# GenkiK/monodepth2

Measured on AMD Instinct MI355X. Metric: training images/sec at 640x192 mono, 1/2/4/8 GPUs; loss delta vs ref, higher is better.
Workload: dtype f32; 1 GPU; mono_640x192 ResNet-18 batch=12/GPU full train step (configs[1]); global_batch=12, height=192, width=640, parallelism=dp1, step=hipgraph replay

## Files before the change

include/md2hot.h:

```cpp
#ifndef MD2HOT_H
#define MD2HOT_H

#include <stddef.h>
#include <stdint.h>

#ifdef __cplusplus
extern "C" {
#endif

#define MD2_ABI_VERSION 24
#define MD2_MAX_SCALES 4
#define MD2_MAX_SRC 3

#define MD2_OK 0
#define MD2_ERR_ARG (-1)
#define MD2_ERR_HIP (-2)

#define MD2_NO_SSIM          (1u << 0)
#define MD2_AVG_REPROJECTION (1u << 1)
#define MD2_NO_AUTOMASK      (1u << 2)
#define MD2_V1_MULTISCALE    (1u << 3)
#define MD2_T_PER_SCALE      (1u << 4)
#define MD2_PREDICTIVE_MASK  (1u << 5)

// ... 136 lines not shown
int md2_adam_apply_dev(const md2_adam_chunk* table, const int* chunk_start, int k_begin, int k_end,
                       const float* const* grads, double beta1, double beta2, double eps, const float* hyper,
                       void* stream);

int md2_pose_fwd(int32_t frames, int32_t batch, uint32_t invert_mask, const float* axisangle,
                 const float* translation, float* T, void* stream);
int md2_pose_bwd(int32_t frames, int32_t batch, uint32_t invert_mask, const float* axisangle,
                 const float* translation, const float* grad_T, float* grad_axisangle,
                 float* grad_translation, void* stream);

typedef struct md2_aug_desc {
    int32_t items;
    int32_t frames;
    int32_t in_height, in_width;
    int32_t height, width;
    int32_t num_scales;
    int32_t reserved;
} md2_aug_desc;

#define MD2_AUG_BRIGHTNESS 0
#define MD2_AUG_CONTRAST   1
#define MD2_AUG_SATURATION 2
#define MD2_AUG_HUE        3

typedef struct md2_aug_item {
    uint8_t flip;
    uint8_t color_aug;
    uint8_t hue_shift;
    uint8_t reserved;
    uint8_t order[4];
    float brightness, contrast, saturation;
} md2_aug_item;

typedef struct md2_aug_plan md2_aug_plan;

md2_aug_plan* md2_aug_plan_create(const md2_aug_desc* desc);
void md2_aug_plan_destroy(md2_aug_plan* plan);

int md2_aug_run(md2_aug_plan* plan, const uint8_t* frames, const md2_aug_item* items,
                float* const* color, float* const* color_aug, void* stream);
int md2_aug_run2(md2_aug_plan* plan, const uint8_t* frames, const md2_aug_item* items,
                 float* const* color, float* const* color_aug, uint32_t* src8, void* stream);

#define MD2_BN_RELU     (1u << 0)
#define MD2_BN_RESIDUAL (1u << 1)
#define MD2_BN_BF16     (1u << 2)

typedef struct md2_bn_desc {
    int64_t pixels;
    int32_t channels;
    uint32_t flags;
    float eps, momentum;
    int32_t groups;
    int32_t reserved;
} md2_bn_desc;

size_t md2_bn_workspace_bytes(const md2_bn_desc* desc);
int md2_bn_fwd(const md2_bn_desc* desc, const void* x, const float* gamma, const float* beta,
               const void* residual, float* running_mean, float* running_var, void* y,
               float* save_mean, float* save_invstd, void* workspace, void* stream);
int md2_bn_bwd(const md2_bn_desc* desc, const void* x, const void* y, const void* grad_y,
               const float* gamma, const float* save_mean, const float* save_invstd,
               void* grad_x, void* grad_residual, float* grad_gamma, float* grad_beta,
               void* workspace, void* stream);
int md2_bn_bwd_multi(const md2_bn_desc* desc, const void* x, const void* y, const void* grad_y,
                     const void* grad_y2, const void* grad_y3, const float* gamma, const float* save_mean,
                     const float* save_invstd, void* grad_x, void* grad_residual, float* grad_gamma,
                     float* grad_beta, void* workspace, void* stream);
int md2_bn_fwd_mask(const md2_bn_desc* desc, const void* x, const float* gamma, const float* beta,
                    const void* residual, float* running_mean, float* running_var, void* y, uint8_t* relu_mask,
                    float* save_mean, float* save_invstd, void* workspace, void* stream);
int md2_bn_bwd_mask(const md2_bn_desc* desc, const void* x, const uint8_t* relu_mask, const void* grad_y,
                    const void* grad_y2, const void* grad_y3, const float* gamma, const float* save_mean,
                    const float* save_invstd, void* grad_x, void* grad_residual, float* grad_gamma,
                    float* grad_beta, void* workspace, void* stream);

#define MD2_POOL_BF16 (1u << 0)

typedef struct md2_pool_desc {
    int32_t batch, channels, height, width;
    uint32_t flags;
    int32_t reserved;
} md2_pool_desc;

int md2_maxpool3s2_fwd(const md2_pool_desc* desc, const void* x, void* y, uint32_t* idx, void* stream);
int md2_maxpool3s2_bwd(const md2_pool_desc* desc, const uint32_t* idx, const void* grad_y, void* grad_x,
                       void* stream);
int md2_maxpool3s2_bwd_add(const md2_pool_desc* desc, const uint32_t* idx, const void* grad_y, const void* grad_add,
                           void* grad_x, void* stream);
int md2_maxpool3s2_bwd_multi(const md2_pool_desc* desc, const uint32_t* idx, const void* grad_y, const void* grad_y2,
                             const void* grad_add, void* grad_x, void* stream);

#define MD2_CONV_NO_SPLIT  (1u << 1)
#define MD2_CONV_TILE_N32  (1u << 2)
#define MD2_CONV_TILE_N64  (1u << 3)
#define MD2_CONV_TILE_N128 (1u << 4)
#define MD2_CONV_X6        (1u << 5)
#define MD2_CONV_BM256     (1u << 6)
#define MD2_CONV_PRESPLIT  (1u << 7)
#define MD2_CONV_PATCH     (1u << 8)
#define MD2_CONV_S2_ONE    (1u << 9)
#define MD2_CONV_WS        (1u << 10)
#define MD2_CONV_BF16      (1u << 11)

typedef struct md2_conv_desc {
    int32_t batch, height, width, in_channels;
    int32_t out_channels, kernel_h, kernel_w, stride, pad;
    uint32_t flags;
} md2_conv_desc;

size_t md2_conv_workspace_bytes(const md2_conv_desc* desc);
int md2_conv_split_weights(const md2_conv_desc* desc, const float* weight, void* planes_fwd, void* planes_dgrad,
                           void* stream);
typedef struct md2_wsplit_entry {
    const float* weight;
    void* planes_fwd;
    void* planes_dgrad;
    int32_t co, kt, ci;
    int32_t block0;
    void* planes_col;
} md2_wsplit_entry;
int md2_conv_split_weights_multi(const md2_wsplit_entry* table, int n, int total_blocks, void* stream);
int md2_conv_bf16_weights(const md2_conv_desc* desc, const float* weight, void* w_fwd, void* w_dgrad, void* stream);
int md2_conv_bf16_weights_multi(const md2_wsplit_entry* table, int n, int total_blocks, void* stream);
int md2_conv_fwd(const md2_conv_desc* desc, const float* x, const float* weight, float* y, void* workspace,
                 void* stream);
int md2_conv_dgrad(const md2_conv_desc* desc, const float* grad_y, const float* weight, float* grad_x,
                   void* workspace, void* stream);
int md2_conv_col2im(const md2_conv_desc* desc, const float* cols, float* grad_x, void* stream);
int md2_conv_wgrad(const md2_conv_desc* desc, const float* x, const float* grad_y, float* grad_weight,
                   void* workspace, void* stream);
int md2_conv_direct(const md2_conv_desc* desc, const float* x, const float* wk, float* y, void* stream);
size_t md2_conv_wgrad_direct_workspace_bytes(const md2_conv_desc* desc);
int md2_conv_wgrad_direct(const md2_conv_desc* desc, const float* x, const float* grad_y, float* grad_weight,
                          void* workspace, void* stream);

#define MD2_EVAL_POST_PROCESS (1u << 0)
#define MD2_EVAL_RESIZE_DEPTH (1u << 1)
#define MD2_EVAL_GT_RANGE     (1u << 2)
#define MD2_EVAL_MEDIAN_SCALE (1u << 3)
#define MD2_EVAL_MEDIAN_LOWER (1u << 4)
#define MD2_EVAL_POOL_BATCH   (1u << 5)
#define MD2_EVAL_OUT 10

typedef struct md2_eval_desc {
    int32_t batch;
    int32_t height, width;
    int32_t gt_height, gt_width;
    int32_t crop_y0, crop_y1, crop_x0, crop_x1;
    uint32_t flags;
    double min_depth, max_depth;
    float eval_min, eval_max;
    double scale_factor;
} md2_eval_desc;

size_t md2_depth_eval_workspace_bytes(const md2_eval_desc* desc);
int md2_depth_eval(const md2_eval_desc* desc, const float* disp, const float* disp_flipped, const float* gt,
                   float* out, void* workspace, void* stream);

#ifdef __cplusplus
}
#endif
#endif
```

monodepth2_amd/_lib.py:

```python
from __future__ import annotations

import ctypes
import os
import threading

import torch

from .build import LIB_PATH as _BUILT_LIB
from .build import source_hash

LIB_PATH = os.environ.get("MD2_LIB", _BUILT_LIB)

MAX_SCALES = 4
MAX_SRC = 3
ABI_VERSION = 24

NO_SSIM = 1 << 0
AVG_REPROJECTION = 1 << 1
NO_AUTOMASK = 1 << 2
V1_MULTISCALE = 1 << 3
T_PER_SCALE = 1 << 4
PREDICTIVE_MASK = 1 << 5

_vp = ctypes.c_void_p


class Desc(ctypes.Structure):
    _fields_ = [("batch", ctypes.c_int32), ("height", ctypes.c_int32), ("width", ctypes.c_int32),
                ("num_src", ctypes.c_int32), ("num_scales", ctypes.c_int32), ("flags", ctypes.c_uint32),
                ("min_depth", ctypes.c_float), ("max_depth", ctypes.c_float),
                ("disparity_smoothness", ctypes.c_float), ("disp_dtype", ctypes.c_uint32),
                ("seed", ctypes.c_uint64)]


class Tensors(ctypes.Structure):
    _fields_ = [("disp", _vp * MAX_SCALES),
                ("color", (_vp * (1 + MAX_SRC)) * MAX_SCALES),
                ("K", _vp * MAX_SCALES),
                ("inv_K", _vp * MAX_SCALES),
                ("T", _vp),
                ("noise", _vp),
                ("seed_ptr", _vp),
                ("mask", _vp),
                ("src8", _vp)]


_lock = threading.Lock()
_lib = None

EXPORTS = ["md2_abi_version", "md2_last_error", "md2_workspace_bytes", "md2_select_bytes",
           "md2_photometric_fwd", "md2_photometric_bwd", "md2_generate_images", "md2_tiebreak_noise",
           "md2_timing_begin", "md2_timing_end", "md2_timing_calls", "md2_decoder_pad_fwd", "md2_decoder_pad_bwd",
           "md2_decoder_pad_workspace_bytes", "md2_adam_step", "md2_adam_step_dev", "md2_adam_hyper", "md2_adam_apply_dev", "md2_encoder_input",
           "md2_pose_fwd", "md2_pose_bwd", "md2_aug_plan_create", "md2_aug_plan_destroy", "md2_aug_run",
           "md2_bn_workspace_bytes", "md2_bn_fwd", "md2_bn_bwd", "md2_maxpool3s2_fwd", "md2_maxpool3s2_bwd",
           "md2_disp_head_workspace_bytes", "md2_disp_head_fwd", "md2_disp_head_bwd",
           "md2_stem_wgrad_workspace_bytes", "md2_stem_wgrad", "md2_stem_fwd", "md2_conv_col2im", "md2_bias_act_fwd", "md2_bias_act_bwd",
           "md2_bias_act_workspace_bytes", "md2_maxpool3s2_bwd_add", "md2_bn_bwd_multi",
           "md2_conv_fwd", "md2_conv_workspace_bytes", "md2_conv_split_weights",
           "md2_conv_dgrad", "md2_conv_wgrad", "md2_conv_direct", "md2_conv_wgrad_direct",
           "md2_conv_wgrad_direct_workspace_bytes", "md2_conv_split_weights_multi", "md2_bn_fwd_mask",
           "md2_bn_bwd_mask", "md2_build_id", "md2_maxpool3s2_bwd_multi", "md2_decoder_pad_bwd2", "md2_aug_run2",
           "md2_conv_bf16_weights", "md2_conv_bf16_weights_multi",
           "md2_depth_eval", "md2_depth_eval_workspace_bytes"]

DTYPE_F32 = 0
DTYPE_BF16 = 1
PAD_ELU = 1 << 0
PAD_UPSAMPLE = 1 << 1
PAD_NHWC = 1 << 2
PAD_BF16 = 1 << 3


class PadDesc(ctypes.Structure):
    _fields_ = [("batch", ctypes.c_int32), ("channels", ctypes.c_int32), ("height", ctypes.c_int32),
                ("width", ctypes.c_int32), ("skip_channels", ctypes.c_int32), ("flags", ctypes.c_uint32)]


class AugDesc(ctypes.Structure):
    _fields_ = [("items", ctypes.c_int32), ("frames", ctypes.c_int32), ("in_height", ctypes.c_int32),
                ("in_width", ctypes.c_int32), ("height", ctypes.c_int32), ("width", ctypes.c_int32),
                ("num_scales", ctypes.c_int32), ("reserved", ctypes.c_int32)]


class AugItem(ctypes.Structure):
    _fields_ = [("flip", ctypes.c_uint8), ("color_aug", ctypes.c_uint8), ("hue_shift", ctypes.c_uint8),
                ("reserved", ctypes.c_uint8), ("order", ctypes.c_uint8 * 4), ("brightness", ctypes.c_float),
                ("contrast", ctypes.c_float), ("saturation", ctypes.c_float)]


BN_RELU = 1 << 0
BN_RESIDUAL = 1 << 1
BN_BF16 = 1 << 2


class BnDesc(ctypes.Structure):
    _fields_ = [("pixels", ctypes.c_int64), ("channels", ctypes.c_int32), ("flags", ctypes.c_uint32),
                ("eps", ctypes.c_float), ("momentum", ctypes.c_float), ("groups", ctypes.c_int32),
                ("reserved", ctypes.c_int32)]


POOL_BF16 = 1 << 0


CONV_NO_SPLIT = 1 << 1
CONV_TILE_N32 = 1 << 2
CONV_TILE_N64 = 1 << 3
CONV_TILE_N128 = 1 << 4
CONV_X6 = 1 << 5
CONV_BM256 = 1 << 6
CONV_PRESPLIT = 1 << 7
CONV_PATCH = 1 << 8
CONV_S2_ONE = 1 << 9
CONV_WS = 1 << 10
CONV_BF16 = 1 << 11


class ConvDesc(ctypes.Structure):
    _fields_ = [("batch", ctypes.c_int32), ("height", ctypes.c_int32), ("width", ctypes.c_int32),
                ("in_channels", ctypes.c_int32), ("out_channels", ctypes.c_int32), ("kernel_h", ctypes.c_int32),
                ("kernel_w", ctypes.c_int32), ("stride", ctypes.c_int32), ("pad", ctypes.c_int32),
                ("flags", ctypes.c_uint32)]


class WsplitEntry(ctypes.Structure):
    _fields_ = [("weight", _vp), ("planes_fwd", _vp), ("planes_dgrad", _vp), ("co", ctypes.c_int32),
                ("kt", ctypes.c_int32), ("ci", ctypes.c_int32), ("block0", ctypes.c_int32), ("planes_col", _vp)]


class PoolDesc(ctypes.Structure):
    _fields_ = [("batch", ctypes.c_int32), ("channels", ctypes.c_int32), ("height", ctypes.c_int32),
                ("width", ctypes.c_int32), ("flags", ctypes.c_uint32), ("reserved", ctypes.c_int32)]


HEAD_WEIGHT_CL = 1 << 0
HEAD_BF16 = 1 << 1


class HeadDesc(ctypes.Structure):
    _fields_ = [("batch", ctypes.c_int32), ("channels", ctypes.c_int32), ("height", ctypes.c_int32),
                ("width", ctypes.c_int32), ("flags", ctypes.c_uint32)]


STEM_WEIGHT_CL = 1 << 0
STEM_BF16 = 1 << 1


class StemDesc(ctypes.Structure):
    _fields_ = [("batch", ctypes.c_int32), ("channels", ctypes.c_int32), ("height", ctypes.c_int32),
                ("width", ctypes.c_int32), ("flags", ctypes.c_uint32)]


# ... 88 lines not shown
    L.md2_generate_images.restype = ctypes.c_int
    L.md2_generate_images.argtypes = [ctypes.POINTER(Desc), ctypes.POINTER(Tensors),
                                      ctypes.POINTER(_vp), ctypes.POINTER(_vp), ctypes.POINTER(_vp), _vp]
    L.md2_tiebreak_noise.restype = ctypes.c_int
    L.md2_tiebreak_noise.argtypes = [ctypes.POINTER(Desc), _vp, ctypes.c_int, _vp, _vp]
    L.md2_decoder_pad_fwd.restype = ctypes.c_int
    L.md2_decoder_pad_fwd.argtypes = [ctypes.POINTER(PadDesc), _vp, _vp, _vp, _vp, _vp]
    L.md2_decoder_pad_bwd.restype = ctypes.c_int
    L.md2_decoder_pad_bwd.argtypes = [ctypes.POINTER(PadDesc), _vp, _vp, _vp, _vp, _vp, _vp, _vp, _vp]
    L.md2_decoder_pad_bwd2.restype = ctypes.c_int
    L.md2_decoder_pad_bwd2.argtypes = [ctypes.POINTER(PadDesc)] + [_vp] * 9
    L.md2_encoder_input.restype = ctypes.c_int
    L.md2_encoder_input.argtypes = [ctypes.c_int, ctypes.c_int, ctypes.c_int, ctypes.c_int, ctypes.c_int, _vp,
                                    ctypes.c_float, ctypes.c_float, _vp, _vp]
    L.md2_adam_step.restype = ctypes.c_int
    L.md2_adam_step.argtypes = [_vp, _vp, ctypes.c_int, _vp, ctypes.c_double, ctypes.c_double, ctypes.c_double,
                                ctypes.c_double, ctypes.c_int, _vp]
    L.md2_adam_step_dev.restype = ctypes.c_int
    L.md2_adam_step_dev.argtypes = [_vp, _vp, ctypes.c_int, _vp, _vp, ctypes.c_double, ctypes.c_double,
                                    ctypes.c_double, _vp, _vp, _vp]
    L.md2_adam_hyper.restype = ctypes.c_int
    L.md2_adam_hyper.argtypes = [_vp, ctypes.c_double, ctypes.c_double, _vp, _vp, _vp]
    L.md2_adam_apply_dev.restype = ctypes.c_int
    L.md2_adam_apply_dev.argtypes = [_vp, _vp, ctypes.c_int, ctypes.c_int, _vp, ctypes.c_double, ctypes.c_double,
                                     ctypes.c_double, _vp, _vp]
    L.md2_decoder_pad_workspace_bytes.restype = ctypes.c_size_t
    L.md2_decoder_pad_workspace_bytes.argtypes = [ctypes.POINTER(PadDesc)]
    L.md2_pose_fwd.restype = ctypes.c_int
    L.md2_pose_fwd.argtypes = [ctypes.c_int32, ctypes.c_int32, ctypes.c_uint32, _vp, _vp, _vp, _vp]
    L.md2_pose_bwd.restype = ctypes.c_int
    L.md2_pose_bwd.argtypes = [ctypes.c_int32, ctypes.c_int32, ctypes.c_uint32, _vp, _vp, _vp, _vp, _vp, _vp]
    L.md2_aug_plan_create.restype = _vp
    L.md2_aug_plan_create.argtypes = [ctypes.POINTER(AugDesc)]
    L.md2_aug_plan_destroy.restype = None
    L.md2_aug_plan_destroy.argtypes = [_vp]
    L.md2_aug_run.restype = ctypes.c_int
    L.md2_aug_run.argtypes = [_vp, _vp, _vp, ctypes.POINTER(_vp), ctypes.POINTER(_vp), _vp]
    L.md2_aug_run2.restype = ctypes.c_int
    L.md2_aug_run2.argtypes = [_vp, _vp, _vp, ctypes.POINTER(_vp), ctypes.POINTER(_vp), _vp, _vp]
    L.md2_bn_workspace_bytes.restype = ctypes.c_size_t
    L.md2_bn_workspace_bytes.argtypes = [ctypes.POINTER(BnDesc)]
    L.md2_bn_fwd.restype = ctypes.c_int
    L.md2_bn_fwd.argtypes = [ctypes.POINTER(BnDesc)] + [_vp] * 11
    L.md2_bn_bwd.restype = ctypes.c_int
    L.md2_bn_bwd.argtypes = [ctypes.POINTER(BnDesc)] + [_vp] * 12
    L.md2_maxpool3s2_fwd.restype = ctypes.c_int
    L.md2_maxpool3s2_fwd.argtypes = [ctypes.POINTER(PoolDesc), _vp, _vp, _vp, _vp]
    L.md2_maxpool3s2_bwd.restype = ctypes.c_int
    L.md2_maxpool3s2_bwd.argtypes = [ctypes.POINTER(PoolDesc), _vp, _vp, _vp, _vp]
    L.md2_bn_bwd_multi.restype = ctypes.c_int
    L.md2_bn_bwd_multi.argtypes = [ctypes.POINTER(BnDesc)] + [_vp] * 14
    L.md2_bn_fwd_mask.restype = ctypes.c_int
    L.md2_bn_fwd_mask.argtypes = [ctypes.POINTER(BnDesc)] + [_vp] * 12
    L.md2_bn_bwd_mask.restype = ctypes.c_int
    L.md2_bn_bwd_mask.argtypes = [ctypes.POINTER(BnDesc)] + [_vp] * 14
    L.md2_maxpool3s2_bwd_add.restype = ctypes.c_int
    L.md2_maxpool3s2_bwd_add.argtypes = [ctypes.POINTER(PoolDesc)] + [_vp] * 5
    L.md2_maxpool3s2_bwd_multi.restype = ctypes.c_int
    L.md2_maxpool3s2_bwd_multi.argtypes = [ctypes.POINTER(PoolDesc)] + [_vp] * 6
    L.md2_timing_begin.restype = ctypes.c_int
    L.md2_timing_begin.argtypes = [ctypes.c_int]
    L.md2_timing_calls.restype = ctypes.c_int
    L.md2_timing_calls.argtypes = [ctypes.POINTER(ctypes.c_double), ctypes.POINTER(ctypes.c_int),
                                   ctypes.POINTER(ctypes.c_double), ctypes.POINTER(ctypes.c_int)]
    L.md2_timing_end.restype = ctypes.c_int
    L.md2_timing_end.argtypes = [ctypes.POINTER(ctypes.c_double), ctypes.POINTER(ctypes.c_int),
                                 ctypes.POINTER(ctypes.c_double), ctypes.POINTER(ctypes.c_int)]


def lib():
    global _lib
    if _lib is not None:
        return _lib
    with _lock:
        if _lib is None:
            if not os.path.exists(LIB_PATH):
                raise RuntimeError(
                    f"{LIB_PATH} is not built. Build it with `python -m monodepth2_amd.build` "
                    "(hipcc --offload-arch=gfx950); there is no CPU fallback.")
            L = ctypes.CDLL(LIB_PATH, mode=ctypes.RTLD_GLOBAL)
            _declare(L)
            v = L.md2_abi_version()
            if v != ABI_VERSION:
                raise RuntimeError(f"libmd2hot ABI {v} != expected {ABI_VERSION}")
            if LIB_PATH == _BUILT_LIB:
                got, want = L.md2_build_id().decode(), source_hash()
                if got != want:
                    raise RuntimeError(
                        f"{LIB_PATH} was built from other sources (build id {got}, tree {want}): "
                        "rebuild it with `python -m monodepth2_amd.build`")
            _lib = L
    return _lib


def stream(device) -> int:
    idx = device.index if isinstance(device, torch.device) else device
    return torch._C._cuda_getCurrentRawStream(torch.cuda.current_device() if idx is None else idx)


def check(rc: int, what: str):
    if rc != 0:
        msg = lib().md2_last_error().decode(errors="replace")
        raise RuntimeError(f"{what} failed ({rc}): {msg}")


class KernelTimer:
# ... 21 lines not shown
```

monodepth2_amd/bn_ops.py:

```python
from __future__ import annotations

import contextlib
import ctypes
import os
from typing import Dict, Optional

import torch
import torch.nn as nn
import torch.nn.functional as F

from . import _lib

ENABLED = True
_GROUPS = 1


@contextlib.contextmanager
def bn_groups(n: int):
    global _GROUPS
    prev, _GROUPS = _GROUPS, int(n)
    try:
        yield
    finally:
        _GROUPS = prev

_CL = torch.channels_last
_workspaces: Dict[int, torch.Tensor] = {}
_workspaces_keep = []


def _workspace(device: torch.device, nbytes: int) -> torch.Tensor:
    key = _lib.stream(device)
    ws = _workspaces.get(key)
    if ws is None or ws.numel() < nbytes:
        if ws is not None:
            _workspaces_keep.append(ws)
        with torch.cuda.stream(torch.cuda.current_stream(device)):
            ws = torch.empty(max(nbytes, 1 << 20), dtype=torch.uint8, device=device)
        _workspaces[key] = ws
    return ws


_descs: Dict[tuple, tuple] = {}


def _desc(key: tuple):
    hit = _descs.get(key)
    if hit is None:
        d = _lib.BnDesc(*key, 0)
        hit = _descs[key] = (d, _lib.lib().md2_bn_workspace_bytes(ctypes.byref(d)))
    return hit


def _supported(C: int) -> bool:
    Q = C // 4
    return C % 4 == 0 and Q > 0 and (Q & (Q - 1)) == 0


class _BNAct(torch.autograd.Function):

    @staticmethod
    def forward(ctx, x, weight, bias, running_mean, running_var, residual, relu: bool, eps: float,
                momentum: float, groups: int, aliases: int = 0):
        B, C, H, W = x.shape
        flags = ((_lib.BN_RELU if relu else 0) | (_lib.BN_RESIDUAL if residual is not None else 0)
                 | (_lib.BN_BF16 if x.dtype == torch.bfloat16 else 0))
        key = (B * H * W, C, flags, eps, momentum, groups)
        d, nbytes = _desc(key)
        L = _lib.lib()
        ws = _workspace(x.device, nbytes)
        y = torch.empty_like(x, memory_format=_CL)
        stats = torch.empty(2, groups, C, device=x.device)
        mean, invstd = stats[0], stats[1]
        mask = torch.empty(x.numel() // 4, dtype=torch.uint8, device=x.device) if relu else None
        stream = _lib.stream(x.device)
        rc = L.md2_bn_fwd_mask(ctypes.byref(d), x.data_ptr(), weight.data_ptr(), bias.data_ptr(),
                               residual.data_ptr() if residual is not None else None,
                               running_mean.data_ptr() if running_mean is not None else None,
                               running_var.data_ptr() if running_var is not None else None,
                               y.data_ptr(), mask.data_ptr() if mask is not None else None,
                               mean.data_ptr(), invstd.data_ptr(), ws.data_ptr(), stream)
        _lib.check(rc, "md2_bn_fwd_mask")
        ctx.save_for_backward(x, mask, weight, mean, invstd)
        ctx.desc = key
        ctx.has_res = residual is not None
        if aliases:
            ctx.set_materialize_grads(False)
            return (y,) + tuple(y.view_as(y) for _ in range(aliases))
        return y

    @staticmethod
    def backward(ctx, *grads):
        x, mask, weight, mean, invstd = ctx.saved_tensors
        gs = [g.to(x.dtype).contiguous(memory_format=_CL) for g in grads if g is not None]
        if not gs:
            return (None,) * 11
        gy = gs[0]
        d, nbytes = _desc(ctx.desc)
        L = _lib.lib()
        ws = _workspace(x.device, nbytes)
        gx = torch.empty_like(x, memory_format=_CL)
        gr = torch.empty_like(x, memory_format=_CL) if ctx.has_res else None
        gw = torch.empty_like(weight)
        gb = torch.empty_like(weight)
        bwd, name = (L.md2_bn_bwd_mask, "md2_bn_bwd_mask") if mask is not None else \
            (L.md2_bn_bwd_multi, "md2_bn_bwd_multi")
        rc = bwd(ctypes.byref(d), x.data_ptr(), mask.data_ptr() if mask is not None else None,
                 gy.data_ptr(), gs[1].data_ptr() if len(gs) > 1 else None,
                 gs[2].data_ptr() if len(gs) > 2 else None,
                 weight.data_ptr(), mean.data_ptr(), invstd.data_ptr(), gx.data_ptr(),
                 gr.data_ptr() if gr is not None else None, gw.data_ptr(), gb.data_ptr(), ws.data_ptr(),
                 _lib.stream(x.device))
        _lib.check(rc, name)
        return gx, gw, gb, None, None, gr, None, None, None, None, None


def bn_act(bn: nn.BatchNorm2d, x: torch.Tensor, residual: Optional[torch.Tensor] = None,
           relu: bool = True, aliases: int = 0):
    if not 0 <= aliases <= 2:
        raise ValueError("bn_act: at most two aliases")
    groups = _GROUPS if bn.training else 1
    if groups > 1 and x.shape[0] % groups:
        raise ValueError(f"batch {x.shape[0]} does not split into {groups} BatchNorm groups")
    if (ENABLED and bn.training and x.is_cuda and x.dtype in (torch.float32, torch.bfloat16) and x.dim() == 4
            and bn.affine and bn.track_running_stats and bn.momentum is not None and _supported(x.shape[1])
            and x.numel() // 4 // groups < 2 ** 31
            and x.is_contiguous(memory_format=_CL) and x.shape[1] > 1
            and (residual is None or residual.is_contiguous(memory_format=_CL))):
        if residual is not None and residual.dtype != x.dtype:
            residual = residual.to(x.dtype)
        if bn.num_batches_tracked is not None:
            bn.num_batches_tracked.add_(groups)
        k = aliases if torch.is_grad_enabled() else 0
        out = _BNAct.apply(x, bn.weight, bn.bias, bn.running_mean, bn.running_var, residual, relu, bn.eps,
                           bn.momentum, groups, k)
        if aliases and not k:
            return (out,) * (aliases + 1)
        return out
    y = bn(x) if groups == 1 else torch.cat([bn(xc) for xc in x.chunk(groups)], 0)
    if residual is not None:
        y = y + residual
    y = F.relu(y) if relu else y
    return (y,) * (aliases + 1) if aliases else y


_ALIAS_SUM = os.environ.get("MD2_ALIAS_SUM", "1") != "0"


class _MaxPool(torch.autograd.Function):

    @staticmethod
    def forward(ctx, x, with_alias: bool = False, out_alias: bool = False):
        B, C, H, W = x.shape
        Ho, Wo = (H - 1) // 2 + 1, (W - 1) // 2 + 1
        d = _lib.PoolDesc(B, C, H, W, _lib.POOL_BF16 if x.dtype == torch.bfloat16 else 0, 0)
        y = torch.empty((B, C, Ho, Wo), device=x.device, dtype=x.dtype, memory_format=_CL)
        idx = torch.empty(B * Ho * Wo * C // 4, device=x.device, dtype=torch.int32)
        stream = _lib.stream(x.device)
        _lib.check(_lib.lib().md2_maxpool3s2_fwd(ctypes.byref(d), x.data_ptr(), y.data_ptr(), idx.data_ptr(), stream),
                   "md2_maxpool3s2_fwd")
        ctx.save_for_backward(idx)
        ctx.desc = (B, C, H, W, d.flags, 0)
        ctx.xshape, ctx.dtype = x.shape, x.dtype
        ctx.with_alias, ctx.out_alias = with_alias, out_alias
        if not (with_alias or out_alias):
            return y
        ctx.set_materialize_grads(False)
        outs = (y,) + ((y.view_as(y),) if out_alias else ()) + ((x.view_as(x),) if with_alias else ())
        return outs

    @staticmethod
    def backward(ctx, gy, *rest):
        (idx,) = ctx.saved_tensors
        rest = list(rest)
        gy2 = rest.pop(0) if ctx.out_alias else None
        galias = rest.pop(0) if ctx.with_alias else None
        if gy is None:
            gy, gy2 = gy2, None
        if gy is None:
            return (galias.to(ctx.dtype) if galias is not None else None), None, None
        gy = gy.to(ctx.dtype).contiguous(memory_format=_CL)
        if gy2 is not None:
            gy2 = gy2.to(ctx.dtype).contiguous(memory_format=_CL)
        if galias is not None:
            galias = galias.to(ctx.dtype).contiguous(memory_format=_CL)
        gx = torch.empty(ctx.xshape, device=gy.device, dtype=ctx.dtype, memory_format=_CL)
        d = _lib.PoolDesc(*ctx.desc)
        _lib.check(_lib.lib().md2_maxpool3s2_bwd_multi(ctypes.byref(d), idx.data_ptr(), gy.data_ptr(),
                                                       gy2.data_ptr() if gy2 is not None else None,
                                                       galias.data_ptr() if galias is not None else None,
                                                       gx.data_ptr(), _lib.stream(gy.device)),
                   "md2_maxpool3s2_bwd_multi")
        return gx, None, None


def _pool_ok(pool: nn.MaxPool2d, x: torch.Tensor) -> bool:
# ... 21 lines not shown
```

monodepth2_amd/build.py:

```python
from __future__ import annotations

import hashlib
import os
import shutil
import subprocess
import sys

HERE = os.path.dirname(os.path.abspath(__file__))
CSRC = os.path.join(HERE, "csrc")
INCLUDE = os.path.join(os.path.dirname(HERE), "include")
LIB_NAME = "libmd2hot.so"
LIB_PATH = os.path.join(CSRC, LIB_NAME)
SOURCES = ["md2hot.hip", "decoder.hip", "pose.hip", "augment.hip", "bnorm.hip", "pool.hip", "adam.hip", "disphead.hip", "stem.hip", "bias_act.hip", "conv.hip", "direct.hip", "glue.hip", "eval.hip"]
ARCH = os.environ.get("MD2_OFFLOAD_ARCH", "gfx950")


def hipcc() -> str:
    for cand in (os.environ.get("HIPCC"), "/opt/rocm/bin/hipcc", shutil.which("hipcc")):
        if cand and os.path.exists(cand):
            return cand
    raise RuntimeError("hipcc not found (ROCm toolchain required to build libmd2hot.so)")


def needs_build() -> bool:
    if not os.path.exists(LIB_PATH):
        return True
    t = os.path.getmtime(LIB_PATH)
    deps = [os.path.join(CSRC, s) for s in SOURCES] + [os.path.join(INCLUDE, "md2hot.h"),
                                                       os.path.join(CSRC, "md2_bf16.h")]
    if any(os.path.getmtime(d) > t for d in deps):
        return True
    return built_id(LIB_PATH) != source_hash()


def built_id(path: str):
    try:
        with open(path, "rb") as f:
            data = f.read()
    except OSError:
        return None
    i = data.find(BUILD_ID_MARKER)
    if i < 0:
        return None
    i += len(BUILD_ID_MARKER)
    return data[i:i + 16].decode("ascii", errors="replace")


BUILD_ID_MARKER = b"md2-build-id:"


FLAGS = {"md2hot.hip": ["-fno-slp-vectorize", "-mllvm", "--amdgpu-sched-strategy=iterative-ilp"],
         "conv.hip": ["-mllvm", "--amdgpu-sched-strategy=max-ilp"],
         "bnorm.hip": ["-mllvm", "--amdgpu-sched-strategy=max-ilp"],
         "decoder.hip": ["-mllvm", "--amdgpu-sched-strategy=max-ilp"],
         "disphead.hip": ["-fno-slp-vectorize"], "glue.hip": ["-fno-slp-vectorize"]}


def source_hash() -> str:
    h = hashlib.sha256()
    for path in [os.path.join(CSRC, s) for s in SOURCES] + [os.path.join(INCLUDE, "md2hot.h"),
                                                          os.path.join(CSRC, "md2_bf16.h")]:
        h.update(os.path.basename(path).encode())
        with open(path, "rb") as f:
            h.update(f.read())
    h.update(repr(sorted(FLAGS.items())).encode())
    h.update(ARCH.encode())
    return h.hexdigest()[:16]


def build(force: bool = False, verbose: bool = False) -> str:
    if not force and not needs_build():
        return LIB_PATH
    import concurrent.futures as cf
    objdir = os.path.join(CSRC, "obj")
    os.makedirs(objdir, exist_ok=True)
    base = [hipcc(), "-O3", f"--offload-arch={ARCH}", "-std=c++17", "-fPIC", "-I" + INCLUDE]
    bid = ['-DMD2_BUILD_ID="%s"' % source_hash()]

    def compile_one(src):
        obj = os.path.join(objdir, os.path.splitext(src)[0] + ".o")
        cmd = base + FLAGS.get(src, []) + (bid if src == "glue.hip" else []) + ["-c", os.path.join(CSRC, src), "-o", obj]
        if verbose:
            print(" ".join(cmd), file=sys.stderr)
        subprocess.run(cmd, check=True)
        return obj

    with cf.ThreadPoolExecutor(max_workers=min(len(SOURCES), os.cpu_count() or 1)) as ex:
        objs = list(ex.map(compile_one, SOURCES))
    tmp = LIB_PATH + ".tmp"
    cmd = [hipcc(), f"--offload-arch={ARCH}", "-fPIC", "-shared", "-o", tmp] + objs
    if verbose:
        print(" ".join(cmd), file=sys.stderr)
    subprocess.run(cmd, check=True)
    os.replace(tmp, LIB_PATH)
    return LIB_PATH


if __name__ == "__main__":
    print(build(force="--force" in sys.argv, verbose=True))
```

monodepth2_amd/conv_ops.py:

```python
from __future__ import annotations

import ctypes
import os
import types
from typing import Dict, Tuple

import torch
import torch.nn as nn
import torch.nn.functional as F

from . import _lib

_CL = torch.channels_last
ENABLED = True
AUTOTUNE = True
PLANE_BANK = os.environ.get("MD2_PLANE_BANK", "1") != "0"
_ws: Dict[Tuple[int, int], torch.Tensor] = {}
_choice: Dict[tuple, int] = {}
_times: Dict[tuple, dict] = {}
X6 = _lib.CONV_X6
BM256 = _lib.CONV_BM256
PRESPLIT = _lib.CONV_PRESPLIT
PATCH = _lib.CONV_PATCH
S2_ONE = _lib.CONV_S2_ONE
# ... 4 lines not shown
_NAMES_X6 = ("x6", "x6_256", "x6_ns", "x6_256_ns")
_NAMES_X6P = ("x6p", "x6p_256", "x6p_ns", "x6p_256_ns")
_WFLAGS = (X6 | WS, X6 | WS | BM256)
_NAMES_WS = ("x6ws", "x6ws_256")


def _x6_flags(gemm_c: int, k: int, stride: int, n_out: int):
    flags, names = _FLAGS, _NAMES_X6
    if n_out > 64 and gemm_c >= 32:
        flags, names = flags + _WFLAGS, names + _NAMES_WS
    if k == 3 and stride == 1 and gemm_c % 32 == 0 and n_out > 16:
        return flags + _PFLAGS, names + _NAMES_X6P
    return flags, names


_ws_keep = []


def _workspace(device: torch.device, nbytes: int) -> torch.Tensor:
    key = (device.index, _lib.stream(device))
    ws = _ws.get(key)
    if ws is None or ws.numel() < nbytes:
        if ws is not None:
            _ws_keep.append(ws)
        ws = torch.empty(max(nbytes, 1 << 20), dtype=torch.uint8, device=device)
        _ws[key] = ws
    return ws


_descs: Dict[tuple, tuple] = {}


def _desc_ws(x: torch.Tensor, w: torch.Tensor, stride: int, pad: int, flags: int = 0):
    k = (tuple(x.shape), tuple(w.shape), stride, pad, flags)
    hit = _descs.get(k)
    if hit is None:
        B, C, H, W = x.shape
        N, _, KH, KW = w.shape
        d = _lib.ConvDesc(B, H, W, C, N, KH, KW, stride, pad, flags)
        hit = _descs[k] = (d, _lib.lib().md2_conv_workspace_bytes(ctypes.byref(d)))
    return hit


def _desc(x: torch.Tensor, w: torch.Tensor, stride: int, pad: int, flags: int = 0):
    return _desc_ws(x, w, stride, pad, flags)[0]


def _call(fn: str, x, w, stride, pad, flags, p0, p1, p2, device):
    d, nbytes = _desc_ws(x, w, stride, pad, flags)
    ws = _workspace(device, nbytes)
    _lib.check(getattr(_lib.lib(), fn)(ctypes.byref(d), p0, p1, p2, ws.data_ptr(), _lib.stream(device)), fn)


def _fwd(x, w, stride, pad, flags=0):
    B, _, H, W = x.shape
    N, _, KH, KW = w.shape
    y = torch.empty(B, N, (H + 2 * pad - KH) // stride + 1, (W + 2 * pad - KW) // stride + 1, device=x.device,
                    memory_format=_CL)
    _call("md2_conv_fwd", x, w, stride, pad, flags, x.data_ptr(), w.data_ptr(), y.data_ptr(), x.device)
    return y


def _dgrad(gy, x, w, pad, flags=0, stride=1):
    gx = torch.empty_like(x, memory_format=_CL)
    _call("md2_conv_dgrad", x, w, stride, pad, flags, gy.data_ptr(), w.data_ptr(), gx.data_ptr(), x.device)
    return gx


def _dgrad_col(gy, x, w, stride, pad, flags):
    N, C, KH, KW = w.shape
    B, _, H, W = x.shape
    pc = _bank.col_planes(w) if (_bank is not None and flags & X6 and _COL_BANK) else None
    if pc is not None:
        cols = _fwd_planes(gy, _col_shape(KH * KW * C, N), pc, 1, 0, flags)
    else:
        wcol = w.permute(2, 3, 1, 0).reshape(KH * KW * C, N, 1, 1).contiguous()
        cols = _fwd(gy, wcol, 1, 0, flags)
    gx = torch.empty_like(x, memory_format=_CL)
    d = _lib.ConvDesc(B, H, W, C, N, KH, KW, stride, pad, 0)
    _lib.check(_lib.lib().md2_conv_col2im(ctypes.byref(d), cols.data_ptr(), gx.data_ptr(), _lib.stream(x.device)),
               "md2_conv_col2im")
    return gx


_COL_BANK = os.environ.get("MD2_COL_PLANES", "1") != "0"


def _col_shape(rows: int, n: int):
    return types.SimpleNamespace(shape=torch.Size((rows, n, 1, 1)))


def _col_x(w):
    return types.SimpleNamespace(shape=torch.Size((1, w.shape[1], 8, 8)))


def _x6_ok(x, w) -> bool:
    return x.shape[1] % 8 == 0 and w.shape[0] % 8 == 0


def _x6_s2_ok(x, w, stride) -> bool:
    return stride == 2 and _x6_ok(x, w) and w.shape[0] >= 32


def _split_weights(x, w, stride, pad, dgrad: bool):
    n = w.numel()
    pf = torch.empty(3 * n, dtype=torch.bfloat16, device=w.device)
    pd = torch.empty(3 * n, dtype=torch.bfloat16, device=w.device) if dgrad else None
    _lib.check(_lib.lib().md2_conv_split_weights(ctypes.byref(_desc(x, w, stride, pad)), w.data_ptr(), pf.data_ptr(),
                                                 pd.data_ptr() if pd is not None else None,
                                                 _lib.stream(w.device)),
               "md2_conv_split_weights")
    return pf, pd
# ... 94 lines not shown
                                                         pf.data_ptr(), None, _lib.stream(w.device)),
                       "md2_conv_split_weights")
            self.entries[k] = [w, pf, None, pc]
        else:
            e[3] = pc
        self._col_pending.add(k)
        self.dirty = True
        return None


_bank: PlaneBank | None = None
_bank_bf: PlaneBank | None = None


def plane_bank() -> PlaneBank:
    global _bank
    if _bank is None:
        _bank = PlaneBank()
    return _bank


def plane_bank_bf16() -> PlaneBank:
    global _bank_bf
    if _bank_bf is None:
        _bank_bf = PlaneBank(bf16=True)
    return _bank_bf


def begin_step(device: torch.device, bf16: bool = False):
    (plane_bank_bf16() if bf16 else plane_bank()).begin_step(device)


def end_step():
    for b in (_bank, _bank_bf):
        if b is not None:
            b.end_step()


def _planes_for(x, w, stride, pad, need_dg: bool):
    if _bank is not None:
        got = _bank.planes(x, w, stride, pad, need_dg)
        if got is not None:
            return got
    return _split_weights(x, w, stride, pad, need_dg)


def _bank_dgrad(x, w, stride, pad):
    if _bank is None:
        return None
    got = _bank.planes(x, w, stride, pad, True)
    return got[1] if got is not None else None


def _fwd_planes(x, w, planes, stride, pad, flags):
    B, _, H, W = x.shape
    N, _, KH, KW = w.shape
    y = torch.empty(B, N, (H + 2 * pad - KH) // stride + 1, (W + 2 * pad - KW) // stride + 1, device=x.device,
                    memory_format=_CL)
    _call("md2_conv_fwd", x, w, stride, pad, flags | PRESPLIT, x.data_ptr(), planes.data_ptr(), y.data_ptr(),
          x.device)
    return y


def _dgrad_planes(gy, x, w, planes, pad, flags, stride=1):
    gx = torch.empty_like(x, memory_format=_CL)
    _call("md2_conv_dgrad", x, w, stride, pad, flags | PRESPLIT, gy.data_ptr(), planes.data_ptr(), gx.data_ptr(),
          x.device)
    return gx


def _wgrad(gy, x, w, stride, pad, flags=0):
    gw = torch.empty_like(w, memory_format=_CL)
    _call("md2_conv_wgrad", x, w, stride, pad, flags, x.data_ptr(), gy.data_ptr(), gw.data_ptr(), x.device)
    return gw


def _miopen_bwd(gy, x, w, stride, pad, mask):
    return torch.ops.aten.convolution_backward(gy, x, w, None, (stride, stride), (pad, pad), (1, 1), False, (0, 0), 1,
                                               mask)


_pinned: Dict[tuple, str] = {}


def _key_of(row) -> tuple:
    return (row["op"], tuple(row["x"]), tuple(row["w"]), int(row["stride"]), int(row["pad"]))


def load_choices(path: str) -> int:
    import json
    with open(path) as f:
        rows = json.load(f)["rows"]
    for row in rows:
        _pinned[_key_of(row)] = row["kept"]
    _choice.clear()
    return len(rows)


def save_choices(path: str) -> int:
    import json
    rows = []
    for k, i in sorted(_choice.items()):
        names = _names.get(k)
        if names is None:
            continue
        op, xs, ws, st, pd = k
        rows.append({"op": op, "x": list(xs), "w": list(ws), "stride": st, "pad": pd, "kept": names[i],
                     "ms": _times.get(k, {})})
    with open(path, "w") as f:
        json.dump({"rows": rows}, f, indent=1)
    return len(rows)


# ... 112 lines not shown
            i = names.index(name)
            changed += int(_choice.get(k) != i)
            _choice[k] = i
    return changed


_DIRECT = ((16, 16), (32, 16), (16, 32))
_ddescs: Dict[tuple, object] = {}


def _direct_ok(cin: int, cout: int, k: int, stride: int) -> bool:
    return k == 3 and stride == 1 and (cin, cout) in _DIRECT


def _direct(a: torch.Tensor, wk: torch.Tensor, pad: int, cout: int, flags: int = 0) -> torch.Tensor:
    B, C, H, W = a.shape
    y = torch.empty(B, cout, H + 2 * pad - 2, W + 2 * pad - 2, device=a.device, memory_format=_CL,
                    dtype=torch.bfloat16 if flags & BF else torch.float32)
    k = (tuple(a.shape), cout, pad, flags)
    d = _ddescs.get(k)
    if d is None:
        d = _ddescs[k] = _lib.ConvDesc(B, H, W, C, cout, 3, 3, 1, pad, flags)
    _lib.check(_lib.lib().md2_conv_direct(ctypes.byref(d), a.data_ptr(), wk.data_ptr(), y.data_ptr(),
                                          _lib.stream(a.device)), "md2_conv_direct")
    return y


def _direct_wgrad(gy, x, w, pad, flags=0):
    N, C = w.shape[0], w.shape[1]
    gw = torch.empty_like(w, memory_format=_CL)
    d = _desc(x, w, 1, pad, flags)
    nbytes = _lib.lib().md2_conv_wgrad_direct_workspace_bytes(ctypes.byref(d))
    ws = _workspace(x.device, nbytes)
    _lib.check(_lib.lib().md2_conv_wgrad_direct(ctypes.byref(d), x.data_ptr(), gy.data_ptr(), gw.data_ptr(),
                                                ws.data_ptr(), _lib.stream(x.device)), "md2_conv_wgrad_direct")
    return gw


def _direct_fwd(x, w, pad, flags=0):
    return _direct(x, w.permute(2, 3, 1, 0).contiguous(), pad, w.shape[0], flags)


def _direct_dgrad(gy, w, pad, flags=0):
    return _direct(gy, w.flip(2, 3).permute(2, 3, 0, 1).contiguous(), 2 - pad, w.shape[1], flags)


def _fits(cin: int, cout: int) -> bool:
    return cin % 4 == 0 and cout % 4 == 0


class _Conv(torch.autograd.Function):

    @staticmethod
    def forward(ctx, x, weight, stride: int, pad: int):
        ctx.stride, ctx.pad = stride, pad
        ctx.key = (tuple(x.shape), tuple(weight.shape), stride, pad)
        x6 = _x6_ok(x, weight)
        xf, xn = _x6_flags(x.shape[1], weight.shape[2], stride, weight.shape[0]) if x6 else ((), ())
        cands = None
        i = _cached("fwd", ctx.key)
        if i is None or not (x6 and i < len(xf)):
            direct = _direct_ok(weight.shape[1], weight.shape[0], weight.shape[2], stride)
            cands = [(lambda f=f: _fwd(x, weight, stride, pad, f)) for f in xf] + \
                [lambda: _fwd(x, weight, stride, pad)] + \
                ([lambda: _direct_fwd(x, weight, pad), lambda: _direct_fwd(x, weight, pad, X6)] if direct else []) + \
                [lambda: F.conv2d(x, weight, None, stride, pad)]
            names = list(xn) + ["f32mfma"] + (["direct", "direct_x6"] if direct else []) + ["miopen"]
            if i is None:
                i = _fastest("fwd", ctx.key, cands, names)
        planes_dg = None
        if x6 and i < len(xf):
            pf, planes_dg = _planes_for(x, weight, stride, pad, stride == 1 or _x6_s2_ok(x, weight, stride))
            y = _fwd_planes(x, weight, pf, stride, pad, xf[i])
        else:
            y = cands[i]()
        ctx.save_for_backward(x, weight, planes_dg)
        return y

    @staticmethod
    def backward(ctx, gy):
        x, w, planes_dg = ctx.saved_tensors
        s, p = ctx.stride, ctx.pad
        gy = gy.contiguous(memory_format=_CL)
        need_x, need_w = ctx.needs_input_grad[0], ctx.needs_input_grad[1]
        gx = gw = None
        mi_x = mi_w = False
        if need_x:
            if s == 1:
                x6 = _x6_ok(x, w)
                xf, xn = _x6_flags(w.shape[0], w.shape[2], 1, w.shape[1]) if x6 else ((), ())
                direct = _direct_ok(w.shape[0], w.shape[1], w.shape[2], s)
                cands = [(lambda f=f: _dgrad(gy, x, w, p, f)) for f in xf] + \
                    [lambda: _dgrad(gy, x, w, p)] + \
                    ([lambda: _direct_dgrad(gy, w, p), lambda: _direct_dgrad(gy, w, p, X6)] if direct else []) + \
                    [lambda: _miopen_bwd(gy, x, w, s, p, (True, False, False))[0]]
                names = list(xn) + ["f32mfma"] + (["direct", "direct_x6"] if direct else []) + ["miopen"]
                i = _fastest("dgrad", ctx.key, cands, names)
                if x6 and i < len(xf) and planes_dg is None:
                    planes_dg = _bank_dgrad(x, w, s, p)
                if x6 and i < len(xf) and planes_dg is not None:
                    gx = _dgrad_planes(gy, x, w, planes_dg, p, xf[i])
                elif i < len(cands) - 1:
                    gx = cands[i]()
                else:
                    mi_x = True
            elif _x6_s2_ok(x, w, s):
                sf = (X6, X6 | S2_ONE)
                cands = [(lambda f=f: _dgrad(gy, x, w, p, f, 2)) for f in sf] + \
                    [lambda: _dgrad_col(gy, x, w, s, p, X6), lambda: _dgrad_col(gy, x, w, s, p, X6 | BM256)] + \
                    [lambda: _miopen_bwd(gy, x, w, s, p, (True, False, False))[0]]
                i = _fastest("dgrad", ctx.key, cands, ["x6_s2", "x6_s2one", "x6_col", "x6_col_256", "miopen"])
                if i < len(sf) and planes_dg is None:
                    planes_dg = _bank_dgrad(x, w, s, p)
                if i < len(sf):
                    gx = (_dgrad_planes(gy, x, w, planes_dg, p, sf[i], 2) if planes_dg is not None else cands[i]())
                elif i < len(cands) - 1:
                    gx = cands[i]()
                else:
                    mi_x = True
            else:
                mi_x = True
        if need_w:
            direct = _direct_ok(w.shape[1], w.shape[0], w.shape[2], s) and w.shape[0] == 16
            x6 = _x6_ok(x, w)
            pw = x6 and w.shape[2] == 3 and w.shape[3] == 3 and s == 1
            wsw = x6 and w.shape[0] > 64
            cands = ([lambda: _wgrad(gy, x, w, s, p, X6)] if x6 else []) + \
                ([lambda: _wgrad(gy, x, w, s, p, X6 | WS), lambda: _wgrad(gy, x, w, s, p, X6 | WS | BM256)]
                 if wsw else []) + \
                ([lambda: _wgrad(gy, x, w, s, p, X6 | PATCH)] if pw else []) + [lambda: _wgrad(gy, x, w, s, p)] + \
                ([lambda: _direct_wgrad(gy, x, w, p), lambda: _direct_wgrad(gy, x, w, p, X6)] if direct else []) + \
                [lambda: _miopen_bwd(gy, x, w, s, p, (False, True, False))[1]]
            i = _fastest("wgrad", ctx.key, cands,
                         (["x6"] if x6 else []) + (["x6ws", "x6ws_256"] if wsw else []) + (["x6pw"] if pw else []) + ["f32mfma"] +
                         (["direct", "direct_x6"] if direct else []) + ["miopen"])
            if i < len(cands) - 1:
                gw = cands[i]()
            else:
                mi_w = True
        if mi_x or mi_w:
            gxm, gwm, _ = _miopen_bwd(gy, x, w, s, p, (mi_x, mi_w, False))
            gx = gxm if mi_x else gx
            gw = gwm if mi_w else gw
        return gx, gw, None, None


BF16_ENABLED = os.environ.get("MD2_CONV_BF16", "1") != "0"
BF = _lib.CONV_BF16
_FLAGS_BF = (BF, BF | BM256, BF | NO_SPLIT, BF | BM256 | NO_SPLIT)
_NAMES_BF = ("bf16", "bf16_256", "bf16_ns", "bf16_256_ns")


_PFLAGS_BF = (BF | PATCH, BF | PATCH | NO_SPLIT, BF | PATCH | BM256, BF | PATCH | BM256 | NO_SPLIT)
_PNAMES_BF = ("bf16p", "bf16p_ns", "bf16p_256", "bf16p_256_ns")


def _bf_flags(n_out: int, gemm_c: int = 0, k: int = 0, stride: int = 0):
    wide = n_out > 64
    fl = _FLAGS_BF if wide else (_FLAGS_BF[0], _FLAGS_BF[2])
    nm = _NAMES_BF if wide else (_NAMES_BF[0], _NAMES_BF[2])
    if k == 3 and stride == 1 and gemm_c % 32 == 0 and n_out > 16:
        fl = fl + (_PFLAGS_BF if wide else _PFLAGS_BF[:2])
        nm = nm + (_PNAMES_BF if wide else _PNAMES_BF[:2])
    return fl, nm


def _bf_planes_for(x, w, stride, pad, need_dg: bool):
    if _bank_bf is not None:
        got = _bank_bf.planes(x, w, stride, pad, need_dg)
        if got is not None:
            return got
    return _bf16_weights(x, w, stride, pad, need_dg)


def _w_bf16_view(x, w, stride, pad):
    N, C, kh, kw = w.shape
    pf = _bf_planes_for(x, w, stride, pad, False)[0]
    return pf.view(N, kh, kw, C).permute(0, 3, 1, 2)


def _fwd_bf(x, w, plane, stride, pad, flags):
    B, _, H, W = x.shape
    N, _, KH, KW = w.shape
    y = torch.empty(B, N, (H + 2 * pad - KH) // stride + 1, (W + 2 * pad - KW) // stride + 1, device=x.device,
                    dtype=torch.bfloat16, memory_format=_CL)
    _call("md2_conv_fwd", x, w, stride, pad, flags, x.data_ptr(), plane.data_ptr(), y.data_ptr(), x.device)
    return y


def _dgrad_bf(gy, x, w, plane, pad, flags, stride=1):
    gx = torch.empty_like(x, memory_format=_CL)
    _call("md2_conv_dgrad", x, w, stride, pad, flags, gy.data_ptr(), plane.data_ptr(), gx.data_ptr(), x.device)
    return gx


def _wgrad_bf(gy, x, w, stride, pad, flags=BF):
    gw = torch.empty_like(w, memory_format=_CL)
# ... 65 lines not shown
                                ["bf16"] + (["bf16pw"] if pw else []) + (["bf16ws_256"] if w256 else []) +
                                (["direct_bf16"] if direct else []))]()
        return gx, gw, None, None


def _bf16_autocast() -> bool:
    return torch.is_autocast_enabled("cuda") and torch.get_autocast_dtype("cuda") == torch.bfloat16


def _bf16_ok(x: torch.Tensor, weight: torch.Tensor, stride: int, pad: int) -> bool:
    return (ENABLED and BF16_ENABLED and x.is_cuda and x.dim() == 4 and x.dtype in (torch.bfloat16, torch.float32)
            and weight.dtype == torch.float32 and weight.shape[2] == weight.shape[3]
            and _fits(weight.shape[1], weight.shape[0]) and x.is_contiguous(memory_format=_CL)
            and weight.is_contiguous(memory_format=_CL) and stride >= 1 and 0 <= pad < weight.shape[2]
            and _sizes_ok(x, weight, stride, pad) and _bf16_autocast())


def conv2d_bf16(x: torch.Tensor, weight: torch.Tensor, stride: int, pad: int) -> torch.Tensor:
    xb = x if x.dtype == torch.bfloat16 else x.to(torch.bfloat16)
    with torch.autocast("cuda", enabled=False):
        return _ConvBF16.apply(xb, weight, stride, pad)


def _sizes_ok(x: torch.Tensor, weight: torch.Tensor, stride: int, pad: int) -> bool:
    B, _, H, W = x.shape
    Co, _, kh, kw = weight.shape
    ho = (H + 2 * pad - kh) // stride + 1
    wo = (W + 2 * pad - kw) // stride + 1
    return (ho >= 1 and wo >= 1 and x.numel() < 2 ** 29 and B * ho * wo * Co < 2 ** 29
            and weight.numel() < 2 ** 29)


def _shape_ok(x: torch.Tensor, weight: torch.Tensor, stride: int = 1, pad: int = 0) -> bool:
    return (ENABLED and x.is_cuda and x.dtype == torch.float32 and weight.dtype == torch.float32 and x.dim() == 4
            and weight.shape[2] == weight.shape[3] and _fits(weight.shape[1], weight.shape[0])
            and x.is_contiguous(memory_format=_CL) and weight.is_contiguous(memory_format=_CL)
            and not torch.is_autocast_enabled() and stride >= 1 and 0 <= pad < weight.shape[2]
            and _sizes_ok(x, weight, stride, pad))


def supports(conv: nn.Conv2d, x: torch.Tensor) -> bool:
    k, s, p = conv.kernel_size, conv.stride, conv.padding
    return (conv.bias is None and conv.groups == 1 and tuple(conv.dilation) == (1, 1)
            and conv.padding_mode == "zeros" and k[0] == k[1] and s[0] == s[1] and p[0] == p[1] and p[0] < k[0]
            and _shape_ok(x, conv.weight, s[0], p[0]))


def _module_ok(conv: nn.Conv2d) -> bool:
    k, s, p = conv.kernel_size, conv.stride, conv.padding
    return (conv.bias is None and conv.groups == 1 and tuple(conv.dilation) == (1, 1)
            and conv.padding_mode == "zeros" and k[0] == k[1] and s[0] == s[1] and p[0] == p[1] and p[0] < k[0])


def conv2d(conv: nn.Conv2d, x: torch.Tensor) -> torch.Tensor:
    if supports(conv, x):
        return _Conv.apply(x, conv.weight, conv.stride[0], conv.padding[0])
    if _module_ok(conv) and _bf16_ok(x, conv.weight, conv.stride[0], conv.padding[0]):
        return conv2d_bf16(x, conv.weight, conv.stride[0], conv.padding[0])
    return conv(x)


def conv2d_w(x: torch.Tensor, weight: torch.Tensor, stride: int = 1, pad: int = 0) -> torch.Tensor:
    if _shape_ok(x, weight, stride, pad):
        return _Conv.apply(x, weight, stride, pad)
    if _bf16_ok(x, weight, stride, pad):
        return conv2d_bf16(x, weight, stride, pad)
    return F.conv2d(x, weight, None, stride, pad)


if os.environ.get("MD2_CONV_CHOICES"):
    load_choices(os.environ["MD2_CONV_CHOICES"])
```

monodepth2_amd/csrc/bnorm.hip:

```cpp

#include <hip/hip_runtime.h>

#include <stdint.h>
#include <stdlib.h>

#include "md2_bf16.h"
#include "md2hot.h"

int md2_report_error(int code, const char* msg);

namespace {

constexpr int kThreads = 256;
constexpr int kMaxBlocks = 1024;

struct Map {
    int Q;
    int QPT;
    int PPB;
};

__host__ __device__ inline Map make_map(int C) {
    Map m;
    m.Q = C / 4;
    m.QPT = m.Q > kThreads ? m.Q / kThreads : 1;
    m.PPB = m.Q >= kThreads ? 1 : kThreads / m.Q;
    return m;
}

struct Work {
    float* part;
    float* coef;
};

__host__ __device__ __forceinline__ Work work(void* ws, int G, int C, int NG) {
    Work w;
    w.part = (float*)ws;
    w.coef = w.part + 2 * (size_t)NG * G * C;
    return w;
}

__device__ __forceinline__ float4 ld4(const float* p) { return *(const float4*)p; }
__device__ __forceinline__ void st4(float* p, float4 v) { *(float4*)p = v; }

template <typename T>
__device__ __forceinline__ float4 ldT(const void* p, size_t off) { return md2::ld4T<T>(p, off); }
template <typename T>
__device__ __forceinline__ void stT(void* p, size_t off, float4 v) { md2::st4T<T>(p, off, v); }

__device__ void block_partials(float4 a, float4 b, int q, int pl, const Map& m, int C, int rows, int row, Work w,
                               float4 (*lds)[kThreads]) {
    lds[0][threadIdx.x] = a;
    lds[1][threadIdx.x] = b;
    __syncthreads();
    for (int half = m.PPB / 2; half > 0; half /= 2) {
        if (pl < half) {
            const int o = threadIdx.x + half * m.Q;
            const float4 u = lds[0][o], v = lds[1][o];
            a.x += u.x; a.y += u.y; a.z += u.z; a.w += u.w;
            b.x += v.x; b.y += v.y; b.z += v.z; b.w += v.w;
            lds[0][threadIdx.x] = a;
            lds[1][threadIdx.x] = b;
        }
        __syncthreads();
    }
    if (pl == 0) {
        float* pa = w.part + (size_t)(4 * q) * rows + row;
        float* pb = w.part + ((size_t)C + 4 * q) * rows + row;
        pa[0] = a.x; pa[rows] = a.y; pa[2 * (size_t)rows] = a.z; pa[3 * (size_t)rows] = a.w;
        pb[0] = b.x; pb[rows] = b.y; pb[2 * (size_t)rows] = b.z; pb[3 * (size_t)rows] = b.w;
    }
    __syncthreads();
}

template <typename T>
__global__ void __launch_bounds__(kThreads) bn_stats_kernel(const void* __restrict__ x, long long P, int C, int G,
                                                            void* ws) {
    const Map m = make_map(C);
    const int NG = gridDim.y, grp = blockIdx.y;
    const Work w = work(ws, G, C, NG);
    x = (const char*)x + (size_t)grp * P * C * sizeof(T);
    __shared__ float4 lds[2][kThreads];
    for (int qq = 0; qq < m.QPT; ++qq) {
        const int q = (threadIdx.x % m.Q) + qq * kThreads, pl = threadIdx.x / m.Q;
        float4 s = {0.f, 0.f, 0.f, 0.f}, ss = {0.f, 0.f, 0.f, 0.f};
        auto acc = [&](const float4 v) {
            s.x += v.x; s.y += v.y; s.z += v.z; s.w += v.w;
            ss.x += v.x * v.x; ss.y += v.y * v.y; ss.z += v.z * v.z; ss.w += v.w * v.w;
        };
        const long long stride = (long long)G * m.PPB;
        long long p = (long long)blockIdx.x * m.PPB + pl;
        for (; p + 3 * stride < P; p += 4 * stride) {
            const float4 v0 = ldT<T>(x, p * C + 4 * q), v1 = ldT<T>(x, (p + stride) * C + 4 * q),
                         v2 = ldT<T>(x, (p + 2 * stride) * C + 4 * q), v3 = ldT<T>(x, (p + 3 * stride) * C + 4 * q);
            acc(v0); acc(v1); acc(v2); acc(v3);
        }
        for (; p < P; p += stride) acc(ldT<T>(x, p * C + 4 * q));
        block_partials(s, ss, q, pl, m, C, NG * G, grp * G + blockIdx.x, w, lds);
    }
}

__device__ bool channel_sums(Work w, int rows, int r0, int G, int C, int c, double& a, double& b) {
    __shared__ double red[2][kThreads / 64];
    static_assert(kMaxBlocks <= 4 * kThreads, "four partial rows per thread at most");
    const float* ca = w.part + (size_t)c * rows + r0;
    const float* cb = w.part + ((size_t)C + c) * rows + r0;
    float pa[4], pb[4];
#pragma unroll
    for (int u = 0; u < 4; ++u) {
        const int g = threadIdx.x + u * kThreads;
        pa[u] = g < G ? ca[g] : 0.f;
        pb[u] = g < G ? cb[g] : 0.f;
    }
    a = 0.0;
    b = 0.0;
#pragma unroll
    for (int u = 0; u < 4; ++u) {
        a += pa[u];
        b += pb[u];
    }
#pragma unroll
    for (int o = 32; o > 0; o >>= 1) {
        a += __shfl_xor(a, o, 64);
        b += __shfl_xor(b, o, 64);
    }
    if ((threadIdx.x & 63) == 0) {
        red[0][threadIdx.x >> 6] = a;
        red[1][threadIdx.x >> 6] = b;
    }
    __syncthreads();
    a = red[0][0];
    b = red[1][0];
#pragma unroll
    for (int i = 1; i < kThreads / 64; ++i) {
        a += red[0][i];
        b += red[1][i];
    }
    __syncthreads();
    return threadIdx.x == 0;
}

__global__ void __launch_bounds__(kThreads) bn_stats_final_kernel(long long P, int C, int G, int NG, float eps,
// ... 353 lines not shown
        if (g2) {
            float u[8];
            ld8bf(g2, o, u);
#pragma unroll
            for (int e = 0; e < 8; ++e) gv[e] += u[e];
        }
        if (g3) {
            float u[8];
            ld8bf(g3, o, u);
#pragma unroll
            for (int e = 0; e < 8; ++e) gv[e] += u[e];
        }
        if (RELU) {
            if constexpr (MIN) {
                const uint32_t m = ((const uint16_t*)y)[o / 8];
#pragma unroll
                for (int e = 0; e < 8; ++e) gv[e] = ((m >> ((e & 3) + 8 * (e >> 2))) & 1u) ? gv[e] : 0.f;
            } else {
                float yv[8];
                ld8bf(y, o, yv);
#pragma unroll
                for (int e = 0; e < 8; ++e) gv[e] = yv[e] > 0.f ? gv[e] : 0.f;
            }
        }
        ld8bf(x, o, v);
#pragma unroll
        for (int e = 0; e < 8; ++e) {
            s[e] += gv[e];
            sx[e] += gv[e] * (v[e] - mu[e]);
        }
    }
    block_partials(make_float4(s[0], s[1], s[2], s[3]), make_float4(sx[0], sx[1], sx[2], sx[3]), 2 * q8, pl, m8, C,
                   NG * G, grp * G + blockIdx.x, w, lds);
    block_partials(make_float4(s[4], s[5], s[6], s[7]), make_float4(sx[4], sx[5], sx[6], sx[7]), 2 * q8 + 1, pl, m8,
                   C, NG * G, grp * G + blockIdx.x, w, lds);
}

bool reduce8_on() {
    static const bool on = [] {
        const char* e = getenv("MD2_BN_RED8");
        return !(e && e[0] == '0');
    }();
    return on;
}

bool apply8_on() {
    static const bool on = [] {
        const char* e = getenv("MD2_BN_V8");
        return !(e && e[0] == '0');
    }();
    return on;
}

int blocks_for_stats(long long P, int C) {
    const Map m = make_map(C);
    const long long rows = (P + m.PPB - 1) / m.PPB;
    const long long g = (rows + 7) / 8;
    return (int)(g < 1 ? 1 : (g > kMaxBlocks ? kMaxBlocks : g));
}

int grid_elem(long long n4, int NG) {
    const long long cap = (4096 + NG - 1) / NG;
    const long long g = (n4 + kThreads - 1) / kThreads;
    return (int)(g < cap ? g : cap);
}

int groups_of(const md2_bn_desc* d) { return d->groups > 1 ? d->groups : 1; }

bool valid(const md2_bn_desc* d) {
    if (!d || d->channels < 4 || d->channels % 4) return false;
    if (d->groups < 0 || d->pixels % groups_of(d) || d->pixels / groups_of(d) < 2) return false;
    const int Q = d->channels / 4;
    if ((Q & (Q - 1)) != 0) return false;
    if ((long long)d->pixels / groups_of(d) * Q >= (1ll << 31)) return false;
    return Q >= kThreads ? (Q % kThreads == 0) : (kThreads % Q == 0);
}

template <typename T>
void launch_fwd(const md2_bn_desc* d, const void* x, const float* gamma, const float* beta, const void* residual,
                float* running_mean, float* running_var, void* y, float* save_mean, float* save_invstd,
                void* workspace, hipStream_t st, uint8_t* mask = nullptr) {
    const int NG = groups_of(d);
    const long long P = d->pixels / NG;
    const int C = d->channels, G = blocks_for_stats(P, C);
    if (sizeof(T) == 2 && C % 8 == 0 && C <= 8 * kThreads && reduce8_on())
        hipLaunchKernelGGL(bn_stats8_kernel<>, dim3(G, NG), dim3(kThreads), 0, st, x, P, C, G, workspace);
    else
        hipLaunchKernelGGL(bn_stats_kernel<T>, dim3(G, NG), dim3(kThreads), 0, st, x, P, C, G, workspace);
    hipLaunchKernelGGL(bn_stats_final_kernel, dim3(C), dim3(kThreads), 0, st, P, C, G, NG, d->eps, d->momentum,
                       running_mean, running_var, save_mean, save_invstd, workspace);
    const int n4g = (int)(P * C / 4);
    const bool relu = d->flags & MD2_BN_RELU, res = d->flags & MD2_BN_RESIDUAL;
    if (sizeof(T) == 2 && C % 8 == 0 && apply8_on()) {
        auto k8 = relu ? (mask ? (res ? bn_apply8_kernel<true, true, true> : bn_apply8_kernel<true, false, true>)
                               : (res ? bn_apply8_kernel<true, true> : bn_apply8_kernel<true, false>))
                       : (res ? bn_apply8_kernel<false, true> : bn_apply8_kernel<false, false>);
        hipLaunchKernelGGL(k8, dim3(grid_elem(n4g / 2, NG), NG), dim3(kThreads), 0, st, x, residual, gamma, beta,
                           save_mean, save_invstd, y, n4g / 2, C / 8, mask);
        return;
    }
    auto k = relu ? (mask ? (res ? bn_apply_kernel<T, true, true, true> : bn_apply_kernel<T, true, false, true>)
                          : (res ? bn_apply_kernel<T, true, true> : bn_apply_kernel<T, true, false>))
                  : (res ? bn_apply_kernel<T, false, true> : bn_apply_kernel<T, false, false>);
    hipLaunchKernelGGL(k, dim3(grid_elem(n4g, NG), NG), dim3(kThreads), 0, st, x, residual, gamma, beta, save_mean,
                       save_invstd, y, n4g, C / 4, mask);
}

template <typename T>
void launch_bwd(const md2_bn_desc* d, const void* x, const void* y, const void* grad_y, const void* grad_y2,
                const void* grad_y3, const float* gamma,
                const float* save_mean, const float* save_invstd, void* grad_x, void* grad_residual,
                float* grad_gamma, float* grad_beta, void* workspace, hipStream_t st, bool mask_in = false) {
    const int NG = groups_of(d);
    const long long P = d->pixels / NG;
    const int C = d->channels, G = blocks_for_stats(P, C);
    const bool relu = d->flags & MD2_BN_RELU, res = d->flags & MD2_BN_RESIDUAL;
    auto red = relu ? (mask_in ? bn_bwd_reduce_kernel<T, true, true> : bn_bwd_reduce_kernel<T, true>)
                    : bn_bwd_reduce_kernel<T, false>;
    if (sizeof(T) == 2 && C % 8 == 0 && C <= 8 * kThreads && reduce8_on())
        red = relu ? (mask_in ? bn_bwd_reduce8_kernel<true, true> : bn_bwd_reduce8_kernel<true>)
                   : bn_bwd_reduce8_kernel<false>;
    hipLaunchKernelGGL(red, dim3(G, NG), dim3(kThreads), 0, st, x, y, grad_y, grad_y2, grad_y3, P, C, G, save_mean,
                       workspace);
    hipLaunchKernelGGL(bn_bwd_final_kernel, dim3(C), dim3(kThreads), 0, st, P, C, G, NG, gamma, save_invstd,
                       grad_gamma, grad_beta, workspace);
    const int n4g = (int)(P * C / 4);
    const float* coef = work(workspace, G, C, NG).coef;
    if (sizeof(T) == 2 && C % 8 == 0 && apply8_on()) {
        auto k8 = relu ? (mask_in ? (res ? bn_bwd_apply8_kernel<true, true, true> : bn_bwd_apply8_kernel<true, false, true>)
                                  : (res ? bn_bwd_apply8_kernel<true, true> : bn_bwd_apply8_kernel<true, false>))
                       : (res ? bn_bwd_apply8_kernel<false, true> : bn_bwd_apply8_kernel<false, false>);
        hipLaunchKernelGGL(k8, dim3(grid_elem(n4g / 2, NG), NG), dim3(kThreads), 0, st, x, y, grad_y, grad_y2,
                           grad_y3, save_mean, coef, grad_x, grad_residual, n4g / 2, C / 8, C, NG);
        return;
    }
    auto k = relu ? (mask_in ? (res ? bn_bwd_apply_kernel<T, true, true, true> : bn_bwd_apply_kernel<T, true, false, true>)
                             : (res ? bn_bwd_apply_kernel<T, true, true> : bn_bwd_apply_kernel<T, true, false>))
                  : (res ? bn_bwd_apply_kernel<T, false, true> : bn_bwd_apply_kernel<T, false, false>);
    hipLaunchKernelGGL(k, dim3(grid_elem(n4g, NG), NG), dim3(kThreads), 0, st, x, y, grad_y, grad_y2, grad_y3,
                       save_mean, coef, grad_x, grad_residual, n4g, C / 4, C, NG);
}

}

extern "C" {

size_t md2_bn_workspace_bytes(const md2_bn_desc* d) {
    if (!valid(d)) return 0;
    const int NG = groups_of(d);
    const int G = blocks_for_stats(d->pixels / NG, d->channels);
    return (2 * (size_t)NG * G * d->channels + 3 * (size_t)NG * d->channels) * sizeof(float);
}

int md2_bn_fwd_mask(const md2_bn_desc* d, const void* x, const float* gamma, const float* beta, const void* residual,
                    float* running_mean, float* running_var, void* y, uint8_t* relu_mask, float* save_mean,
                    float* save_invstd, void* workspace, void* stream) {
    if (!valid(d)) return md2_report_error(MD2_ERR_ARG, "bn: need pixels >= 2 and channels a multiple of 4 "
                                                        "with channels/4 dividing (or a multiple of) 256");
    if (!x || !gamma || !beta || !y || !save_mean || !save_invstd || !workspace ||
        ((d->flags & MD2_BN_RESIDUAL) && !residual) || (!running_mean != !running_var))
        return md2_report_error(MD2_ERR_ARG, "bn_fwd: NULL operand");
    if (relu_mask && !(d->flags & MD2_BN_RELU)) return md2_report_error(MD2_ERR_ARG, "bn_fwd: relu_mask without MD2_BN_RELU");
    if (d->flags & MD2_BN_BF16)
        launch_fwd<uint16_t>(d, x, gamma, beta, residual, running_mean, running_var, y, save_mean, save_invstd,
                             workspace, (hipStream_t)stream, relu_mask);
    else
        launch_fwd<float>(d, x, gamma, beta, residual, running_mean, running_var, y, save_mean, save_invstd,
                          workspace, (hipStream_t)stream, relu_mask);
    const hipError_t e = hipGetLastError();
    return e == hipSuccess ? MD2_OK : md2_report_error(MD2_ERR_HIP, hipGetErrorString(e));
}

int md2_bn_fwd(const md2_bn_desc* d, const void* x, const float* gamma, const float* beta, const void* residual,
               float* running_mean, float* running_var, void* y, float* save_mean, float* save_invstd,
               void* workspace, void* stream) {
    return md2_bn_fwd_mask(d, x, gamma, beta, residual, running_mean, running_var, y, nullptr, save_mean, save_invstd,
                           workspace, stream);
}

static int bn_bwd_impl(const md2_bn_desc* d, const void* x, const void* y, bool mask_in, const void* grad_y,
                       const void* grad_y2, const void* grad_y3, const float* gamma, const float* save_mean,
                       const float* save_invstd, void* grad_x, void* grad_residual, float* grad_gamma,
                       float* grad_beta, void* workspace, void* stream) {
    if (!valid(d)) return md2_report_error(MD2_ERR_ARG, "bn: unsupported shape");
    const bool relu = d->flags & MD2_BN_RELU, res = d->flags & MD2_BN_RESIDUAL;
    if (!x || !grad_y || !gamma || !save_mean || !save_invstd || !grad_x || !grad_gamma || !grad_beta ||
        !workspace || (relu && !y) || (res && !grad_residual) || (grad_y3 && !grad_y2))
        return md2_report_error(MD2_ERR_ARG, "bn_bwd: NULL operand");
    if (d->flags & MD2_BN_BF16)
        launch_bwd<uint16_t>(d, x, y, grad_y, grad_y2, grad_y3, gamma, save_mean, save_invstd, grad_x,
                             grad_residual, grad_gamma, grad_beta, workspace, (hipStream_t)stream, mask_in);
    else
        launch_bwd<float>(d, x, y, grad_y, grad_y2, grad_y3, gamma, save_mean, save_invstd, grad_x, grad_residual,
                          grad_gamma, grad_beta, workspace, (hipStream_t)stream, mask_in);
    const hipError_t e = hipGetLastError();
    return e == hipSuccess ? MD2_OK : md2_report_error(MD2_ERR_HIP, hipGetErrorString(e));
}

int md2_bn_bwd_multi(const md2_bn_desc* d, const void* x, const void* y, const void* grad_y, const void* grad_y2,
                     const void* grad_y3, const float* gamma, const float* save_mean, const float* save_invstd,
                     void* grad_x, void* grad_residual, float* grad_gamma, float* grad_beta, void* workspace,
                     void* stream) {
    return bn_bwd_impl(d, x, y, false, grad_y, grad_y2, grad_y3, gamma, save_mean, save_invstd, grad_x, grad_residual,
                       grad_gamma, grad_beta, workspace, stream);
// ... 20 lines not shown
```

monodepth2_amd/csrc/conv.hip:

```cpp

#include <hip/hip_runtime.h>

#include <stdlib.h>

#include <stdint.h>

#include <algorithm>
#include <type_traits>

#include "md2hot.h"

int md2_report_error(int code, const char* msg);

namespace {

typedef float f32x16 __attribute__((ext_vector_type(16)));

constexpr int kThreads = 256;
constexpr int BM = 128;
constexpr int BK = 32;

enum { MODE_FWD = 0, MODE_DGRAD = 1, MODE_WGRAD = 2 };

__device__ __forceinline__ int swz(int r, int q) { return (q ^ (r >> 1)) & 7; }

struct ConvArgs {
    int B, H, W, C;
    int Ho, Wo;
    int N;
    int M;
    int P;
    int Cg;
    int KH, KW, stride, pad;
    int mblocks, nblocks, splits, chunks_per_split, nchunks;
    int a_elems, b_elems;
    int bn;
    int bm;
    int par, py, px, kh0, kw0, ntw, dy0, dx0, oHf, oWf;
    int flatk;
    int ptr, ptc;
    int ncls;
    int cls_blk[4], cls_py[4], cls_px[4], cls_kh0[4], cls_kw0[4], cls_ntw[4], cls_dy0[4], cls_dx0[4], cls_Ho[4],
        cls_Wo[4], cls_nchunks[4];
    const float* a;
    const float* b;
    float* y;
    int ybf16;
};

__device__ __forceinline__ int xcd_contiguous_block(int bid, int n) {
    const int q = n >> 3, r = n & 7;
    const int xcd = bid & 7, idx = bid >> 3;
    return xcd < r ? xcd * (q + 1) + idx : r * (q + 1) + (xcd - r) * q + idx;
}

__device__ __forceinline__ float4 bload(__amdgpu_buffer_rsrc_t r, int byte_off) {
    return __builtin_bit_cast(float4, __builtin_amdgcn_raw_buffer_load_b128(r, byte_off, 0, 0));
}

constexpr int kBad = 0x7fffffff;

__device__ __forceinline__ uint2 bload8(__amdgpu_buffer_rsrc_t r, int byte_off) {
    return __builtin_bit_cast(uint2, __builtin_amdgcn_raw_buffer_load_b64(r, byte_off, 0, 0));
}
__device__ __forceinline__ uint16_t f2bf16(float v) {
    const uint32_t u = __builtin_bit_cast(uint32_t, v);
    if ((u & 0x7fffffffu) > 0x7f800000u) return (uint16_t)((u >> 16) | 0x40u);
    return (uint16_t)((u + 0x7fffu + ((u >> 16) & 1u)) >> 16);
}
__device__ __forceinline__ float bf16_round(float v) {
    return __builtin_bit_cast(float, (uint32_t)f2bf16(v) << 16);
}

__device__ __forceinline__ int fdiv(int n, int d, float rd) {
    int q = (int)((float)n * rd);
    const int r = n - q * d;
    q += (r >= d) - (r < 0);
    return q;
}

template <int BN, int MODE>
struct Cfg {
    static constexpr int WAVES_M = BN == 32 ? 4 : 2;
    static constexpr int WAVES_N = 4 / WAVES_M;
    static constexpr int TM = BM / WAVES_M / 32;
    static constexpr int TN = BN / WAVES_N / 32;
    static constexpr bool A_ROWK = MODE != MODE_WGRAD;
    static constexpr bool B_ROWK = MODE == MODE_FWD;
    static constexpr int AQ = BM * BK / 4 / kThreads;
    static constexpr int BQ = BN * BK / 4 / kThreads;
    static constexpr int A_FLOATS = BM * BK, B_FLOATS = BN * BK;
};

template <int BN, int MODE>
__global__ __launch_bounds__(kThreads, BN == 128 ? 2 : (BN == 64 ? 3 : 4)) void conv_gemm_kernel(ConvArgs a) {
    using G = Cfg<BN, MODE>;
    constexpr int TM = G::TM, TN = G::TN, AQ = G::AQ, BQ = G::BQ;
    __shared__ float lds[2][G::A_FLOATS + G::B_FLOATS];

    const int tid = threadIdx.x, lane = tid & 63, wid = tid >> 6;
    const int wm = wid / G::WAVES_N, wn = wid % G::WAVES_N;
    int blk = xcd_contiguous_block(blockIdx.x, gridDim.x);
    const int nb = blk % a.nblocks;
    blk /= a.nblocks;
    const int mb = blk % a.mblocks, ks = blk / a.mblocks;
    const int m0 = mb * BM, n0 = nb * BN;
    const int t0 = ks * a.chunks_per_split;
    const int nchunks = min(a.chunks_per_split, a.nchunks - t0);
    const int KT = a.KH * a.KW;

    const int qa = tid & 7, ra = tid >> 3;
    int aih[AQ], aiw[AQ], apb[AQ];
    const __amdgpu_buffer_rsrc_t ar = __builtin_amdgcn_make_buffer_rsrc(
        (void*)a.a, 0, a.a_elems * 4, 0x00020000);
    if (MODE != MODE_WGRAD) {
#pragma unroll
        for (int j = 0; j < AQ; ++j) {
            const int m = m0 + ra + 32 * j;
            if (m < a.M) {
                const int b = m / (a.Ho * a.Wo), rem = m - b * a.Ho * a.Wo;
                const int oh = rem / a.Wo, ow = rem - oh * a.Wo;
                aih[j] = oh * a.stride - a.pad;
                aiw[j] = ow * a.stride - a.pad;
                apb[j] = ((b * a.H + aih[j]) * a.W + aiw[j]) * a.C + 4 * qa;
            } else {
                aih[j] = -(1 << 20);
                aiw[j] = 0;
                apb[j] = 0;
            }
        }
    }
    int wkh[AQ], wkw[AQ], wci[AQ];
    int pb_b = 0, pb_oh = 0, pb_ow = 0;
    if (MODE == MODE_WGRAD) {
#pragma unroll
        for (int j = 0; j < AQ; ++j) {
            const int m = m0 + 4 * (tid % (BM / 4));
            const int tap = m / a.C, ci = m - tap * a.C;
            wkh[j] = m < a.M ? tap / a.KW : -(1 << 20);
            wkw[j] = tap - (tap / a.KW) * a.KW;
            wci[j] = ci;
        }
        const int pk = t0 * BK + tid / (BM / 4);
        pb_b = pk / (a.Ho * a.Wo);
        const int rem = pk - pb_b * a.Ho * a.Wo;
        pb_oh = rem / a.Wo;
        pb_ow = rem - pb_oh * a.Wo;
// ... 100 lines not shown
#define CONV_MMA(buf)                                                                                        \
    {                                                                                                        \
        const float* As_ = lds[buf];                                                                         \
        const float* Bs_ = lds[buf] + G::A_FLOATS;                                                           \
        _Pragma("unroll") for (int kq = 0; kq < 4; ++kq) {                                                   \
            float fa[TM][4], fb[TN][4];                                                                      \
            _Pragma("unroll") for (int i = 0; i < TM; ++i) {                                                 \
                if (G::A_ROWK) {                                                                             \
                    const float4 v = *(const float4*)(As_ + (arow + 32 * i) * BK + 4 * swz(arow + 32 * i, 4 * h + kq)); \
                    fa[i][0] = v.x; fa[i][1] = v.y; fa[i][2] = v.z; fa[i][3] = v.w;                          \
                } else {                                                                                     \
                    _Pragma("unroll") for (int e = 0; e < 4; ++e)                                            \
                        fa[i][e] = As_[(16 * h + 4 * kq + e) * BM + arow + 32 * i];                          \
                }                                                                                            \
            }                                                                                                \
            _Pragma("unroll") for (int j = 0; j < TN; ++j) {                                                 \
                if (G::B_ROWK) {                                                                             \
                    const float4 v = *(const float4*)(Bs_ + (brow + 32 * j) * BK + 4 * swz(brow + 32 * j, 4 * h + kq)); \
                    fb[j][0] = v.x; fb[j][1] = v.y; fb[j][2] = v.z; fb[j][3] = v.w;                          \
                } else {                                                                                     \
                    _Pragma("unroll") for (int e = 0; e < 4; ++e)                                            \
                        fb[j][e] = Bs_[(16 * h + 4 * kq + e) * BN + brow + 32 * j];                          \
                }                                                                                            \
            }                                                                                                \
            _Pragma("unroll") for (int e = 0; e < 4; ++e)                                                    \
                _Pragma("unroll") for (int i = 0; i < TM; ++i)                                               \
                    _Pragma("unroll") for (int j = 0; j < TN; ++j)                                           \
                        acc[i][j] = __builtin_amdgcn_mfma_f32_32x32x2f32(fa[i][e], fb[j][e], acc[i][j], 0, 0, 0); \
        }                                                                                                    \
        asm volatile("" ::: "memory");                    \
    }

    CONV_LOAD(0, ra0, rb0);
    if (nchunks > 1) CONV_LOAD(1, ra1, rb1);
    CONV_STORE(0, ra0, rb0);
    __syncthreads();
    int t = 0;
    for (; t + 1 < nchunks; t += 2) {
        if (t + 2 < nchunks) CONV_LOAD(t + 2, ra0, rb0);
        CONV_MMA(0);
        CONV_STORE(1, ra1, rb1);
        __syncthreads();
        if (t + 3 < nchunks) CONV_LOAD(t + 3, ra1, rb1);
        CONV_MMA(1);
        if (t + 2 < nchunks) CONV_STORE(0, ra0, rb0);
        __syncthreads();
    }
    if (t < nchunks) CONV_MMA(0);
#undef CONV_LOAD
#undef CONV_STORE
#undef CONV_MMA

    float* out = a.y + (size_t)ks * a.M * a.N;
#pragma unroll
    for (int i = 0; i < TM; ++i)
#pragma unroll
        for (int j = 0; j < TN; ++j) {
            const int n = n0 + wn * (TN * 32) + 32 * j + (lane & 31);
            if (n < a.N) {
#pragma unroll
                for (int e = 0; e < 16; ++e) {
                    const int m = m0 + wm * (TM * 32) + 32 * i + (e & 3) + 8 * (e >> 2) + 4 * h;
                    if (m < a.M) out[MODE == MODE_WGRAD ? n * a.M + m : m * a.N + n] = acc[i][j][e];
                }
            }
        }
}

typedef __bf16 bf16x8 __attribute__((ext_vector_type(8)));
typedef __bf16 bf16x4 __attribute__((ext_vector_type(4)));
constexpr int XBK = 32;

__device__ __forceinline__ uint32_t hi16x2(float lo, float hi) {
    return __builtin_amdgcn_perm(__builtin_bit_cast(uint32_t, hi), __builtin_bit_cast(uint32_t, lo), 0x07060302u);
}
__device__ __forceinline__ float trunc16(float x) {
    return __builtin_bit_cast(float, __builtin_bit_cast(uint32_t, x) & 0xFFFF0000u);
}
__device__ __forceinline__ void split3(float4 v, bf16x4& p0, bf16x4& p1, bf16x4& p2) {
    const float x[4] = {v.x, v.y, v.z, v.w};
    float a[4], b[4], c[4];
#pragma unroll
    for (int i = 0; i < 4; ++i) {
        a[i] = trunc16(x[i]);
        const float r1 = x[i] - a[i];
        b[i] = trunc16(r1);
        c[i] = r1 - b[i];
    }
    typedef uint32_t u32x2 __attribute__((ext_vector_type(2)));
    u32x2 q0, q1, q2;
    q0.x = hi16x2(a[0], a[1]), q0.y = hi16x2(a[2], a[3]);
    q1.x = hi16x2(b[0], b[1]), q1.y = hi16x2(b[2], b[3]);
    q2.x = hi16x2(c[0], c[1]), q2.y = hi16x2(c[2], c[3]);
    p0 = __builtin_bit_cast(bf16x4, q0);
    p1 = __builtin_bit_cast(bf16x4, q1);
    p2 = __builtin_bit_cast(bf16x4, q2);
}

__device__ __forceinline__ int xidx(int r, int k) { return r * XBK + ((((k >> 3) ^ (r >> 2)) & 3) << 3) + (k & 7); }
__device__ __forceinline__ int xidx2(int r, int k) { return xidx(r ^ ((r >> 2) & 1), k); }
template <int MT>
__device__ __forceinline__ int xsw(int r, int k) {
    if constexpr (MT == 32) return xidx(r, k);
    return r * XBK + ((((k >> 3) ^ ((r >> 2) & 2)) & 3) << 3) + (k & 7);
}

// ... 363 lines not shown
        split(fa1);
        mma(0);
        asm volatile("" ::: "memory");
        store(1);
        wait_vm<AQ>();
        lds_sync();
        if (t + 1 >= nchunks) break;
        dma(t + 2, 0);
        load(t + 3, fa1);
        split(fa0);
        mma(1);
        asm volatile("" ::: "memory");
        store(0);
        wait_vm<AQ>();
        lds_sync();
    }

    float* out = a.y + (size_t)ks * a.M * a.N;
    auto orow = [&](int m) {
        if (!a.par || a.splits > 1) return m;
        const int hw = a.Ho * a.Wo, b = m / hw, rem = m - b * hw, oh = rem / a.Wo, ow = rem - oh * a.Wo;
        return (b * a.oHf + 2 * oh + a.py) * a.oWf + 2 * ow + a.px;
    };
    const bool obf = BF && a.ybf16 == 1 && a.splits == 1;
    auto put = [&](int m, int n, float v) {
        if (obf) ((uint16_t*)a.y)[orow(m) * a.N + n] = f2bf16(v);
        else out[orow(m) * a.N + n] = v;
    };
    if constexpr (G::MT == 16) {
        const int n = n0 + wn * 16 + (lane & 15);
        if (n < a.N) {
#pragma unroll
            for (int i = 0; i < TM; ++i)
#pragma unroll
                for (int e = 0; e < 4; ++e) {
                    const int m = m0 + wm * (TM * 16) + 16 * i + 4 * (lane >> 4) + e;
                    if (m < a.M) put(m, n, acc[i][e]);
                }
        }
    } else {
        const int n = n0 + wn * 32 + lr;
        if (n < a.N) {
#pragma unroll
            for (int i = 0; i < TM; ++i)
#pragma unroll
                for (int e = 0; e < 16; ++e) {
                    const int m = m0 + wm * (TM * 32) + 32 * i + (e & 3) + 8 * (e >> 2) + 4 * h;
                    if (m < a.M) put(m, n, acc[i][e]);
                }
        }
    }
}

template <int BMX>
__global__ __launch_bounds__(512, 1) void conv_x6ws_kernel(ConvArgs a) {
    constexpr int BN = 128, NP = 256;
    constexpr int TMc = BMX / 64, TNc = 2;
    constexpr int AQ = BMX * XBK / 4 / NP;
    constexpr int PIECES = 3 * BN / 16, BQ = PIECES / 4;
    constexpr int PA = BMX * XBK, PB = BN * XBK;
    static_assert(AQ * NP * 4 == BMX * XBK && BQ * 4 == PIECES, "staging must tile the chunk");
    __shared__ __bf16 lds[2][3 * (PA + PB)];

    const int tid = threadIdx.x, lane = tid & 63, wid = __builtin_amdgcn_readfirstlane(tid >> 6);
    const bool mfma_wave = wid < 4;
    int blk = xcd_contiguous_block(blockIdx.x, gridDim.x);
    const int nb = blk % a.nblocks;
    blk /= a.nblocks;
    const int mb = blk % a.mblocks, ks = blk / a.mblocks;
    const int m0 = mb * BMX, n0 = nb * BN;
    const int t0 = ks * a.chunks_per_split;
    const int nchunks = min(a.chunks_per_split, a.nchunks - t0);
    const int KT = a.KH * a.KW;
    const int cchunks = (a.C + XBK - 1) / XBK;

    const int st = tid - 256, sw = wid - 4;
    const int qa = st & 7, ra = st >> 3;
    int aih[AQ], aiw[AQ], apb[AQ];
    int bsrc[BQ], bk8[BQ], bdst[BQ];
    const __amdgpu_buffer_rsrc_t ar = __builtin_amdgcn_make_buffer_rsrc((void*)a.a, 0, a.a_elems * 4, 0x00020000);
    const __amdgpu_buffer_rsrc_t br = __builtin_amdgcn_make_buffer_rsrc((void*)a.b, 0, a.b_elems * 2, 0x00020000);
    if (!mfma_wave) {
#pragma unroll
        for (int j = 0; j < AQ; ++j) {
            const int m = m0 + ra + (NP / 8) * j;
            if (m < a.M) {
                const int b = m / (a.Ho * a.Wo), rem = m - b * a.Ho * a.Wo;
                const int oh = rem / a.Wo, ow = rem - oh * a.Wo;
                aih[j] = oh * a.stride - a.pad;
                aiw[j] = ow * a.stride - a.pad;
                apb[j] = ((b * a.H + aih[j]) * a.W + aiw[j]) * a.C + 4 * qa;
            } else {
                aih[j] = -(1 << 20);
                aiw[j] = 0;
                apb[j] = 0;
            }
        }
#pragma unroll
        for (int j = 0; j < BQ; ++j) {
            const int piece = sw + 4 * j, pl = piece / (BN / 16), rb = piece - pl * (BN / 16);
            const int r = rb * 16 + (lane >> 2), q = ((lane & 3) ^ (r >> 2)) & 3;
            const int n = n0 + r;
            bk8[j] = 8 * q;
            bsrc[j] = n < a.N ? ((pl * a.N + n) * KT) * a.C + 8 * q : -1;
            bdst[j] = (3 * PA + pl * PB + rb * 16 * XBK) * 2;
        }
    }
// ... 44 lines not shown
#pragma unroll
            for (int e = 0; e < 16; ++e) acc[i][jn][e] = 0.f;
    auto mma = [&](int buf) {
        const __bf16* L = lds[buf];
#pragma unroll
        for (int s2 = 0; s2 < XBK / 16; ++s2) {
            bf16x8 fb[TNc][3];
#pragma unroll
            for (int jn = 0; jn < TNc; ++jn) {
                const int eb = xidx(wn * 64 + 32 * jn + lr, 16 * s2 + 8 * h);
#pragma unroll
                for (int pl = 0; pl < 3; ++pl) fb[jn][pl] = *(const bf16x8*)(L + 3 * PA + pl * PB + eb);
            }
#pragma unroll
            for (int i = 0; i < TMc; ++i) {
                bf16x8 fa[3];
                const int e = xidx(wm * (BMX / 2) + 32 * i + lr, 16 * s2 + 8 * h);
#pragma unroll
                for (int pl = 0; pl < 3; ++pl) fa[pl] = *(const bf16x8*)(L + pl * PA + e);
#pragma unroll
                for (int jn = 0; jn < TNc; ++jn) {
                    acc[i][jn] = __builtin_amdgcn_mfma_f32_32x32x16_bf16(fa[2], fb[jn][0], acc[i][jn], 0, 0, 0);
                    acc[i][jn] = __builtin_amdgcn_mfma_f32_32x32x16_bf16(fa[1], fb[jn][1], acc[i][jn], 0, 0, 0);
                    acc[i][jn] = __builtin_amdgcn_mfma_f32_32x32x16_bf16(fa[0], fb[jn][2], acc[i][jn], 0, 0, 0);
                    acc[i][jn] = __builtin_amdgcn_mfma_f32_32x32x16_bf16(fa[1], fb[jn][0], acc[i][jn], 0, 0, 0);
                    acc[i][jn] = __builtin_amdgcn_mfma_f32_32x32x16_bf16(fa[0], fb[jn][1], acc[i][jn], 0, 0, 0);
                    acc[i][jn] = __builtin_amdgcn_mfma_f32_32x32x16_bf16(fa[0], fb[jn][0], acc[i][jn], 0, 0, 0);
                }
            }
        }
    };

    if (!mfma_wave) {
        load(0);
        dma(0, 0);
        wait_vm<BQ>();
        split_store(0);
        load(1);
        wait_vm<AQ>();
    }
    lds_sync();
    for (int t = 0; t < nchunks; ++t) {
        if (mfma_wave) {
            mma(t & 1);
        } else if (t + 1 < nchunks) {
            dma(t + 1, (t + 1) & 1);
            wait_vm<BQ>();
            split_store((t + 1) & 1);
            load(t + 2);
            wait_vm<AQ>();
        }
        lds_sync();
    }
    if (!mfma_wave) return;

    float* out = a.y + (size_t)ks * a.M * a.N;
#pragma unroll
    for (int jn = 0; jn < TNc; ++jn) {
        const int n = n0 + wn * 64 + 32 * jn + lr;
        if (n >= a.N) continue;
#pragma unroll
        for (int i = 0; i < TMc; ++i)
#pragma unroll
            for (int e = 0; e < 16; ++e) {
                const int m = m0 + wm * (BMX / 2) + 32 * i + (e & 3) + 8 * (e >> 2) + 4 * h;
                if (m < a.M) out[(size_t)m * a.N + n] = acc[i][jn][e];
            }
    }
}

__device__ __forceinline__ int pidx16(int pix, int pr, int pc, int k) {
    const int sw = (pr & 1) ^ (((pc >> 2) & 1) << 1);
    return pix * XBK + ((((k >> 3) ^ sw) & 3) << 3) + (k & 7);
}

template <int BN, int BMX, int TC, bool BF = false>
__global__ __launch_bounds__((X6Geo<BN, BMX>::NT), 1) void conv_x6p_kernel(ConvArgs a) {
    using G = X6Geo<BN, BMX>;
    static_assert(G::MT == 32, "patch kernel: 32x32x16 MFMA tiles");
    constexpr int NT = G::NT, TM = G::TM;
    constexpr int NP = BF ? 1 : 3;
    constexpr int TR = BMX / TC, PW = TC + 2, PH = TR + 2, PP = PH * PW;
    constexpr int AQP = (PP * 8 + NT - 1) / NT;
    constexpr int NW = NT / 64, PIECES = NP * BN / 16;
    constexpr int BQ = (PIECES + NW - 1) / NW;
    constexpr int PA = PP * XBK, PB = BN * XBK;
    constexpr int TPS = BF ? 3 : 1, NGR = 9 / TPS;
    __shared__ __bf16 lds[NP * PA + 2 * TPS * NP * PB];

    const int tid = threadIdx.x, lane = tid & 63, wid = tid >> 6;
    const int wm = wid / G::WN, wn = wid % G::WN;
    int blk = xcd_contiguous_block(blockIdx.x, gridDim.x);
    const int nb = blk % a.nblocks;
    blk /= a.nblocks;
    const int mb = blk % a.mblocks, ks = blk / a.mblocks;
    const int per_img = a.ptr * a.ptc;
    const int b = mb / per_img, trc = mb - b * per_img, tr = trc / a.ptc, tc = trc - tr * a.ptc;
    const int oh0 = tr * TR, ow0 = tc * TC, n0 = nb * BN;
    const int t0 = ks * a.chunks_per_split;
    const int nchunks = min(a.chunks_per_split, a.nchunks - t0);
    constexpr int KT = 9;

    int aofs[AQP];
    const __amdgpu_buffer_rsrc_t ar =
        __builtin_amdgcn_make_buffer_rsrc((void*)a.a, 0, a.a_elems * (BF ? 2 : 4), 0x00020000);
#pragma unroll
    for (int j = 0; j < AQP; ++j) {
        const int f = tid + NT * j, pix = f >> 3, q = f & 7;
        const int pr = pix / PW, pc = pix - pr * PW;
        const int ih = oh0 + pr - a.pad, iw = ow0 + pc - a.pad;
        const bool ok = f < PP * 8 && (unsigned)ih < (unsigned)a.H && (unsigned)iw < (unsigned)a.W;
        aofs[j] = ok ? ((b * a.H + ih) * a.W + iw) * a.C + 4 * q : -1;
    }
    constexpr int RB16 = BN / 16;
    int bsrc[BQ], bk8[BQ], bdst[BQ];
    const __amdgpu_buffer_rsrc_t br = __builtin_amdgcn_make_buffer_rsrc((void*)a.b, 0, a.b_elems * 2, 0x00020000);
#pragma unroll
    for (int j = 0; j < BQ; ++j) {
        const int piece = wid + NW * j, pl = piece / RB16, rb = piece - pl * RB16;
        const int r = rb * 16 + (lane >> 2), q = ((lane & 3) ^ (r >> 2)) & 3;
        const int n = n0 + r;
        bk8[j] = 8 * q;
        bsrc[j] = n < a.N ? ((pl * a.N + n) * KT) * a.C + 8 * q : -1;
        bdst[j] = (NP * PA + pl * PB + rb * 16 * XBK) * 2;
    }
    f32x16 acc[TM];
#pragma unroll
    for (int i = 0; i < TM; ++i)
#pragma unroll
// ... 65 lines not shown
            for (int pl = 0; pl < NP; ++pl) fb[pl] = *(const bf16x8*)(LB + pl * PB + eb);
#pragma unroll
            for (int i = 0; i < TM; ++i) {
                bf16x8 fa[NP];
                const int e = TC == 16 ? pidx16(abase[i] + toff, arow[i] + th, acol[i] + tw, 16 * s + 8 * h)
                                       : xidx(abase[i] + toff, 16 * s + 8 * h);
#pragma unroll
                for (int pl = 0; pl < NP; ++pl) fa[pl] = *(const bf16x8*)(lds + pl * PA + e);
                if constexpr (BF) {
                    acc[i] = __builtin_amdgcn_mfma_f32_32x32x16_bf16(fa[0], fb[0], acc[i], 0, 0, 0);
                    continue;
                } else {
                acc[i] = __builtin_amdgcn_mfma_f32_32x32x16_bf16(fa[2], fb[0], acc[i], 0, 0, 0);
                acc[i] = __builtin_amdgcn_mfma_f32_32x32x16_bf16(fa[1], fb[1], acc[i], 0, 0, 0);
                acc[i] = __builtin_amdgcn_mfma_f32_32x32x16_bf16(fa[0], fb[2], acc[i], 0, 0, 0);
                acc[i] = __builtin_amdgcn_mfma_f32_32x32x16_bf16(fa[1], fb[0], acc[i], 0, 0, 0);
                acc[i] = __builtin_amdgcn_mfma_f32_32x32x16_bf16(fa[0], fb[1], acc[i], 0, 0, 0);
                acc[i] = __builtin_amdgcn_mfma_f32_32x32x16_bf16(fa[0], fb[0], acc[i], 0, 0, 0);
                }
            }
        }
    };

    if (NT == 512 && wid >= 4) __builtin_amdgcn_s_setprio(1);
    if (nchunks > 0) {
        load(0);
        dma_group(0, 0, 0);
        store_patch();
        wait_vm<0>();
        lds_sync();
    }
    int buf = 0;
    for (int t = 0; t < nchunks; ++t) {
        for (int g = 0; g < NGR; ++g) {
            const bool more = g + 1 < NGR || t + 1 < nchunks;
            if (more) dma_group(g + 1 < NGR ? t : t + 1, g + 1 < NGR ? g + 1 : 0, buf ^ 1);
            if (g == 0 && t + 1 < nchunks) load(t + 1);
#pragma unroll
            for (int u = 0; u < TPS; ++u) mma(buf * TPS + u, g * TPS + u);
            asm volatile("" ::: "memory");
            if (g == 0 && t + 1 < nchunks) wait_vm<AQP>();
            else wait_vm<0>();
            lds_sync();
            buf ^= 1;
        }
        if (t + 1 < nchunks) {
            store_patch();
            lds_sync();
        }
    }

    float* out = a.y + (size_t)ks * a.M * a.N;
    const int n = n0 + wn * 32 + lr;
    if (n < a.N) {
#pragma unroll
        for (int i = 0; i < TM; ++i)
#pragma unroll
            for (int e = 0; e < 16; ++e) {
                const int ml = wm * (TM * 32) + 32 * i + (e & 3) + 8 * (e >> 2) + 4 * h;
                const int r = ml / TC, c = ml - r * TC, oh = oh0 + r, ow = ow0 + c;
                if (oh < a.Ho && ow < a.Wo) {
                    const size_t o = ((size_t)(b * a.Ho + oh) * a.Wo + ow) * a.N + n;
                    if (BF && a.ybf16 == 1 && a.splits == 1) ((uint16_t*)a.y)[o] = f2bf16(acc[i][e]);
                    else out[o] = acc[i][e];
                }
            }
    }
}

template <int BMW, bool XFAST, bool BF = false>
__global__ __launch_bounds__(512, (BMW == 64 ? 2 : 1)) void conv_x6_wgrad_kernel(ConvArgs a) {
    constexpr int NT = 512, BNW = 128, TM = BMW / 64;
    constexpr int NP = BF ? 1 : 3;
    constexpr int PA = BMW * XBK, PB = BNW * XBK;
    static_assert(BMW == 64 || BMW == 128, "wgrad row tile");
    __shared__ __bf16 lds[2][NP * (PA + PB)];
    const int tid = threadIdx.x, lane = tid & 63, wid = tid >> 6;
    const int wm = wid >> 2, wn = wid & 3;
    int blk = xcd_contiguous_block(blockIdx.x, gridDim.x);
    const int nb = blk % a.nblocks;
    blk /= a.nblocks;
    const int mb = blk % a.mblocks, ks = blk / a.mblocks;
    const int m0 = mb * BMW, n0 = nb * BNW;
    const int t0 = ks * a.chunks_per_split;
    const int nchunks = min(a.chunks_per_split, a.nchunks - t0);
    const int HoWo = a.Ho * a.Wo;
    const float rHoWo = 1.0f / (float)HoWo, rWo = 1.0f / (float)a.Wo;

    const int side = tid >> 8, u = tid & 255, kq = u & 7, mq = u >> 3;
    const int row = 4 * mq;
    const bool stager = side == 1 || u < 2 * BMW;
    int ci = 0, kh = 0, kw = 0;
    bool rok;
    if (side == 0) {
        rok = stager && m0 + row < a.M;
    } else {
        const int n = n0 + row;
        rok = n < a.N;
        const int tap = n / a.C;
        ci = n - tap * a.C;
        kh = tap / a.KW;
        kw = tap - kh * a.KW;
    }
    constexpr int ES = BF ? 2 : 4;
    const __amdgpu_buffer_rsrc_t xr = __builtin_amdgcn_make_buffer_rsrc((void*)a.a, 0, a.a_elems * ES, 0x00020000);
    const __amdgpu_buffer_rsrc_t gr = __builtin_amdgcn_make_buffer_rsrc((void*)a.b, 0, a.b_elems * ES, 0x00020000);
// ... 894 lines not shown

constexpr int kRedOut = 64, kRedLanes = 256 / kRedOut;
template <int OUT, int OM = 0>
__global__ __launch_bounds__(256) void conv_reduce_kernel(const float4* part, float4* y, int n4, int splits) {
    constexpr int LANES = 256 / OUT;
    __shared__ float4 red[LANES][OUT];
    const int o = threadIdx.x % OUT, l = threadIdx.x / OUT;
    const int i = blockIdx.x * OUT + o;
    float4 s = {0.f, 0.f, 0.f, 0.f};
    if (i < n4) {
#pragma unroll 4
        for (int k = l; k < splits; k += LANES) {
            const float4 v = part[(size_t)k * n4 + i];
            s.x += v.x;
            s.y += v.y;
            s.z += v.z;
            s.w += v.w;
        }
    }
    red[l][o] = s;
    __syncthreads();
    if (l == 0 && i < n4) {
#pragma unroll
        for (int j = 1; j < LANES; ++j) {
            const float4 v = red[j][o];
            s.x += v.x;
            s.y += v.y;
            s.z += v.z;
            s.w += v.w;
        }
        if constexpr (OM == 1) {
            ((uint2*)y)[i] = make_uint2((uint32_t)f2bf16(s.x) | ((uint32_t)f2bf16(s.y) << 16),
                                        (uint32_t)f2bf16(s.z) | ((uint32_t)f2bf16(s.w) << 16));
        } else if constexpr (OM == 2) {
            y[i] = make_float4(bf16_round(s.x), bf16_round(s.y), bf16_round(s.z), bf16_round(s.w));
        } else {
            y[i] = s;
        }
    }
}

template <int OM>
void launch_reduce_om(const float4* part, float4* y, int n4, int splits, hipStream_t st) {
    if (splits >= 16 && (n4 + kRedOut - 1) / kRedOut < 512)
        hipLaunchKernelGGL((conv_reduce_kernel<16, OM>), dim3((n4 + 15) / 16), dim3(256), 0, st, part, y, n4, splits);
    else
        hipLaunchKernelGGL((conv_reduce_kernel<kRedOut, OM>), dim3((n4 + kRedOut - 1) / kRedOut), dim3(256), 0, st,
                           part, y, n4, splits);
}
void launch_reduce(const float4* part, float4* y, int n4, int splits, hipStream_t st, int om = 0) {
    if (om == 1) launch_reduce_om<1>(part, y, n4, splits, st);
    else if (om == 2) launch_reduce_om<2>(part, y, n4, splits, st);
    else launch_reduce_om<0>(part, y, n4, splits, st);
}

template <int OM = 0>
__global__ __launch_bounds__(256) void conv_reduce_scatter_kernel(const float4* part, float4* y, int n4, int splits,
                                                                   int N4, int Hc, int Wc, int oHf, int oWf, int py,
                                                                   int px) {
    __shared__ float4 red[kRedLanes][kRedOut];
    const int o = threadIdx.x % kRedOut, l = threadIdx.x / kRedOut;
    const int i = blockIdx.x * kRedOut + o;
    float4 s = {0.f, 0.f, 0.f, 0.f};
    if (i < n4) {
        for (int k = l; k < splits; k += kRedLanes) {
            const float4 v = part[(size_t)k * n4 + i];
            s.x += v.x;
            s.y += v.y;
            s.z += v.z;
            s.w += v.w;
        }
    }
    red[l][o] = s;
    __syncthreads();
    if (l == 0 && i < n4) {
#pragma unroll
        for (int j = 1; j < kRedLanes; ++j) {
            const float4 v = red[j][o];
            s.x += v.x;
            s.y += v.y;
            s.z += v.z;
            s.w += v.w;
        }
        const int m = i / N4, q = i - m * N4, hw = Hc * Wc, b = m / hw, rem = m - b * hw, oh = rem / Wc,
                  ow = rem - oh * Wc;
        const size_t o = ((size_t)(b * oHf + 2 * oh + py) * oWf + 2 * ow + px) * N4 + q;
        if constexpr (OM == 1)
            ((uint2*)y)[o] = make_uint2((uint32_t)f2bf16(s.x) | ((uint32_t)f2bf16(s.y) << 16),
                                        (uint32_t)f2bf16(s.z) | ((uint32_t)f2bf16(s.w) << 16));
        else
            y[o] = s;
    }
}

bool valid(const md2_conv_desc* d) {
    if (!d) return false;
    if (d->batch < 1 || d->height < 1 || d->width < 1) return false;
    if (d->in_channels < 4 || d->in_channels % 4 || d->out_channels < 4 || d->out_channels % 4) return false;
    if (d->kernel_h < 1 || d->kernel_w < 1 || d->stride < 1 || d->pad < 0) return false;
    if (d->pad >= d->kernel_h || d->pad >= d->kernel_w) return false;
    const long long ho = (d->height + 2ll * d->pad - d->kernel_h) / d->stride + 1;
    const long long wo = (d->width + 2ll * d->pad - d->kernel_w) / d->stride + 1;
    if (ho < 1 || wo < 1) return false;
    if ((long long)d->batch * d->height * d->width * d->in_channels >= (1ll << 29)) return false;
    if ((long long)d->batch * ho * wo * d->out_channels >= (1ll << 29)) return false;
    if ((long long)d->out_channels * d->kernel_h * d->kernel_w * d->in_channels >= (1ll << 29)) return false;
// ... 81 lines not shown
        a.Cg = s.N;
        a.N = s.N;
        a.P = s.B * s.Ho * s.Wo;
        a.nchunks = (a.P + BK - 1) / BK;
        a.a_elems = s.B * s.H * s.W * s.C;
        a.b_elems = s.B * s.Ho * s.Wo * s.N;
    }
    return a;
}

int resident_blocks_x6(int BN, int BMX) { return 256 * ((BN <= 64 && BMX == 128) || BMX == 64 ? 2 : 1); }

double split_launch_cost() {
    static const double c = [] {
        const char* e = getenv("MD2_X6_SPLIT_COST");
        return e ? atof(e) : 0.0;
    }();
    return c;
}

void plan_x6(ConvArgs& a, uint32_t flags, bool wgrad = false) {
    const bool w256 = wgrad && a.M > 64 && (flags & MD2_CONV_WS) && (flags & MD2_CONV_BM256);
    const int BN = wgrad ? (w256 ? 256 : 128) : (a.N <= 16 ? 16 : (a.N <= 32 ? 32 : (a.N <= 64 ? 64 : 128)));
    const int BMX = wgrad ? (a.M <= 64 ? 64 : 128) : ((BN == 128 && (flags & MD2_CONV_BM256)) ? 256 : 128);
    const int mblocks = (a.M + BMX - 1) / BMX, nblocks = (a.N + BN - 1) / BN;
    const int base = mblocks * nblocks, res = resident_blocks_x6(BN, BMX);
    int best_s = 1;
    double best_t = 1e30;
    const int smin = w256 ? (a.nchunks + 63) / 64 : 1;
    const int smax = std::max(smin, (flags & MD2_CONV_NO_SPLIT) ? 1 : (a.nchunks / 6 > 1 ? a.nchunks / 6 : 1));
    for (int sp = smin; sp <= smax && sp <= std::max(64, smin); ++sp) {
        const int per = (a.nchunks + sp - 1) / sp;
        const int splits = (a.nchunks + per - 1) / per;
        const int rounds = (base * splits + res - 1) / res;
        const double red = splits > 1 ? (double)(splits + 1) * a.M * a.N * 4.0 / 2400.0 / 1536.0 + split_launch_cost()
                                      : 0.0;
        const double t = (double)rounds * per * (BMX / 128.0) * (BN / 128 > 1 ? BN / 128 : 1) + red;
        if (t < best_t - 1e-9) {
            best_t = t;
            best_s = splits;
        }
    }
    a.bm = BMX;
    a.bn = BN;
    a.mblocks = mblocks;
    a.nblocks = nblocks;
    a.chunks_per_split = (a.nchunks + best_s - 1) / best_s;
    a.splits = (a.nchunks + a.chunks_per_split - 1) / a.chunks_per_split;
}

template <int MODE>
void launch(const ConvArgs& a, int BN, hipStream_t st) {
    const dim3 grid(a.mblocks * a.nblocks * a.splits);
    if (BN == 128)
        hipLaunchKernelGGL((conv_gemm_kernel<128, MODE>), grid, dim3(kThreads), 0, st, a);
    else if (BN == 64)
        hipLaunchKernelGGL((conv_gemm_kernel<64, MODE>), grid, dim3(kThreads), 0, st, a);
    else
        hipLaunchKernelGGL((conv_gemm_kernel<32, MODE>), grid, dim3(kThreads), 0, st, a);
}

int min_chunks_of(int mode) { return mode == MODE_WGRAD ? 8 : 6; }

bool use_x6(const md2_conv_desc* d, int mode) {
    if (d->flags & MD2_CONV_BF16) return false;
    if (!((d->flags & MD2_CONV_X6) && d->in_channels % 8 == 0 && d->out_channels % 8 == 0)) return false;
    if (mode == MODE_WGRAD) {
        const Shape s = shape_of(d);
        if ((long long)s.B * s.Ho * s.Wo + 64 >= (1ll << 24)) return false;
    }
    return true;
}

bool use_bf(const md2_conv_desc* d, int mode) {
    if (!(d->flags & MD2_CONV_BF16)) return false;
    if (mode == MODE_FWD) return d->in_channels % 8 == 0;
    if (mode == MODE_DGRAD) return d->stride == 1 && d->out_channels % 8 == 0;
    const Shape s = shape_of(d);
    return (long long)s.B * s.Ho * s.Wo + 64 < (1ll << 24);
}

bool use_bfp(const md2_conv_desc* d, int mode, const ConvArgs& a) {
    return (d->flags & MD2_CONV_PATCH) && use_bf(d, mode) && mode != MODE_WGRAD && a.KH == 3 && a.KW == 3 &&
           a.stride == 1 && a.C % XBK == 0 && a.N > 16 && !a.flatk;
}

bool use_bfpw(const md2_conv_desc* d) {
    return (d->flags & MD2_CONV_PATCH) && use_bf(d, MODE_WGRAD) && d->kernel_h == 3 && d->kernel_w == 3 &&
           d->stride == 1;
}

ConvArgs args_x6_wgrad(const md2_conv_desc* d) {
    const Shape s = shape_of(d);
    ConvArgs a = {};
    a.KH = s.KH;
    a.KW = s.KW;
    a.B = s.B; a.H = s.H; a.W = s.W; a.C = s.C;
    a.Ho = s.Ho; a.Wo = s.Wo; a.stride = s.s; a.pad = s.p;
    a.M = s.N;
    a.N = s.KH * s.KW * s.C;
    a.Cg = s.N;
    a.P = s.B * s.Ho * s.Wo;
    a.nchunks = (a.P + XBK - 1) / XBK;
    a.a_elems = s.B * s.H * s.W * s.C;
    a.b_elems = s.B * s.Ho * s.Wo * s.N;
    return a;
}

size_t x6_planes_bytes(const md2_conv_desc* d) {
    return (3 * sizeof(uint16_t) * (size_t)d->out_channels * d->kernel_h * d->kernel_w * d->in_channels + 255) &
           ~(size_t)255;
}

void flat_k(ConvArgs& a, int mode) {
    if (mode != MODE_WGRAD && a.C < XBK) {
        a.flatk = 1;
        a.nchunks = (a.KH * a.KW * a.C + XBK - 1) / XBK;
    }
}

void launch_bf(const ConvArgs& a, hipStream_t st) {
    const dim3 grid(a.mblocks * a.nblocks * a.splits);
    if (a.bm == 256) hipLaunchKernelGGL((conv_x6_kernel<128, 256, true>), grid, dim3(X6Geo<128, 256>::NT), 0, st, a);
    else if (a.bn == 128)
        hipLaunchKernelGGL((conv_x6_kernel<128, 128, true>), grid, dim3(X6Geo<128, 128>::NT), 0, st, a);
    else if (a.bn == 64) hipLaunchKernelGGL((conv_x6_kernel<64, 128, true>), grid, dim3(X6Geo<64, 128>::NT), 0, st, a);
    else if (a.bn == 32) hipLaunchKernelGGL((conv_x6_kernel<32, 128, true>), grid, dim3(X6Geo<32, 128>::NT), 0, st, a);
    else hipLaunchKernelGGL((conv_x6_kernel<16, 128, true>), grid, dim3(X6Geo<16, 128>::NT), 0, st, a);
}

void launch_x6(const ConvArgs& a, hipStream_t st, bool ws = false) {
    const dim3 grid(a.mblocks * a.nblocks * a.splits);
    if (ws && a.bn == 128 && !a.flatk && !a.par) {
        if (a.bm == 256) hipLaunchKernelGGL((conv_x6ws_kernel<256>), grid, dim3(512), 0, st, a);
        else hipLaunchKernelGGL((conv_x6ws_kernel<128>), grid, dim3(512), 0, st, a);
        return;
    }
    if (a.bm == 256) hipLaunchKernelGGL((conv_x6_kernel<128, 256>), grid, dim3(X6Geo<128, 256>::NT), 0, st, a);
    else if (a.bn == 128) hipLaunchKernelGGL((conv_x6_kernel<128, 128>), grid, dim3(X6Geo<128, 128>::NT), 0, st, a);
    else if (a.bn == 64) hipLaunchKernelGGL((conv_x6_kernel<64, 128>), grid, dim3(X6Geo<64, 128>::NT), 0, st, a);
    else if (a.bn == 32) hipLaunchKernelGGL((conv_x6_kernel<32, 128>), grid, dim3(X6Geo<32, 128>::NT), 0, st, a);
    else hipLaunchKernelGGL((conv_x6_kernel<16, 128>), grid, dim3(X6Geo<16, 128>::NT), 0, st, a);
}

bool use_x6p(const md2_conv_desc* d, int mode, const ConvArgs& a) {
    return (d->flags & MD2_CONV_PATCH) && use_x6(d, mode) && mode != MODE_WGRAD && a.KH == 3 && a.KW == 3 &&
           a.stride == 1 && a.C % XBK == 0 && a.N > 16 && !a.flatk;
}

void plan_x6p(ConvArgs& a, uint32_t flags) {
    const int BN = a.N <= 32 ? 32 : (a.N <= 64 ? 64 : 128);
    const int BMX = (BN == 128 && (flags & MD2_CONV_BM256)) ? 256 : 128;
    int best_tc = 64;
    long long best_cost = -1;
    for (int TC = 64; TC >= 16; TC /= 2) {
        const int TR = BMX / TC;
        const long long area = (long long)((a.Ho + TR - 1) / TR) * TR * ((a.Wo + TC - 1) / TC) * TC;
        const long long cost = area * 4096 + (TR + 2) * (TC + 2);
        if (best_cost < 0 || cost < best_cost) {
            best_cost = cost;
            best_tc = TC;
        }
    }
    const int TR = BMX / best_tc;
    a.ptr = (a.Ho + TR - 1) / TR;
    a.ptc = (a.Wo + best_tc - 1) / best_tc;
    a.nchunks = a.C / XBK;
    const int mblocks = a.B * a.ptr * a.ptc, nblocks = (a.N + BN - 1) / BN;
    const int base = mblocks * nblocks, res = BN == 128 ? 256 : 512;
    int best_s = 1;
    double best_t = 1e30;
    const int smax = (flags & MD2_CONV_NO_SPLIT) ? 1 : a.nchunks;
    for (int sp = 1; sp <= smax && sp <= 64; ++sp) {
        const int per = (a.nchunks + sp - 1) / sp;
        const int splits = (a.nchunks + per - 1) / per;
        const int rounds = (base * splits + res - 1) / res;
        const double red = splits > 1 ? (double)(splits + 1) * a.M * a.N * 4.0 / 2400.0 / 1536.0 + split_launch_cost()
                                      : 0.0;
        const double t = (double)rounds * per * 9.0 * (BMX / 128.0) + red;
        if (t < best_t - 1e-9) {
            best_t = t;
            best_s = splits;
        }
    }
    a.bm = BMX;
    a.bn = BN;
    a.mblocks = mblocks;
    a.nblocks = nblocks;
    a.chunks_per_split = (a.nchunks + best_s - 1) / best_s;
    a.splits = (a.nchunks + a.chunks_per_split - 1) / a.chunks_per_split;
    a.flatk = best_tc;
}

template <int BN, int BMX, bool BF = false>
void launch_x6p_tc(const ConvArgs& a, hipStream_t st) {
    const dim3 grid(a.mblocks * a.nblocks * a.splits), block(X6Geo<BN, BMX>::NT);
    ConvArgs b = a;
    b.flatk = 0;
    if (a.flatk == 64) hipLaunchKernelGGL((conv_x6p_kernel<BN, BMX, 64, BF>), grid, block, 0, st, b);
    else if (a.flatk == 32) hipLaunchKernelGGL((conv_x6p_kernel<BN, BMX, 32, BF>), grid, block, 0, st, b);
    else hipLaunchKernelGGL((conv_x6p_kernel<BN, BMX, 16, BF>), grid, block, 0, st, b);
}

template <bool BF = false>
void launch_x6p(const ConvArgs& a, hipStream_t st) {
    if (a.bm == 256) launch_x6p_tc<128, 256, BF>(a, st);
    else if (a.bn == 128) launch_x6p_tc<128, 128, BF>(a, st);
    else if (a.bn == 64) launch_x6p_tc<64, 128, BF>(a, st);
    else launch_x6p_tc<32, 128, BF>(a, st);
}

bool use_x6pw(const md2_conv_desc* d) {
    return (d->flags & MD2_CONV_PATCH) && use_x6(d, MODE_WGRAD) && d->kernel_h == 3 && d->kernel_w == 3 &&
           d->stride == 1;
}

constexpr int kX6pwMaxChunks = 64;

void plan_x6pw(ConvArgs& a, uint32_t flags) {
    const int BMW = a.M <= 32 ? 32 : 64;
    a.ptc = (a.Wo + 31) / 32;
    a.nchunks = a.B * a.Ho * a.ptc;
    const int smin = (a.nchunks + kX6pwMaxChunks - 1) / kX6pwMaxChunks;
    const int mblocks = (a.M + BMW - 1) / BMW, nblocks = (a.C + XBK - 1) / XBK;
    const int base = mblocks * nblocks, res = 256;
    int best_s = 1;
    double best_t = 1e30;
    const int smax = std::max(1, a.nchunks / 4);
    for (int k = 0; k <= 8; ++k) {
        const int sp = std::max(smin, std::min(smax, k == 0 ? 1 : std::max(1, k * res / base)));
        const int per = (a.nchunks + sp - 1) / sp;
        const int splits = (a.nchunks + per - 1) / per;
        const int rounds = (base * splits + res - 1) / res;
        const double red = splits > 1 ? (double)(splits + 1) * a.M * a.N * 4.0 / 2400.0 / 1700.0 + split_launch_cost()
                                      : 0.0;
        const double t = (double)rounds * per + red;
        if (t < best_t - 1e-9) {
            best_t = t;
            best_s = splits;
        }
    }
    a.bm = BMW;
    a.mblocks = mblocks;
    a.nblocks = nblocks;
    a.chunks_per_split = (a.nchunks + best_s - 1) / best_s;
    a.splits = (a.nchunks + a.chunks_per_split - 1) / a.chunks_per_split;
}

bool dgrad_s2_class(const md2_conv_desc* d, int py, int px, ConvArgs& a, uint32_t extra_flags = 0) {
    const Shape s = shape_of(d);
    a = ConvArgs{};
// ... 153 lines not shown
                if (j >= Wo) continue;
                const float4 v = cols[(((size_t)(b * Ho + i) * Wo + j) * (KH * KW) + kh * KW + kw) * Q + q];
                acc.x += v.x;
                acc.y += v.y;
                acc.z += v.z;
                acc.w += v.w;
            }
        }
        gx[t] = acc;
    }
}

int run_bf(const md2_conv_desc* d, int mode, const void* A, const void* B, void* out, void* ws, void* stream,
           const char* name) {
    if (!use_bf(d, mode))
        return md2_report_error(MD2_ERR_ARG, "conv bf16: fwd in_channels % 8; dgrad stride 1, out_channels % 8; "
                                             "wgrad fewer than 2^24 output pixels");
    ConvArgs a = mode == MODE_WGRAD ? args_x6_wgrad(d) : args_of(d, mode);
    const bool pw = mode == MODE_WGRAD && use_bfpw(d);
    flat_k(a, mode);
    const bool patch = use_bfp(d, mode, a);
    if (pw) plan_x6pw(a, d->flags);
    else if (patch) plan_x6p(a, d->flags);
    else plan_x6(a, d->flags, mode == MODE_WGRAD);
    a.a = (const float*)A;
    a.b = (const float*)B;
    a.ybf16 = mode == MODE_WGRAD ? 2 : 1;
    if (mode != MODE_WGRAD) a.b_elems = d->out_channels * d->kernel_h * d->kernel_w * d->in_channels;
    if (a.splits > 1 && !ws) return md2_report_error(MD2_ERR_ARG, name);
    a.y = a.splits > 1 ? (float*)ws : (float*)out;
    const hipStream_t st = (hipStream_t)stream;
    if (pw) {
        const dim3 grid(a.mblocks * a.nblocks * a.splits);
        if (a.bm == 64) hipLaunchKernelGGL((conv_x6pw_kernel<64, true>), grid, dim3(576), 0, st, a);
        else hipLaunchKernelGGL((conv_x6pw_kernel<32, true>), grid, dim3(576), 0, st, a);
    } else if (mode == MODE_WGRAD) {
        const dim3 grid(a.mblocks * a.nblocks * a.splits);
        const bool xf = (a.Wo & 3) == 0;
        void (*k)(ConvArgs) = a.bm == 64
                                  ? (xf ? conv_x6_wgrad_kernel<64, true, true> : conv_x6_wgrad_kernel<64, false, true>)
                                  : (xf ? conv_x6_wgrad_kernel<128, true, true> : conv_x6_wgrad_kernel<128, false, true>);
        if (a.bn == 256) k = xf ? conv_x6wws256_kernel<true, true> : conv_x6wws256_kernel<false, true>;
        hipLaunchKernelGGL(k, grid, dim3(512), 0, st, a);
    } else if (patch) {
        launch_x6p<true>(a, st);
    } else {
        launch_bf(a, st);
    }
    if (a.splits > 1) launch_reduce((const float4*)a.y, (float4*)out, a.M * a.N / 4, a.splits, st, a.ybf16);
    const hipError_t e = hipGetLastError();
    return e == hipSuccess ? MD2_OK : md2_report_error(MD2_ERR_HIP, hipGetErrorString(e));
}

int run(const md2_conv_desc* d, int mode, const float* A, const float* B, float* out, void* ws, void* stream,
        const char* name) {
    if (d->flags & MD2_CONV_BF16) return run_bf(d, mode, A, B, out, ws, stream, name);
    ConvArgs a = (mode == MODE_WGRAD && use_x6(d, mode)) ? args_x6_wgrad(d) : args_of(d, mode);
    if (use_x6(d, mode)) flat_k(a, mode);
    const bool patch = use_x6p(d, mode, a);
    const bool patch_w = mode == MODE_WGRAD && use_x6pw(d);
    if (patch) plan_x6p(a, d->flags);
    else if (patch_w) plan_x6pw(a, d->flags);
    else if (use_x6(d, mode)) plan_x6(a, d->flags, mode == MODE_WGRAD);
    else plan(a, d->flags, min_chunks_of(mode));
    const int BN = a.bn;
    a.a = A;
    a.b = B;
    if ((a.splits > 1 || (use_x6(d, mode) && mode != MODE_WGRAD)) && !ws) return md2_report_error(MD2_ERR_ARG, name);
    a.y = a.splits > 1 ? (float*)ws : out;
    const hipStream_t st = (hipStream_t)stream;
    if (patch_w) {
        const dim3 grid(a.mblocks * a.nblocks * a.splits);
        if (a.bm == 64) hipLaunchKernelGGL(conv_x6pw_kernel<64>, grid, dim3(576), 0, st, a);
        else hipLaunchKernelGGL(conv_x6pw_kernel<32>, grid, dim3(576), 0, st, a);
    } else if (use_x6(d, mode) && mode == MODE_WGRAD) {
        const dim3 grid(a.mblocks * a.nblocks * a.splits);
        const bool xf = (a.Wo & 3) == 0;
        void (*k)(ConvArgs) = a.bm == 64 ? (xf ? conv_x6_wgrad_kernel<64, true> : conv_x6_wgrad_kernel<64, false>)
                                         : (xf ? conv_x6_wgrad_kernel<128, true> : conv_x6_wgrad_kernel<128, false>);
        if (a.bm == 128 && (d->flags & MD2_CONV_WS))
            k = xf ? conv_x6wws_kernel<true> : conv_x6wws_kernel<false>;
        if (a.bn == 256) k = xf ? conv_x6wws256_kernel<true> : conv_x6wws256_kernel<false>;
        hipLaunchKernelGGL(k, grid, dim3(512), 0, st, a);
    } else if (use_x6(d, mode)) {
        __bf16* planes = (d->flags & MD2_CONV_PRESPLIT) ? (__bf16*)B : (__bf16*)ws;
        a.b = (const float*)planes;
        a.b_elems = 3 * d->out_channels * d->kernel_h * d->kernel_w * d->in_channels;
        if (a.splits > 1) a.y = (float*)((char*)ws + x6_planes_bytes(d));
        const int nw = a.b_elems / 3;
        if (!(d->flags & MD2_CONV_PRESPLIT))
            hipLaunchKernelGGL(conv_wsplit_kernel, dim3((nw + 255) / 256), dim3(256), 0, st, B, planes,
                               d->out_channels, d->kernel_h * d->kernel_w, d->in_channels, mode == MODE_DGRAD ? 1 : 0);
        if (patch) launch_x6p(a, st);
        else launch_x6(a, st, (d->flags & MD2_CONV_WS) != 0);
    } else if (mode == MODE_FWD) launch<MODE_FWD>(a, BN, st);
    else if (mode == MODE_DGRAD) launch<MODE_DGRAD>(a, BN, st);
    else launch<MODE_WGRAD>(a, BN, st);
    if (a.splits > 1) {
        const int n4 = a.M * a.N / 4;
        launch_reduce((const float4*)a.y, (float4*)out, n4, a.splits, st);
    }
    const hipError_t e = hipGetLastError();
    return e == hipSuccess ? MD2_OK : md2_report_error(MD2_ERR_HIP, hipGetErrorString(e));
}

size_t ws_bytes(const md2_conv_desc* d, int mode) {
    if (d->flags & MD2_CONV_BF16) {
        if (mode == MODE_DGRAD && use_bf_s2(d)) {
            size_t part = 0;
            for (int py = 0; py < 2; ++py)
                for (int px = 0; px < 2; ++px) {
                    ConvArgs c;
                    if (dgrad_s2_class(d, py, px, c) && c.splits > 1)
                        part = std::max(part, sizeof(float) * (size_t)c.splits * c.M * c.N);
                }
            return part;
        }
        if (!use_bf(d, mode)) return 0;
        ConvArgs a = mode == MODE_WGRAD ? args_x6_wgrad(d) : args_of(d, mode);
        flat_k(a, mode);
        if (mode == MODE_WGRAD && use_bfpw(d)) plan_x6pw(a, d->flags);
        else if (use_bfp(d, mode, a)) plan_x6p(a, d->flags);
        else plan_x6(a, d->flags, mode == MODE_WGRAD);
        return a.splits > 1 ? sizeof(float) * (size_t)a.splits * a.M * a.N : 0;
    }
    if (mode == MODE_DGRAD && use_x6_s2(d)) {
        size_t part = 0;
        for (int py = 0; py < 2; ++py)
            for (int px = 0; px < 2; ++px) {
                ConvArgs c;
                if (dgrad_s2_class(d, py, px, c) && c.splits > 1)
                    part = std::max(part, sizeof(float) * (size_t)c.splits * c.M * c.N);
            }
        return x6_planes_bytes(d) + part;
    }
    ConvArgs a = (mode == MODE_WGRAD && use_x6(d, mode)) ? args_x6_wgrad(d) : args_of(d, mode);
    if (mode == MODE_WGRAD && use_x6pw(d)) {
        plan_x6pw(a, d->flags);
        return a.splits > 1 ? sizeof(float) * (size_t)a.splits * a.M * a.N : 0;
    }
    if (use_x6(d, mode) && mode == MODE_WGRAD) {
        plan_x6(a, d->flags, true);
        return a.splits > 1 ? sizeof(float) * (size_t)a.splits * a.M * a.N : 0;
    }
    if (use_x6(d, mode)) {
        flat_k(a, mode);
        if (use_x6p(d, mode, a)) plan_x6p(a, d->flags);
        else plan_x6(a, d->flags);
        return x6_planes_bytes(d) + (a.splits > 1 ? sizeof(float) * (size_t)a.splits * a.M * a.N : 0);
    }
    plan(a, d->flags, min_chunks_of(mode));
    return a.splits > 1 ? sizeof(float) * (size_t)a.splits * a.M * a.N : 0;
}
// ... 2 lines not shown

extern "C" {

size_t md2_conv_workspace_bytes(const md2_conv_desc* d) {
    if (!valid(d)) return 0;
    size_t m = ws_bytes(d, MODE_FWD);
    if (d->stride == 1 || use_x6_s2(d) || use_bf_s2(d)) m = m > ws_bytes(d, MODE_DGRAD) ? m : ws_bytes(d, MODE_DGRAD);
    const size_t w = ws_bytes(d, MODE_WGRAD);
    return m > w ? m : w;
}

int md2_conv_split_weights(const md2_conv_desc* d, const float* weight, void* planes_fwd, void* planes_dgrad,
                           void* stream) {
    if (!valid(d) || d->in_channels % 8 || d->out_channels % 8)
        return md2_report_error(MD2_ERR_ARG, "conv_split_weights: channels % 8, pad < kernel, sizes < 2^29");
    if (!weight || !planes_fwd) return md2_report_error(MD2_ERR_ARG, "conv_split_weights: NULL operand");
    const dim3 grid((d->in_channels + 31) / 32, (d->out_channels + 31) / 32, d->kernel_h * d->kernel_w);
    hipLaunchKernelGGL(conv_wsplit_tile_kernel, grid, dim3(256), 0, (hipStream_t)stream, weight,
                       (__bf16*)planes_fwd, (__bf16*)planes_dgrad, d->out_channels, d->kernel_h * d->kernel_w,
                       d->in_channels);
    const hipError_t e = hipGetLastError();
    return e == hipSuccess ? MD2_OK : md2_report_error(MD2_ERR_HIP, hipGetErrorString(e));
}

int md2_conv_bf16_weights(const md2_conv_desc* d, const float* weight, void* w_fwd, void* w_dgrad, void* stream) {
    if (!valid(d)) return md2_report_error(MD2_ERR_ARG, "conv_bf16_weights: channels % 4, pad < kernel, sizes < 2^29");
    if (!weight || !w_fwd) return md2_report_error(MD2_ERR_ARG, "conv_bf16_weights: NULL operand");
    const dim3 grid((d->in_channels + 31) / 32, (d->out_channels + 31) / 32, d->kernel_h * d->kernel_w);
    hipLaunchKernelGGL(conv_wsplit_tile_kernel, grid, dim3(256), 0, (hipStream_t)stream, weight, (__bf16*)w_fwd,
                       (__bf16*)w_dgrad, d->out_channels, d->kernel_h * d->kernel_w, d->in_channels, 1);
    const hipError_t e = hipGetLastError();
    return e == hipSuccess ? MD2_OK : md2_report_error(MD2_ERR_HIP, hipGetErrorString(e));
}

int md2_conv_bf16_weights_multi(const md2_wsplit_entry* table, int n, int total_blocks, void* stream) {
    if (!table || n <= 0 || total_blocks <= 0) return md2_report_error(MD2_ERR_ARG, "conv_bf16_weights_multi: empty");
    hipLaunchKernelGGL(conv_wsplit_multi_kernel, dim3(total_blocks), dim3(256), 0, (hipStream_t)stream, table, n, 1);
    const hipError_t e = hipGetLastError();
    return e == hipSuccess ? MD2_OK : md2_report_error(MD2_ERR_HIP, hipGetErrorString(e));
}

int md2_conv_split_weights_multi(const md2_wsplit_entry* table, int n, int total_blocks, void* stream) {
    if (!table || n <= 0 || total_blocks <= 0) return md2_report_error(MD2_ERR_ARG, "conv_split_weights_multi: empty");
    hipLaunchKernelGGL(conv_wsplit_multi_kernel, dim3(total_blocks), dim3(256), 0, (hipStream_t)stream, table, n);
    const hipError_t e = hipGetLastError();
    return e == hipSuccess ? MD2_OK : md2_report_error(MD2_ERR_HIP, hipGetErrorString(e));
}

int md2_conv_fwd(const md2_conv_desc* d, const float* x, const float* weight, float* y, void* workspace,
                 void* stream) {
    if (!valid(d)) return md2_report_error(MD2_ERR_ARG, "conv_fwd: channels % 4, pad < kernel, sizes < 2^29");
    if (!x || !weight || !y) return md2_report_error(MD2_ERR_ARG, "conv_fwd: NULL operand");
    return run(d, MODE_FWD, x, weight, y, workspace, stream, "conv_fwd: workspace required (K split)");
}

int md2_conv_dgrad(const md2_conv_desc* d, const float* grad_y, const float* weight, float* grad_x,
                   void* workspace, void* stream) {
    if (!valid(d) || (d->stride != 1 && !use_x6_s2(d) && !use_bf_s2(d)))
        return md2_report_error(MD2_ERR_ARG, "conv_dgrad: stride 1 (stride 2: MD2_CONV_X6, channels % 8, >= 32 "
                                             "output channels), channels % 4, pad < kernel, sizes < 2^29");
    if (!grad_y || !weight || !grad_x) return md2_report_error(MD2_ERR_ARG, "conv_dgrad: NULL operand");
    if (d->stride == 2) return run_dgrad_s2(d, grad_y, weight, grad_x, workspace, stream);
    return run(d, MODE_DGRAD, grad_y, weight, grad_x, workspace, stream, "conv_dgrad: workspace required (K split)");
}

int md2_conv_wgrad(const md2_conv_desc* d, const float* x, const float* grad_y, float* grad_weight,
                   void* workspace, void* stream) {
    if (!valid(d)) return md2_report_error(MD2_ERR_ARG, "conv_wgrad: channels % 4, pad < kernel, sizes < 2^29");
    if (!x || !grad_y || !grad_weight) return md2_report_error(MD2_ERR_ARG, "conv_wgrad: NULL operand");
    return run(d, MODE_WGRAD, x, grad_y, grad_weight, workspace, stream, "conv_wgrad: workspace required (K split)");
}

int md2_conv_col2im(const md2_conv_desc* d, const float* cols, float* grad_x, void* stream) {
    if (!d || !cols || !grad_x) return md2_report_error(MD2_ERR_ARG, "conv_col2im: NULL operand");
    if (d->in_channels % 4 || d->stride < 1 || d->pad < 0 || d->kernel_h < 1 || d->kernel_w < 1 || d->batch < 1 ||
        d->height < 1 || d->width < 1)
        return md2_report_error(MD2_ERR_ARG, "conv_col2im: channels % 4, stride >= 1, pad >= 0");
    const int Ho = (d->height + 2 * d->pad - d->kernel_h) / d->stride + 1;
    const int Wo = (d->width + 2 * d->pad - d->kernel_w) / d->stride + 1;
    if (Ho < 1 || Wo < 1) return md2_report_error(MD2_ERR_ARG, "conv_col2im: empty output");
    const int Q = d->in_channels / 4;
    const long long n = (long long)d->batch * d->height * d->width * Q;
    const long long blocks = (n + 255) / 256;
    hipLaunchKernelGGL(conv_col2im_kernel, dim3((unsigned)(blocks < 8192 ? blocks : 8192)), dim3(256), 0,
                       (hipStream_t)stream, (const float4*)cols, (float4*)grad_x, d->batch, d->height, d->width, Q,
                       Ho, Wo, d->kernel_h, d->kernel_w, d->stride, d->pad);
    const hipError_t e = hipGetLastError();
    return e == hipSuccess ? MD2_OK : md2_report_error(MD2_ERR_HIP, hipGetErrorString(e));
}

}
```

monodepth2_amd/networks/resnet_encoder.py:

```python
from __future__ import annotations

import warnings

import numpy as np
import torch
import torch.nn as nn

from ..bn_ops import bn_act, max_pool_3x3s2, max_pool_3x3s2_with_alias
from ..conv_ops import conv2d
from ..stem_ops import stem_conv


def _conv3x3(cin, cout, stride=1):
    return nn.Conv2d(cin, cout, 3, stride=stride, padding=1, bias=False)


def _conv1x1(cin, cout, stride=1):
    return nn.Conv2d(cin, cout, 1, stride=stride, bias=False)


class BasicBlock(nn.Module):
    expansion = 1

    def __init__(self, inplanes, planes, stride=1, downsample=None):
        super().__init__()
        self.conv1 = _conv3x3(inplanes, planes, stride)
        self.bn1 = nn.BatchNorm2d(planes)
        self.relu = nn.ReLU(inplace=True)
        self.conv2 = _conv3x3(planes, planes)
        self.bn2 = nn.BatchNorm2d(planes)
        self.downsample = downsample
        self.stride = stride

    def forward(self, x):
        identity = x if self.downsample is None else _downsample(self.downsample, x)
        out = bn_act(self.bn1, self.conv1(x))
        return bn_act(self.bn2, self.conv2(out), residual=identity)


def _downsample(down: nn.Sequential, x):
    return bn_act(down[1], conv2d(down[0], x), relu=False)


class Bottleneck(nn.Module):
    expansion = 4

    def __init__(self, inplanes, planes, stride=1, downsample=None):
        super().__init__()
        self.conv1 = _conv1x1(inplanes, planes)
        self.bn1 = nn.BatchNorm2d(planes)
        self.conv2 = _conv3x3(planes, planes, stride)
        self.bn2 = nn.BatchNorm2d(planes)
        self.conv3 = _conv1x1(planes, planes * 4)
        self.bn3 = nn.BatchNorm2d(planes * 4)
        self.relu = nn.ReLU(inplace=True)
        self.downsample = downsample
        self.stride = stride

    def forward(self, x):
        identity = x if self.downsample is None else _downsample(self.downsample, x)
        out = bn_act(self.bn1, self.conv1(x))
        out = bn_act(self.bn2, self.conv2(out))
        return bn_act(self.bn3, self.conv3(out), residual=identity)


def _run_layer(layer: nn.Sequential, x, xs, skip_alias: bool):
    n = len(layer)
    skip = None
    for bi, blk in enumerate(layer):
        shortcut = xs if blk.downsample is None else _downsample(blk.downsample, xs)
        out = bn_act(blk.bn1, conv2d(blk.conv1, x))
        if isinstance(blk, Bottleneck):
            out = bn_act(blk.bn2, conv2d(blk.conv2, out))
            bn, conv = blk.bn3, blk.conv3
        else:
            bn, conv = blk.bn2, blk.conv2
        last = bi == n - 1
        k = (2 if skip_alias else 1) if last else 1
        res = bn_act(bn, conv2d(conv, out), residual=shortcut, aliases=k)
        x, xs = res[0], res[1]
        skip = res[2] if (last and skip_alias) else x
    return x, xs, skip


_SPECS = {18: (BasicBlock, [2, 2, 2, 2]), 34: (BasicBlock, [3, 4, 6, 3]), 50: (Bottleneck, [3, 4, 6, 3]),
          101: (Bottleneck, [3, 4, 23, 3]), 152: (Bottleneck, [3, 8, 36, 3])}


class ResNet(nn.Module):

    def __init__(self, num_layers=18, in_channels=3, num_classes=1000):
        super().__init__()
        block, counts = _SPECS[num_layers]
        self.inplanes = 64
        self.conv1 = nn.Conv2d(in_channels, 64, kernel_size=7, stride=2, padding=3, bias=False)
        self.bn1 = nn.BatchNorm2d(64)
        self.relu = nn.ReLU(inplace=True)
        self.maxpool = nn.MaxPool2d(kernel_size=3, stride=2, padding=1)
        self.layer1 = self._stage(block, 64, counts[0])
        self.layer2 = self._stage(block, 128, counts[1], stride=2)
        self.layer3 = self._stage(block, 256, counts[2], stride=2)
        self.layer4 = self._stage(block, 512, counts[3], stride=2)
        self.avgpool = nn.AdaptiveAvgPool2d((1, 1))
        self.fc = nn.Linear(512 * block.expansion, num_classes)
        for m in self.modules():
            if isinstance(m, nn.Conv2d):
                nn.init.kaiming_normal_(m.weight, mode="fan_out", nonlinearity="relu")
            elif isinstance(m, nn.BatchNorm2d):
                nn.init.constant_(m.weight, 1)
                nn.init.constant_(m.bias, 0)

    def _stage(self, block, planes, n, stride=1):
        down = None
        if stride != 1 or self.inplanes != planes * block.expansion:
            down = nn.Sequential(_conv1x1(self.inplanes, planes * block.expansion, stride),
                                 nn.BatchNorm2d(planes * block.expansion))
        blocks = [block(self.inplanes, planes, stride, down)]
        self.inplanes = planes * block.expansion
        blocks += [block(self.inplanes, planes) for _ in range(1, n)]
        return nn.Sequential(*blocks)


class ResnetEncoder(nn.Module):

    def __init__(self, num_layers, pretrained, num_input_images=1):
        super().__init__()
        if num_layers not in _SPECS:
            raise ValueError("{} is not a valid number of resnet layers".format(num_layers))
        if num_input_images > 1 and num_layers not in (18, 50):
            raise AssertionError("Can only run with 18 or 50 layer resnet")
        if pretrained:
            warnings.warn("ImageNet weights need network access and are unavailable offline; "
# ... 46 lines not shown
```

Baseline: 1124 images/s.

## Fuse BatchNorm statistics partial sums into conv forward epilogue

Conv forward kernels, and the split-K reduce kernel, now write per-block channel sum and sum-of-squares partials into the BN workspace. BN forward can then skip its own statistics pass over the conv output and start from these partials through md2_bn_fwd_given. The aim is to remove one full read of each encoder conv activation in the forward pass. In exchange it adds epilogue work and LDS reductions inside the conv kernels, and it only applies to shapes where bnstats_rows is nonzero.

```diff
diff --git a/include/md2hot.h b/include/md2hot.h
--- a/include/md2hot.h
+++ b/include/md2hot.h
@@ -212,7 +212,7 @@
     uint32_t flags;
     float eps, momentum;
     int32_t groups;
-    int32_t reserved;
+    int32_t stat_rows;
 } md2_bn_desc;
 
 size_t md2_bn_workspace_bytes(const md2_bn_desc* desc);
@@ -234,6 +234,9 @@
                     const void* grad_y2, const void* grad_y3, const float* gamma, const float* save_mean,
                     const float* save_invstd, void* grad_x, void* grad_residual, float* grad_gamma,
                     float* grad_beta, void* workspace, void* stream);
+int md2_bn_fwd_given(const md2_bn_desc* desc, int rows, const void* x, const float* gamma, const float* beta,
+                     const void* residual, float* running_mean, float* running_var, void* y, uint8_t* relu_mask,
+                     float* save_mean, float* save_invstd, void* workspace, void* stream);
 
 #define MD2_POOL_BF16 (1u << 0)
 
@@ -283,6 +286,9 @@
 int md2_conv_split_weights_multi(const md2_wsplit_entry* table, int n, int total_blocks, void* stream);
 int md2_conv_bf16_weights(const md2_conv_desc* desc, const float* weight, void* w_fwd, void* w_dgrad, void* stream);
 int md2_conv_bf16_weights_multi(const md2_wsplit_entry* table, int n, int total_blocks, void* stream);
+int md2_conv_bnstats_rows(const md2_conv_desc* desc, int bn_groups);
+int md2_conv_fwd_bnstats(const md2_conv_desc* desc, const float* x, const float* weight, float* y,
+                         void* workspace, void* bn_workspace, int bn_groups, void* stream);
 int md2_conv_fwd(const md2_conv_desc* desc, const float* x, const float* weight, float* y, void* workspace,
                  void* stream);
 int md2_conv_dgrad(const md2_conv_desc* desc, const float* grad_y, const float* weight, float* grad_x,
diff --git a/monodepth2_amd/_lib.py b/monodepth2_amd/_lib.py
--- a/monodepth2_amd/_lib.py
+++ b/monodepth2_amd/_lib.py
@@ -62,7 +62,8 @@
            "md2_conv_wgrad_direct_workspace_bytes", "md2_conv_split_weights_multi", "md2_bn_fwd_mask",
            "md2_bn_bwd_mask", "md2_build_id", "md2_maxpool3s2_bwd_multi", "md2_decoder_pad_bwd2", "md2_aug_run2",
            "md2_conv_bf16_weights", "md2_conv_bf16_weights_multi",
-           "md2_depth_eval", "md2_depth_eval_workspace_bytes"]
+           "md2_depth_eval", "md2_depth_eval_workspace_bytes",
+           "md2_bn_fwd_given", "md2_conv_bnstats_rows", "md2_conv_fwd_bnstats"]
 
 DTYPE_F32 = 0
 DTYPE_BF16 = 1
@@ -97,7 +98,7 @@
 class BnDesc(ctypes.Structure):
     _fields_ = [("pixels", ctypes.c_int64), ("channels", ctypes.c_int32), ("flags", ctypes.c_uint32),
                 ("eps", ctypes.c_float), ("momentum", ctypes.c_float), ("groups", ctypes.c_int32),
-                ("reserved", ctypes.c_int32)]
+                ("stat_rows", ctypes.c_int32)]
 
 
 POOL_BF16 = 1 << 0
@@ -292,6 +293,12 @@
     L.md2_bn_bwd_multi.argtypes = [ctypes.POINTER(BnDesc)] + [_vp] * 14
     L.md2_bn_fwd_mask.restype = ctypes.c_int
     L.md2_bn_fwd_mask.argtypes = [ctypes.POINTER(BnDesc)] + [_vp] * 12
+    L.md2_bn_fwd_given.restype = ctypes.c_int
+    L.md2_bn_fwd_given.argtypes = [ctypes.POINTER(BnDesc), ctypes.c_int] + [_vp] * 12
+    L.md2_conv_bnstats_rows.restype = ctypes.c_int
+    L.md2_conv_bnstats_rows.argtypes = [ctypes.POINTER(ConvDesc), ctypes.c_int]
+    L.md2_conv_fwd_bnstats.restype = ctypes.c_int
+    L.md2_conv_fwd_bnstats.argtypes = [ctypes.POINTER(ConvDesc)] + [_vp] * 5 + [ctypes.c_int, _vp]
     L.md2_bn_bwd_mask.restype = ctypes.c_int
     L.md2_bn_bwd_mask.argtypes = [ctypes.POINTER(BnDesc)] + [_vp] * 14
     L.md2_maxpool3s2_bwd_add.restype = ctypes.c_int
diff --git a/monodepth2_amd/bn_ops.py b/monodepth2_amd/bn_ops.py
--- a/monodepth2_amd/bn_ops.py
+++ b/monodepth2_amd/bn_ops.py
@@ -9,10 +9,11 @@
 import torch.nn as nn
 import torch.nn.functional as F
 
-from . import _lib
+from . import _lib, conv_ops
 
 ENABLED = True
 _GROUPS = 1
+CONV_STATS = os.environ.get("MD2_CONV_BNSTATS", "1") != "0"
 
 
 @contextlib.contextmanager
@@ -47,7 +48,7 @@
 def _desc(key: tuple):
     hit = _descs.get(key)
     if hit is None:
-        d = _lib.BnDesc(*key, 0)
+        d = _lib.BnDesc(*key)
         hit = _descs[key] = (d, _lib.lib().md2_bn_workspace_bytes(ctypes.byref(d)))
     return hit
 
@@ -61,11 +62,11 @@
 
     @staticmethod
     def forward(ctx, x, weight, bias, running_mean, running_var, residual, relu: bool, eps: float,
-                momentum: float, groups: int, aliases: int = 0):
+                momentum: float, groups: int, aliases: int = 0, given_rows: int = 0):
         B, C, H, W = x.shape
         flags = ((_lib.BN_RELU if relu else 0) | (_lib.BN_RESIDUAL if residual is not None else 0)
                  | (_lib.BN_BF16 if x.dtype == torch.bfloat16 else 0))
-        key = (B * H * W, C, flags, eps, momentum, groups)
+        key = (B * H * W, C, flags, eps, momentum, groups, given_rows)
         d, nbytes = _desc(key)
         L = _lib.lib()
         ws = _workspace(x.device, nbytes)
@@ -74,13 +75,16 @@
         mean, invstd = stats[0], stats[1]
         mask = torch.empty(x.numel() // 4, dtype=torch.uint8, device=x.device) if relu else None
         stream = _lib.stream(x.device)
-        rc = L.md2_bn_fwd_mask(ctypes.byref(d), x.data_ptr(), weight.data_ptr(), bias.data_ptr(),
-                               residual.data_ptr() if residual is not None else None,
-                               running_mean.data_ptr() if running_mean is not None else None,
-                               running_var.data_ptr() if running_var is not None else None,
-                               y.data_ptr(), mask.data_ptr() if mask is not None else None,
-                               mean.data_ptr(), invstd.data_ptr(), ws.data_ptr(), stream)
-        _lib.check(rc, "md2_bn_fwd_mask")
+        args = (x.data_ptr(), weight.data_ptr(), bias.data_ptr(),
+                residual.data_ptr() if residual is not None else None,
+                running_mean.data_ptr() if running_mean is not None else None,
+                running_var.data_ptr() if running_var is not None else None,
+                y.data_ptr(), mask.data_ptr() if mask is not None else None,
+                mean.data_ptr(), invstd.data_ptr(), ws.data_ptr(), stream)
+        if given_rows:
+            _lib.check(L.md2_bn_fwd_given(ctypes.byref(d), given_rows, *args), "md2_bn_fwd_given")
+        else:
+            _lib.check(L.md2_bn_fwd_mask(ctypes.byref(d), *args), "md2_bn_fwd_mask")
         ctx.save_for_backward(x, mask, weight, mean, invstd)
         ctx.desc = key
         ctx.has_res = residual is not None
@@ -94,7 +98,7 @@
         x, mask, weight, mean, invstd = ctx.saved_tensors
         gs = [g.to(x.dtype).contiguous(memory_format=_CL) for g in grads if g is not None]
         if not gs:
-            return (None,) * 11
+            return (None,) * 12
         gy = gs[0]
         d, nbytes = _desc(ctx.desc)
         L = _lib.lib()
@@ -112,28 +116,32 @@
                  gr.data_ptr() if gr is not None else None, gw.data_ptr(), gb.data_ptr(), ws.data_ptr(),
                  _lib.stream(x.device))
         _lib.check(rc, name)
-        return gx, gw, gb, None, None, gr, None, None, None, None, None
+        return gx, gw, gb, None, None, gr, None, None, None, None, None, None
+
+
+def _fused(bn: nn.BatchNorm2d, x: torch.Tensor, residual: Optional[torch.Tensor], groups: int) -> bool:
+    return (ENABLED and bn.training and x.is_cuda and x.dtype in (torch.float32, torch.bfloat16) and x.dim() == 4
+            and bn.affine and bn.track_running_stats and bn.momentum is not None and _supported(x.shape[1])
+            and x.numel() // 4 // groups < 2 ** 31
+            and x.is_contiguous(memory_format=_CL) and x.shape[1] > 1
+            and (residual is None or residual.is_contiguous(memory_format=_CL)))
 
 
 def bn_act(bn: nn.BatchNorm2d, x: torch.Tensor, residual: Optional[torch.Tensor] = None,
-           relu: bool = True, aliases: int = 0):
+           relu: bool = True, aliases: int = 0, _given_rows: int = 0):
     if not 0 <= aliases <= 2:
         raise ValueError("bn_act: at most two aliases")
     groups = _GROUPS if bn.training else 1
     if groups > 1 and x.shape[0] % groups:
         raise ValueError(f"batch {x.shape[0]} does not split into {groups} BatchNorm groups")
-    if (ENABLED and bn.training and x.is_cuda and x.dtype in (torch.float32, torch.bfloat16) and x.dim() == 4
-            and bn.affine and bn.track_running_stats and bn.momentum is not None and _supported(x.shape[1])
-            and x.numel() // 4 // groups < 2 ** 31
-            and x.is_contiguous(memory_format=_CL) and x.shape[1] > 1
-            and (residual is None or residual.is_contiguous(memory_format=_CL))):
+    if _fused(bn, x, residual, groups):
         if residual is not None and residual.dtype != x.dtype:
             residual = residual.to(x.dtype)
         if bn.num_batches_tracked is not None:
             bn.num_batches_tracked.add_(groups)
         k = aliases if torch.is_grad_enabled() else 0
         out = _BNAct.apply(x, bn.weight, bn.bias, bn.running_mean, bn.running_var, residual, relu, bn.eps,
-                           bn.momentum, groups, k)
+                           bn.momentum, groups, k, _given_rows)
         if aliases and not k:
             return (out,) * (aliases + 1)
         return out
@@ -142,6 +150,28 @@
         y = y + residual
     y = F.relu(y) if relu else y
     return (y,) * (aliases + 1) if aliases else y
+
+
+def conv_bn_act(conv: nn.Conv2d, bn: nn.BatchNorm2d, x: torch.Tensor, residual: Optional[torch.Tensor] = None,
+                relu: bool = True, aliases: int = 0):
+    groups = _GROUPS if bn.training else 1
+    if not (CONV_STATS and ENABLED and bn.training and x.is_cuda and x.dtype == torch.float32 and x.dim() == 4
+            and x.shape[0] % groups == 0 and conv_ops.supports(conv, x)):
+        return bn_act(bn, conv_ops.conv2d(conv, x), residual, relu, aliases)
+    (B, _, H, W), s, p, k = x.shape, conv.stride[0], conv.padding[0], conv.kernel_size[0]
+    C = conv.out_channels
+    pixels = B * ((H + 2 * p - k) // s + 1) * ((W + 2 * p - k) // s + 1)
+    if not (bn.affine and bn.track_running_stats and bn.momentum is not None and _supported(C) and C > 1
+            and pixels * C // 4 // groups < 2 ** 31
+            and (residual is None or residual.is_contiguous(memory_format=_CL))):
+        return bn_act(bn, conv_ops.conv2d(conv, x), residual, relu, aliases)
+
+    def workspace(rows: int) -> int:
+        return _workspace(x.device, _desc((pixels, C, 0, bn.eps, bn.momentum, groups, rows))[1]).data_ptr()
+
+    stats = conv_ops.BnStats(groups, workspace)
+    y = conv_ops.conv2d(conv, x, stats)
+    return bn_act(bn, y, residual, relu, aliases, _given_rows=stats.rows)
 
 
 _ALIAS_SUM = os.environ.get("MD2_ALIAS_SUM", "1") != "0"
diff --git a/monodepth2_amd/build.py b/monodepth2_amd/build.py
--- a/monodepth2_amd/build.py
+++ b/monodepth2_amd/build.py
@@ -27,7 +27,7 @@
         return True
     t = os.path.getmtime(LIB_PATH)
     deps = [os.path.join(CSRC, s) for s in SOURCES] + [os.path.join(INCLUDE, "md2hot.h"),
-                                                       os.path.join(CSRC, "md2_bf16.h")]
+                                                       os.path.join(CSRC, "md2_bf16.h"), os.path.join(CSRC, "md2_bn_partials.h")]
     if any(os.path.getmtime(d) > t for d in deps):
         return True
     return built_id(LIB_PATH) != source_hash()
@@ -59,7 +59,7 @@
 def source_hash() -> str:
     h = hashlib.sha256()
     for path in [os.path.join(CSRC, s) for s in SOURCES] + [os.path.join(INCLUDE, "md2hot.h"),
-                                                          os.path.join(CSRC, "md2_bf16.h")]:
+                                                          os.path.join(CSRC, "md2_bf16.h"), os.path.join(CSRC, "md2_bn_partials.h")]:
         h.update(os.path.basename(path).encode())
         with open(path, "rb") as f:
             h.update(f.read())
diff --git a/monodepth2_amd/conv_ops.py b/monodepth2_amd/conv_ops.py
--- a/monodepth2_amd/conv_ops.py
+++ b/monodepth2_amd/conv_ops.py
@@ -80,12 +80,38 @@
     _lib.check(getattr(_lib.lib(), fn)(ctypes.byref(d), p0, p1, p2, ws.data_ptr(), _lib.stream(device)), fn)
 
 
-def _fwd(x, w, stride, pad, flags=0):
+class BnStats:
+
+    def __init__(self, groups: int, workspace):
+        self.groups, self.workspace, self.rows = groups, workspace, 0
+
+
+_stat_rows: Dict[tuple, int] = {}
+
+
+def _call_fwd(x, w, stride, pad, flags, p0, p1, p2, stats=None):
+    if stats is not None:
+        k = (tuple(x.shape), tuple(w.shape), stride, pad, flags, stats.groups)
+        rows = _stat_rows.get(k)
+        d, nbytes = _desc_ws(x, w, stride, pad, flags)
+        if rows is None:
+            rows = _stat_rows[k] = _lib.lib().md2_conv_bnstats_rows(ctypes.byref(d), stats.groups)
+        if rows > 0:
+            ws = _workspace(x.device, nbytes)
+            _lib.check(_lib.lib().md2_conv_fwd_bnstats(ctypes.byref(d), p0, p1, p2, ws.data_ptr(),
+                                                       stats.workspace(rows), stats.groups, _lib.stream(x.device)),
+                       "md2_conv_fwd_bnstats")
+            stats.rows = rows
+            return
+    _call("md2_conv_fwd", x, w, stride, pad, flags, p0, p1, p2, x.device)
+
+
+def _fwd(x, w, stride, pad, flags=0, stats=None):
     B, _, H, W = x.shape
     N, _, KH, KW = w.shape
     y = torch.empty(B, N, (H + 2 * pad - KH) // stride + 1, (W + 2 * pad - KW) // stride + 1, device=x.device,
                     memory_format=_CL)
-    _call("md2_conv_fwd", x, w, stride, pad, flags, x.data_ptr(), w.data_ptr(), y.data_ptr(), x.device)
+    _call_fwd(x, w, stride, pad, flags, x.data_ptr(), w.data_ptr(), y.data_ptr(), stats)
     return y
 
 
@@ -286,13 +312,12 @@
     return got[1] if got is not None else None
 
 
-def _fwd_planes(x, w, planes, stride, pad, flags):
+def _fwd_planes(x, w, planes, stride, pad, flags, stats=None):
     B, _, H, W = x.shape
     N, _, KH, KW = w.shape
     y = torch.empty(B, N, (H + 2 * pad - KH) // stride + 1, (W + 2 * pad - KW) // stride + 1, device=x.device,
                     memory_format=_CL)
-    _call("md2_conv_fwd", x, w, stride, pad, flags | PRESPLIT, x.data_ptr(), planes.data_ptr(), y.data_ptr(),
-          x.device)
+    _call_fwd(x, w, stride, pad, flags | PRESPLIT, x.data_ptr(), planes.data_ptr(), y.data_ptr(), stats)
     return y
 
 
@@ -511,7 +536,7 @@
 class _Conv(torch.autograd.Function):
 
     @staticmethod
-    def forward(ctx, x, weight, stride: int, pad: int):
+    def forward(ctx, x, weight, stride: int, pad: int, stats: "BnStats | None" = None):
         ctx.stride, ctx.pad = stride, pad
         ctx.key = (tuple(x.shape), tuple(weight.shape), stride, pad)
         x6 = _x6_ok(x, weight)
@@ -530,7 +555,9 @@
         planes_dg = None
         if x6 and i < len(xf):
             pf, planes_dg = _planes_for(x, weight, stride, pad, stride == 1 or _x6_s2_ok(x, weight, stride))
-            y = _fwd_planes(x, weight, pf, stride, pad, xf[i])
+            y = _fwd_planes(x, weight, pf, stride, pad, xf[i], stats)
+        elif stats is not None and i == len(xf):
+            y = _fwd(x, weight, stride, pad, 0, stats)
         else:
             y = cands[i]()
         ctx.save_for_backward(x, weight, planes_dg)
@@ -601,7 +628,7 @@
             gxm, gwm, _ = _miopen_bwd(gy, x, w, s, p, (mi_x, mi_w, False))
             gx = gxm if mi_x else gx
             gw = gwm if mi_w else gw
-        return gx, gw, None, None
+        return gx, gw, None, None, None
 
 
 BF16_ENABLED = os.environ.get("MD2_CONV_BF16", "1") != "0"
@@ -773,9 +800,9 @@
             and conv.padding_mode == "zeros" and k[0] == k[1] and s[0] == s[1] and p[0] == p[1] and p[0] < k[0])
 
 
-def conv2d(conv: nn.Conv2d, x: torch.Tensor) -> torch.Tensor:
+def conv2d(conv: nn.Conv2d, x: torch.Tensor, stats: "BnStats | None" = None) -> torch.Tensor:
     if supports(conv, x):
-        return _Conv.apply(x, conv.weight, conv.stride[0], conv.padding[0])
+        return _Conv.apply(x, conv.weight, conv.stride[0], conv.padding[0], stats)
     if _module_ok(conv) and _bf16_ok(x, conv.weight, conv.stride[0], conv.padding[0]):
         return conv2d_bf16(x, conv.weight, conv.stride[0], conv.padding[0])
     return conv(x)
diff --git a/monodepth2_amd/csrc/bnorm.hip b/monodepth2_amd/csrc/bnorm.hip
--- a/monodepth2_amd/csrc/bnorm.hip
+++ b/monodepth2_amd/csrc/bnorm.hip
@@ -5,40 +5,14 @@
 #include <stdlib.h>
 
 #include "md2_bf16.h"
+#include "md2_bn_partials.h"
 #include "md2hot.h"
 
 int md2_report_error(int code, const char* msg);
 
 namespace {
 
-constexpr int kThreads = 256;
-constexpr int kMaxBlocks = 1024;
-
-struct Map {
-    int Q;
-    int QPT;
-    int PPB;
-};
-
-__host__ __device__ inline Map make_map(int C) {
-    Map m;
-    m.Q = C / 4;
-    m.QPT = m.Q > kThreads ? m.Q / kThreads : 1;
-    m.PPB = m.Q >= kThreads ? 1 : kThreads / m.Q;
-    return m;
-}
-
-struct Work {
-    float* part;
-    float* coef;
-};
-
-__host__ __device__ __forceinline__ Work work(void* ws, int G, int C, int NG) {
-    Work w;
-    w.part = (float*)ws;
-    w.coef = w.part + 2 * (size_t)NG * G * C;
-    return w;
-}
+using namespace md2bn;
 
 __device__ __forceinline__ float4 ld4(const float* p) { return *(const float4*)p; }
 __device__ __forceinline__ void st4(float* p, float4 v) { *(float4*)p = v; }
@@ -47,31 +21,6 @@
 __device__ __forceinline__ float4 ldT(const void* p, size_t off) { return md2::ld4T<T>(p, off); }
 template <typename T>
 __device__ __forceinline__ void stT(void* p, size_t off, float4 v) { md2::st4T<T>(p, off, v); }
-
-__device__ void block_partials(float4 a, float4 b, int q, int pl, const Map& m, int C, int rows, int row, Work w,
-                               float4 (*lds)[kThreads]) {
-    lds[0][threadIdx.x] = a;
-    lds[1][threadIdx.x] = b;
-    __syncthreads();
-    for (int half = m.PPB / 2; half > 0; half /= 2) {
-        if (pl < half) {
-            const int o = threadIdx.x + half * m.Q;
-            const float4 u = lds[0][o], v = lds[1][o];
-            a.x += u.x; a.y += u.y; a.z += u.z; a.w += u.w;
-            b.x += v.x; b.y += v.y; b.z += v.z; b.w += v.w;
-            lds[0][threadIdx.x] = a;
-            lds[1][threadIdx.x] = b;
-        }
-        __syncthreads();
-    }
-    if (pl == 0) {
-        float* pa = w.part + (size_t)(4 * q) * rows + row;
-        float* pb = w.part + ((size_t)C + 4 * q) * rows + row;
-        pa[0] = a.x; pa[rows] = a.y; pa[2 * (size_t)rows] = a.z; pa[3 * (size_t)rows] = a.w;
-        pb[0] = b.x; pb[rows] = b.y; pb[2 * (size_t)rows] = b.z; pb[3 * (size_t)rows] = b.w;
-    }
-    __syncthreads();
-}
 
 template <typename T>
 __global__ void __launch_bounds__(kThreads) bn_stats_kernel(const void* __restrict__ x, long long P, int C, int G,
@@ -84,10 +33,7 @@
     for (int qq = 0; qq < m.QPT; ++qq) {
         const int q = (threadIdx.x % m.Q) + qq * kThreads, pl = threadIdx.x / m.Q;
         float4 s = {0.f, 0.f, 0.f, 0.f}, ss = {0.f, 0.f, 0.f, 0.f};
-        auto acc = [&](const float4 v) {
-            s.x += v.x; s.y += v.y; s.z += v.z; s.w += v.w;
-            ss.x += v.x * v.x; ss.y += v.y * v.y; ss.z += v.z * v.z; ss.w += v.w * v.w;
-        };
+        auto acc = [&](const float4 v) { stats_acc(s, ss, v); };
         const long long stride = (long long)G * m.PPB;
         long long p = (long long)blockIdx.x * m.PPB + pl;
         for (; p + 3 * stride < P; p += 4 * stride) {
@@ -547,13 +493,6 @@
     return on;
 }
 
-int blocks_for_stats(long long P, int C) {
-    const Map m = make_map(C);
-    const long long rows = (P + m.PPB - 1) / m.PPB;
-    const long long g = (rows + 7) / 8;
-    return (int)(g < 1 ? 1 : (g > kMaxBlocks ? kMaxBlocks : g));
-}
-
 int grid_elem(long long n4, int NG) {
     const long long cap = (4096 + NG - 1) / NG;
     const long long g = (n4 + kThreads - 1) / kThreads;
@@ -574,14 +513,16 @@
 template <typename T>
 void launch_fwd(const md2_bn_desc* d, const void* x, const float* gamma, const float* beta, const void* residual,
                 float* running_mean, float* running_var, void* y, float* save_mean, float* save_invstd,
-                void* workspace, hipStream_t st, uint8_t* mask = nullptr) {
+                void* workspace, hipStream_t st, uint8_t* mask = nullptr, int given_rows = 0) {
     const int NG = groups_of(d);
     const long long P = d->pixels / NG;
-    const int C = d->channels, G = blocks_for_stats(P, C);
-    if (sizeof(T) == 2 && C % 8 == 0 && C <= 8 * kThreads && reduce8_on())
-        hipLaunchKernelGGL(bn_stats8_kernel<>, dim3(G, NG), dim3(kThreads), 0, st, x, P, C, G, workspace);
-    else
-        hipLaunchKernelGGL(bn_stats_kernel<T>, dim3(G, NG), dim3(kThreads), 0, st, x, P, C, G, workspace);
+    const int C = d->channels, G = given_rows > 0 ? given_rows : blocks_for_stats(P, C);
+    if (given_rows <= 0) {
+        if (sizeof(T) == 2 && C % 8 == 0 && C <= 8 * kThreads && reduce8_on())
+            hipLaunchKernelGGL(bn_stats8_kernel<>, dim3(G, NG), dim3(kThreads), 0, st, x, P, C, G, workspace);
+        else
+            hipLaunchKernelGGL(bn_stats_kernel<T>, dim3(G, NG), dim3(kThreads), 0, st, x, P, C, G, workspace);
+    }
     hipLaunchKernelGGL(bn_stats_final_kernel, dim3(C), dim3(kThreads), 0, st, P, C, G, NG, d->eps, d->momentum,
                        running_mean, running_var, save_mean, save_invstd, workspace);
     const int n4g = (int)(P * C / 4);
@@ -643,8 +584,28 @@
 size_t md2_bn_workspace_bytes(const md2_bn_desc* d) {
     if (!valid(d)) return 0;
     const int NG = groups_of(d);
-    const int G = blocks_for_stats(d->pixels / NG, d->channels);
+    int G = blocks_for_stats(d->pixels / NG, d->channels);
+    if (d->stat_rows > G) G = d->stat_rows > kMaxBlocks ? kMaxBlocks : d->stat_rows;
     return (2 * (size_t)NG * G * d->channels + 3 * (size_t)NG * d->channels) * sizeof(float);
+}
+
+int md2_bn_fwd_given(const md2_bn_desc* d, int rows, const void* x, const float* gamma, const float* beta,
+                     const void* residual, float* running_mean, float* running_var, void* y, uint8_t* relu_mask,
+                     float* save_mean, float* save_invstd, void* workspace, void* stream) {
+    if (!valid(d)) return md2_report_error(MD2_ERR_ARG, "bn: need pixels >= 2 and channels a multiple of 4 "
+                                                        "with channels/4 dividing (or a multiple of) 256");
+    if (d->flags & MD2_BN_BF16) return md2_report_error(MD2_ERR_ARG, "bn_fwd_given: fp32 only");
+    if (rows < 1 || rows > kMaxBlocks)
+        return md2_report_error(MD2_ERR_ARG, "bn_fwd_given: rows per group in 1 .. 1024");
+    if (!x || !gamma || !beta || !y || !save_mean || !save_invstd || !workspace ||
+        ((d->flags & MD2_BN_RESIDUAL) && !residual) || (!running_mean != !running_var))
+        return md2_report_error(MD2_ERR_ARG, "bn_fwd_given: NULL operand");
+    if (relu_mask && !(d->flags & MD2_BN_RELU))
+        return md2_report_error(MD2_ERR_ARG, "bn_fwd_given: relu_mask without MD2_BN_RELU");
+    launch_fwd<float>(d, x, gamma, beta, residual, running_mean, running_var, y, save_mean, save_invstd, workspace,
+                      (hipStream_t)stream, relu_mask, rows);
+    const hipError_t e = hipGetLastError();
+    return e == hipSuccess ? MD2_OK : md2_report_error(MD2_ERR_HIP, hipGetErrorString(e));
 }
 
 int md2_bn_fwd_mask(const md2_bn_desc* d, const void* x, const float* gamma, const float* beta, const void* residual,
diff --git a/monodepth2_amd/csrc/conv.hip b/monodepth2_amd/csrc/conv.hip
--- a/monodepth2_amd/csrc/conv.hip
+++ b/monodepth2_amd/csrc/conv.hip
@@ -8,6 +8,7 @@
 #include <algorithm>
 #include <type_traits>
 
+#include "md2_bn_partials.h"
 #include "md2hot.h"
 
 int md2_report_error(int code, const char* msg);
@@ -46,12 +47,94 @@
     const float* b;
     float* y;
     int ybf16;
+    float* bn_part;
+    int bn_P, bn_rows, bn_NG;
 };
 
 __device__ __forceinline__ int xcd_contiguous_block(int bid, int n) {
     const int q = n >> 3, r = n & 7;
     const int xcd = bid & 7, idx = bid >> 3;
     return xcd < r ? xcd * (q + 1) + idx : r * (q + 1) + (xcd - r) * q + idx;
+}
+
+struct ColStat {
+    float s0, q0, s1, q1;
+};
+template <bool TWO>
+__device__ __forceinline__ void col_add(ColStat& c, float v, bool in0, bool in1) {
+    const float v0 = in0 ? v : 0.f;
+    c.s0 += v0;
+    c.q0 += v0 * v0;
+    if (TWO) {
+        const float v1 = in1 ? v : 0.f;
+        c.s1 += v1;
+        c.q1 += v1 * v1;
+    }
+}
+
+struct TileRows {
+    int row0, nz0, row1, nz1;
+    int lim0, bound;
+};
+
+__device__ __forceinline__ TileRows tile_rows(const ConvArgs& a, int mb, int m0, int BMX) {
+    TileRows t;
+    const int P = a.bn_P, R = a.bn_rows;
+    const int g0 = m0 / P;
+    t.bound = (g0 + 1) * P;
+    t.lim0 = min(t.bound, a.M);
+    const int idx0 = mb - (g0 * P) / BMX;
+    t.row0 = g0 * R + idx0;
+    t.nz0 = (t.lim0 - 1) / BMX == mb ? R - 1 - idx0 : 0;
+    t.row1 = -1;
+    t.nz1 = 0;
+    if (t.bound < min(m0 + BMX, a.M)) {
+        t.row1 = (g0 + 1) * R;
+        t.nz1 = (min(t.bound + P, a.M) - 1) / BMX == mb ? R - 1 : 0;
+    }
+    return t;
+}
+
+template <int NCOL, int WM, int BN>
+__device__ __forceinline__ void bn_rows_store(const ConvArgs& a, ColStat (&c)[NCOL], const int (&col)[NCOL], bool holds,
+                                              int wm, int h, int n0, const TileRows& t, void* scratch) {
+#pragma unroll
+    for (int j = 0; j < NCOL; ++j) {
+        c[j].s0 += __shfl_xor(c[j].s0, 32, 64);
+        c[j].q0 += __shfl_xor(c[j].q0, 32, 64);
+        c[j].s1 += __shfl_xor(c[j].s1, 32, 64);
+        c[j].q1 += __shfl_xor(c[j].q1, 32, 64);
+    }
+    float4* sc = (float4*)scratch;
+    __syncthreads();
+    if (holds && h == 0) {
+#pragma unroll
+        for (int j = 0; j < NCOL; ++j) sc[wm * BN + col[j]] = make_float4(c[j].s0, c[j].q0, c[j].s1, c[j].q1);
+    }
+    __syncthreads();
+    const int tid = threadIdx.x, n = n0 + tid;
+    if (tid < BN && n < a.N) {
+        float4 v = sc[tid];
+#pragma unroll
+        for (int w = 1; w < WM; ++w) {
+            const float4 u = sc[w * BN + tid];
+            v.x += u.x;
+            v.y += u.y;
+            v.z += u.z;
+            v.w += u.w;
+        }
+        const size_t rows = (size_t)a.bn_NG * a.bn_rows;
+        float* ps = a.bn_part + (size_t)n * rows;
+        float* pq = a.bn_part + ((size_t)a.N + n) * rows;
+        ps[t.row0] = v.x;
+        pq[t.row0] = v.y;
+        for (int z = 1; z <= t.nz0; ++z) ps[t.row0 + z] = pq[t.row0 + z] = 0.f;
+        if (t.row1 >= 0) {
+            ps[t.row1] = v.z;
+            pq[t.row1] = v.w;
+            for (int z = 1; z <= t.nz1; ++z) ps[t.row1 + z] = pq[t.row1 + z] = 0.f;
+        }
+    }
 }
 
 __device__ __forceinline__ float4 bload(__amdgpu_buffer_rsrc_t r, int byte_off) {
@@ -92,7 +175,7 @@
     static constexpr int A_FLOATS = BM * BK, B_FLOATS = BN * BK;
 };
 
-template <int BN, int MODE>
+template <int BN, int MODE, bool ST = false>
 __global__ __launch_bounds__(kThreads, BN == 128 ? 2 : (BN == 64 ? 3 : 4)) void conv_gemm_kernel(ConvArgs a) {
     using G = Cfg<BN, MODE>;
     constexpr int TM = G::TM, TN = G::TN, AQ = G::AQ, BQ = G::BQ;
@@ -299,6 +382,27 @@
 #undef CONV_MMA
 
     float* out = a.y + (size_t)ks * a.M * a.N;
+    if constexpr (ST) {
+        static_assert(MODE == MODE_FWD, "statistics epilogue: forward only");
+        const TileRows tr = tile_rows(a, mb, m0, BM);
+        ColStat c[TN] = {};
+        int col[TN];
+#pragma unroll
+        for (int j = 0; j < TN; ++j) {
+            col[j] = wn * (TN * 32) + 32 * j + (lane & 31);
+            const int n = n0 + col[j];
+#pragma unroll
+            for (int i = 0; i < TM; ++i)
+#pragma unroll
+                for (int e = 0; e < 16; ++e) {
+                    const int m = m0 + wm * (TM * 32) + 32 * i + (e & 3) + 8 * (e >> 2) + 4 * h;
+                    if (m < a.M && n < a.N) out[m * a.N + n] = acc[i][j][e];
+                    col_add<true>(c[j], acc[i][j][e], m < tr.lim0, m >= tr.bound && m < a.M);
+                }
+        }
+        bn_rows_store<TN, G::WAVES_M, BN>(a, c, col, true, wm, h, n0, tr, lds);
+        return;
+    }
 #pragma unroll
     for (int i = 0; i < TM; ++i)
 #pragma unroll
@@ -768,7 +872,7 @@
     }
 }
 
-template <int BMX>
+template <int BMX, bool ST = false>
 __global__ __launch_bounds__(512, 1) void conv_x6ws_kernel(ConvArgs a) {
     constexpr int BN = 128, NP = 256;
     constexpr int TMc = BMX / 64, TNc = 2;
@@ -919,6 +1023,28 @@
         }
         lds_sync();
     }
+    if constexpr (ST) {
+        float* out = a.y;
+        const TileRows tr = tile_rows(a, mb, m0, BMX);
+        ColStat c[TNc] = {};
+        int col[TNc];
+#pragma unroll
+        for (int jn = 0; jn < TNc; ++jn) {
+            col[jn] = wn * 64 + 32 * jn + lr;
+            const int n = n0 + col[jn];
+            if (!mfma_wave) continue;
+#pragma unroll
+            for (int i = 0; i < TMc; ++i)
+#pragma unroll
+                for (int e = 0; e < 16; ++e) {
+                    const int m = m0 + wm * (BMX / 2) + 32 * i + (e & 3) + 8 * (e >> 2) + 4 * h;
+                    if (m < a.M && n < a.N) out[(size_t)m * a.N + n] = acc[i][jn][e];
+                    col_add<true>(c[jn], acc[i][jn][e], m < tr.lim0, m >= tr.bound && m < a.M);
+                }
+        }
+        bn_rows_store<TNc, 2, BN>(a, c, col, mfma_wave, wm, h, n0, tr, lds);
+        return;
+    }
     if (!mfma_wave) return;
 
     float* out = a.y + (size_t)ks * a.M * a.N;
@@ -941,7 +1067,7 @@
     return pix * XBK + ((((k >> 3) ^ sw) & 3) << 3) + (k & 7);
 }
 
-template <int BN, int BMX, int TC, bool BF = false>
+template <int BN, int BMX, int TC, bool BF = false, bool ST = false>
 __global__ __launch_bounds__((X6Geo<BN, BMX>::NT), 1) void conv_x6p_kernel(ConvArgs a) {
     using G = X6Geo<BN, BMX>;
     static_assert(G::MT == 32, "patch kernel: 32x32x16 MFMA tiles");
@@ -1113,6 +1239,29 @@
 
     float* out = a.y + (size_t)ks * a.M * a.N;
     const int n = n0 + wn * 32 + lr;
+    if constexpr (ST) {
+        static_assert(!BF, "statistics epilogue: fp32 only");
+        ColStat cs[1] = {};
+        const int col[1] = {wn * 32 + lr};
+#pragma unroll
+        for (int i = 0; i < TM; ++i)
+#pragma unroll
+            for (int e = 0; e < 16; ++e) {
+                const int ml = wm * (TM * 32) + 32 * i + (e & 3) + 8 * (e >> 2) + 4 * h;
+                const int r = ml / TC, c = ml - r * TC, oh = oh0 + r, ow = ow0 + c;
+                const bool in = oh < a.Ho && ow < a.Wo;
+                if (in && n < a.N) out[((size_t)(b * a.Ho + oh) * a.Wo + ow) * a.N + n] = acc[i][e];
+                col_add<false>(cs[0], acc[i][e], in, false);
+            }
+        TileRows trw;
+        trw.row0 = mb;
+        trw.nz0 = 0;
+        trw.row1 = -1;
+        trw.nz1 = 0;
+        trw.lim0 = trw.bound = 0;
+        bn_rows_store<1, G::WM, BN>(a, cs, col, true, wm, h, n0, trw, lds);
+        return;
+    }
     if (n < a.N) {
 #pragma unroll
         for (int i = 0; i < TM; ++i)
@@ -2113,6 +2262,70 @@
     if (om == 1) launch_reduce_om<1>(part, y, n4, splits, st);
     else if (om == 2) launch_reduce_om<2>(part, y, n4, splits, st);
     else launch_reduce_om<0>(part, y, n4, splits, st);
+}
+
+template <int LANES>
+__global__ __launch_bounds__(md2bn::kThreads) void conv_reduce_stats_kernel(const float4* __restrict__ part,
+                                                                            float4* __restrict__ y, int n4,
+                                                                            int splits, long long P, int C, int G,
+                                                                            void* bn_ws) {
+    const md2bn::Map m = md2bn::make_map(C);
+    const int NG = gridDim.y, grp = blockIdx.y;
+    const md2bn::Work w = md2bn::work(bn_ws, G, C, NG);
+    __shared__ float4 lds[2][md2bn::kThreads];
+    auto add = [](float4& s, const float4 v) {
+        s.x += v.x;
+        s.y += v.y;
+        s.z += v.z;
+        s.w += v.w;
+    };
+    constexpr int U = LANES <= 4 ? 4 : 1;
+    for (int qq = 0; qq < m.QPT; ++qq) {
+        const int q = (threadIdx.x % m.Q) + qq * md2bn::kThreads, pl = threadIdx.x / m.Q;
+        float4 s = {0.f, 0.f, 0.f, 0.f}, ss = {0.f, 0.f, 0.f, 0.f};
+        const long long stride = (long long)G * m.PPB;
+        auto pixels = [&](long long p, auto nu) {
+            constexpr int NU = decltype(nu)::value;
+            size_t i[NU];
+            float4 c[NU][LANES];
+#pragma unroll
+            for (int u = 0; u < NU; ++u) {
+                i[u] = (size_t)(grp * P + p + u * stride) * m.Q + q;
+#pragma unroll
+                for (int l = 0; l < LANES; ++l) c[u][l] = make_float4(0.f, 0.f, 0.f, 0.f);
+            }
+            int k = 0;
+            for (; k + LANES <= splits; k += LANES) {
+                float4 v[NU][LANES];
+#pragma unroll
+                for (int u = 0; u < NU; ++u)
+#pragma unroll
+                    for (int l = 0; l < LANES; ++l) v[u][l] = part[(size_t)(k + l) * n4 + i[u]];
+#pragma unroll
+                for (int u = 0; u < NU; ++u)
+#pragma unroll
+                    for (int l = 0; l < LANES; ++l) add(c[u][l], v[u][l]);
+            }
+#pragma unroll
+            for (int l = 0; l < LANES - 1; ++l)
+                if (k + l < splits) {
+#pragma unroll
+                    for (int u = 0; u < NU; ++u) add(c[u][l], part[(size_t)(k + l) * n4 + i[u]]);
+                }
+#pragma unroll
+            for (int u = 0; u < NU; ++u) {
+                float4 t = c[u][0];
+#pragma unroll
+                for (int l = 1; l < LANES; ++l) add(t, c[u][l]);
+                y[i[u]] = t;
+                md2bn::stats_acc(s, ss, t);
+            }
+        };
+        long long p = (long long)blockIdx.x * m.PPB + pl;
+        for (; p + (U - 1) * stride < P; p += U * stride) pixels(p, std::integral_constant<int, U>());
+        for (; p < P; p += stride) pixels(p, std::integral_constant<int, 1>());
+        md2bn::block_partials(s, ss, q, pl, m, C, NG * G, grp * G + blockIdx.x, w, lds);
+    }
 }
 
 template <int OM = 0>
@@ -2300,6 +2513,14 @@
 template <int MODE>
 void launch(const ConvArgs& a, int BN, hipStream_t st) {
     const dim3 grid(a.mblocks * a.nblocks * a.splits);
+    if constexpr (MODE == MODE_FWD) {
+        if (a.bn_part) {
+            if (BN == 128) hipLaunchKernelGGL((conv_gemm_kernel<128, MODE, true>), grid, dim3(kThreads), 0, st, a);
+            else if (BN == 64) hipLaunchKernelGGL((conv_gemm_kernel<64, MODE, true>), grid, dim3(kThreads), 0, st, a);
+            else hipLaunchKernelGGL((conv_gemm_kernel<32, MODE, true>), grid, dim3(kThreads), 0, st, a);
+            return;
+        }
+    }
     if (BN == 128)
         hipLaunchKernelGGL((conv_gemm_kernel<128, MODE>), grid, dim3(kThreads), 0, st, a);
     else if (BN == 64)
@@ -2380,6 +2601,11 @@
 void launch_x6(const ConvArgs& a, hipStream_t st, bool ws = false) {
     const dim3 grid(a.mblocks * a.nblocks * a.splits);
     if (ws && a.bn == 128 && !a.flatk && !a.par) {
+        if (a.bn_part) {
+            if (a.bm == 256) hipLaunchKernelGGL((conv_x6ws_kernel<256, true>), grid, dim3(512), 0, st, a);
+            else hipLaunchKernelGGL((conv_x6ws_kernel<128, true>), grid, dim3(512), 0, st, a);
+            return;
+        }
         if (a.bm == 256) hipLaunchKernelGGL((conv_x6ws_kernel<256>), grid, dim3(512), 0, st, a);
         else hipLaunchKernelGGL((conv_x6ws_kernel<128>), grid, dim3(512), 0, st, a);
         return;
@@ -2445,6 +2671,14 @@
     const dim3 grid(a.mblocks * a.nblocks * a.splits), block(X6Geo<BN, BMX>::NT);
     ConvArgs b = a;
     b.flatk = 0;
+    if constexpr (!BF && BN >= 64) {
+        if (a.bn_part) {
+            if (a.flatk == 64) hipLaunchKernelGGL((conv_x6p_kernel<BN, BMX, 64, false, true>), grid, block, 0, st, b);
+            else if (a.flatk == 32) hipLaunchKernelGGL((conv_x6p_kernel<BN, BMX, 32, false, true>), grid, block, 0, st, b);
+            else hipLaunchKernelGGL((conv_x6p_kernel<BN, BMX, 16, false, true>), grid, block, 0, st, b);
+            return;
+        }
+    }
     if (a.flatk == 64) hipLaunchKernelGGL((conv_x6p_kernel<BN, BMX, 64, BF>), grid, block, 0, st, b);
     else if (a.flatk == 32) hipLaunchKernelGGL((conv_x6p_kernel<BN, BMX, 32, BF>), grid, block, 0, st, b);
     else hipLaunchKernelGGL((conv_x6p_kernel<BN, BMX, 16, BF>), grid, block, 0, st, b);
@@ -2704,22 +2938,58 @@
     return e == hipSuccess ? MD2_OK : md2_report_error(MD2_ERR_HIP, hipGetErrorString(e));
 }
 
-int run(const md2_conv_desc* d, int mode, const float* A, const float* B, float* out, void* ws, void* stream,
-        const char* name) {
-    if (d->flags & MD2_CONV_BF16) return run_bf(d, mode, A, B, out, ws, stream, name);
+ConvArgs planned(const md2_conv_desc* d, int mode, bool& patch, bool& patch_w) {
     ConvArgs a = (mode == MODE_WGRAD && use_x6(d, mode)) ? args_x6_wgrad(d) : args_of(d, mode);
     if (use_x6(d, mode)) flat_k(a, mode);
-    const bool patch = use_x6p(d, mode, a);
-    const bool patch_w = mode == MODE_WGRAD && use_x6pw(d);
+    patch = use_x6p(d, mode, a);
+    patch_w = mode == MODE_WGRAD && use_x6pw(d);
     if (patch) plan_x6p(a, d->flags);
     else if (patch_w) plan_x6pw(a, d->flags);
     else if (use_x6(d, mode)) plan_x6(a, d->flags, mode == MODE_WGRAD);
     else plan(a, d->flags, min_chunks_of(mode));
+    return a;
+}
+
+int bnstats_rows(const md2_conv_desc* d, int bn_groups) {
+    if (!valid(d) || (d->flags & MD2_CONV_BF16) || bn_groups < 1 || d->batch % bn_groups) return 0;
+    bool patch, patch_w;
+    const ConvArgs a = planned(d, MODE_FWD, patch, patch_w);
+    if (!md2bn::channels_ok(a.N)) return 0;
+    const int P = a.M / bn_groups;
+    if (P < 2) return 0;
+    if (a.splits > 1) return md2bn::blocks_for_stats(P, a.N);
+    const bool x6 = use_x6(d, MODE_FWD);
+    if (patch) {
+        if (a.bn < 64) return 0;
+        const int rows = a.mblocks / bn_groups;
+        return rows <= md2bn::kMaxBlocks ? rows : 0;
+    }
+    const bool ws = x6 && (d->flags & MD2_CONV_WS) && a.bn == 128 && !a.flatk;
+    if (x6 && !ws) return 0;
+    const int BMX = x6 ? a.bm : BM;
+    if (bn_groups > 2 && P + 1 < BMX) return 0;
+    int rows = 0;
+    for (int g = 0; g < bn_groups; ++g)
+        rows = std::max(rows, ((g + 1) * P - 1) / BMX - (g * P) / BMX + 1);
+    return rows <= md2bn::kMaxBlocks ? rows : 0;
+}
+
+int run(const md2_conv_desc* d, int mode, const float* A, const float* B, float* out, void* ws, void* stream,
+        const char* name, void* bn_ws = nullptr, int bn_groups = 1) {
+    if (d->flags & MD2_CONV_BF16) return run_bf(d, mode, A, B, out, ws, stream, name);
+    bool patch, patch_w;
+    ConvArgs a = planned(d, mode, patch, patch_w);
     const int BN = a.bn;
     a.a = A;
     a.b = B;
     if ((a.splits > 1 || (use_x6(d, mode) && mode != MODE_WGRAD)) && !ws) return md2_report_error(MD2_ERR_ARG, name);
     a.y = a.splits > 1 ? (float*)ws : out;
+    if (bn_ws && a.splits == 1) {
+        a.bn_part = (float*)bn_ws;
+        a.bn_NG = bn_groups;
+        a.bn_P = a.M / bn_groups;
+        a.bn_rows = bnstats_rows(d, bn_groups);
+    }
     const hipStream_t st = (hipStream_t)stream;
     if (patch_w) {
         const dim3 grid(a.mblocks * a.nblocks * a.splits);
@@ -2750,7 +3020,16 @@
     else launch<MODE_WGRAD>(a, BN, st);
     if (a.splits > 1) {
         const int n4 = a.M * a.N / 4;
-        launch_reduce((const float4*)a.y, (float4*)out, n4, a.splits, st);
+        if (bn_ws) {
+            const long long P = (long long)a.M / bn_groups;
+            const int G = md2bn::blocks_for_stats(P, a.N);
+            auto k = (a.splits >= 16 && (n4 + kRedOut - 1) / kRedOut < 512) ? conv_reduce_stats_kernel<16>
+                                                                            : conv_reduce_stats_kernel<kRedLanes>;
+            hipLaunchKernelGGL(k, dim3(G, bn_groups), dim3(md2bn::kThreads), 0, st, (const float4*)a.y,
+                               (float4*)out, n4, a.splits, P, a.N, G, bn_ws);
+        } else {
+            launch_reduce((const float4*)a.y, (float4*)out, n4, a.splits, st);
+        }
     }
     const hipError_t e = hipGetLastError();
     return e == hipSuccess ? MD2_OK : md2_report_error(MD2_ERR_HIP, hipGetErrorString(e));
@@ -2859,6 +3138,19 @@
     if (!valid(d)) return md2_report_error(MD2_ERR_ARG, "conv_fwd: channels % 4, pad < kernel, sizes < 2^29");
     if (!x || !weight || !y) return md2_report_error(MD2_ERR_ARG, "conv_fwd: NULL operand");
     return run(d, MODE_FWD, x, weight, y, workspace, stream, "conv_fwd: workspace required (K split)");
+}
+
+int md2_conv_bnstats_rows(const md2_conv_desc* d, int bn_groups) { return bnstats_rows(d, bn_groups); }
+
+int md2_conv_fwd_bnstats(const md2_conv_desc* d, const float* x, const float* weight, float* y, void* workspace,
+                         void* bn_workspace, int bn_groups, void* stream) {
+    if (!valid(d)) return md2_report_error(MD2_ERR_ARG, "conv_fwd_bnstats: channels % 4, pad < kernel, sizes < 2^29");
+    if (!x || !weight || !y || !bn_workspace) return md2_report_error(MD2_ERR_ARG, "conv_fwd_bnstats: NULL operand");
+    if (bnstats_rows(d, bn_groups) <= 0)
+        return md2_report_error(MD2_ERR_ARG, "conv_fwd_bnstats: md2_conv_bnstats_rows is 0 for this shape and flags "
+                                             "(run md2_conv_fwd and md2_bn_fwd)");
+    return run(d, MODE_FWD, x, weight, y, workspace, stream, "conv_fwd_bnstats: workspace required (K split)",
+               bn_workspace, bn_groups);
 }
 
 int md2_conv_dgrad(const md2_conv_desc* d, const float* grad_y, const float* weight, float* grad_x,
diff --git a/monodepth2_amd/csrc/md2_bn_partials.h b/monodepth2_amd/csrc/md2_bn_partials.h
--- /dev/null
+++ b/monodepth2_amd/csrc/md2_bn_partials.h
@@ -0,0 +1,83 @@
+
+#pragma once
+
+#include <hip/hip_runtime.h>
+
+#include <stddef.h>
+
+namespace md2bn {
+
+constexpr int kThreads = 256;
+constexpr int kMaxBlocks = 1024;
+
+struct Map {
+    int Q;
+    int QPT;
+    int PPB;
+};
+
+__host__ __device__ inline Map make_map(int C) {
+    Map m;
+    m.Q = C / 4;
+    m.QPT = m.Q > kThreads ? m.Q / kThreads : 1;
+    m.PPB = m.Q >= kThreads ? 1 : kThreads / m.Q;
+    return m;
+}
+
+struct Work {
+    float* part;
+    float* coef;
+};
+
+__host__ __device__ __forceinline__ Work work(void* ws, int G, int C, int NG) {
+    Work w;
+    w.part = (float*)ws;
+    w.coef = w.part + 2 * (size_t)NG * G * C;
+    return w;
+}
+
+__device__ inline void block_partials(float4 a, float4 b, int q, int pl, const Map& m, int C, int rows, int row,
+                                      Work w, float4 (*lds)[kThreads]) {
+    lds[0][threadIdx.x] = a;
+    lds[1][threadIdx.x] = b;
+    __syncthreads();
+    for (int half = m.PPB / 2; half > 0; half /= 2) {
+        if (pl < half) {
+            const int o = threadIdx.x + half * m.Q;
+            const float4 u = lds[0][o], v = lds[1][o];
+            a.x += u.x; a.y += u.y; a.z += u.z; a.w += u.w;
+            b.x += v.x; b.y += v.y; b.z += v.z; b.w += v.w;
+            lds[0][threadIdx.x] = a;
+            lds[1][threadIdx.x] = b;
+        }
+        __syncthreads();
+    }
+    if (pl == 0) {
+        float* pa = w.part + (size_t)(4 * q) * rows + row;
+        float* pb = w.part + ((size_t)C + 4 * q) * rows + row;
+        pa[0] = a.x; pa[rows] = a.y; pa[2 * (size_t)rows] = a.z; pa[3 * (size_t)rows] = a.w;
+        pb[0] = b.x; pb[rows] = b.y; pb[2 * (size_t)rows] = b.z; pb[3 * (size_t)rows] = b.w;
+    }
+    __syncthreads();
+}
+
+__device__ __forceinline__ void stats_acc(float4& s, float4& ss, const float4 v) {
+    s.x += v.x; s.y += v.y; s.z += v.z; s.w += v.w;
+    ss.x += v.x * v.x; ss.y += v.y * v.y; ss.z += v.z * v.z; ss.w += v.w * v.w;
+}
+
+inline int blocks_for_stats(long long P, int C) {
+    const Map m = make_map(C);
+    const long long rows = (P + m.PPB - 1) / m.PPB;
+    const long long g = (rows + 7) / 8;
+    return (int)(g < 1 ? 1 : (g > kMaxBlocks ? kMaxBlocks : g));
+}
+
+inline bool channels_ok(int C) {
+    if (C < 4 || C % 4) return false;
+    const int Q = C / 4;
+    if ((Q & (Q - 1)) != 0) return false;
+    return Q >= kThreads ? (Q % kThreads == 0) : (kThreads % Q == 0);
+}
+
+}
diff --git a/monodepth2_amd/networks/resnet_encoder.py b/monodepth2_amd/networks/resnet_encoder.py
--- a/monodepth2_amd/networks/resnet_encoder.py
+++ b/monodepth2_amd/networks/resnet_encoder.py
@@ -6,8 +6,7 @@
 import torch
 import torch.nn as nn
 
-from ..bn_ops import bn_act, max_pool_3x3s2, max_pool_3x3s2_with_alias
-from ..conv_ops import conv2d
+from ..bn_ops import bn_act, conv_bn_act, max_pool_3x3s2, max_pool_3x3s2_with_alias
 from ..stem_ops import stem_conv
 
 
@@ -39,7 +38,7 @@
 
 
 def _downsample(down: nn.Sequential, x):
-    return bn_act(down[1], conv2d(down[0], x), relu=False)
+    return conv_bn_act(down[0], down[1], x, relu=False)
 
 
 class Bottleneck(nn.Module):
@@ -69,15 +68,15 @@
     skip = None
     for bi, blk in enumerate(layer):
         shortcut = xs if blk.downsample is None else _downsample(blk.downsample, xs)
-        out = bn_act(blk.bn1, conv2d(blk.conv1, x))
+        out = conv_bn_act(blk.conv1, blk.bn1, x)
         if isinstance(blk, Bottleneck):
-            out = bn_act(blk.bn2, conv2d(blk.conv2, out))
+            out = conv_bn_act(blk.conv2, blk.bn2, out)
             bn, conv = blk.bn3, blk.conv3
         else:
             bn, conv = blk.bn2, blk.conv2
         last = bi == n - 1
         k = (2 if skip_alias else 1) if last else 1
-        res = bn_act(bn, conv2d(conv, out), residual=shortcut, aliases=k)
+        res = conv_bn_act(conv, bn, out, residual=shortcut, aliases=k)
         x, xs = res[0], res[1]
         skip = res[2] if (last and skip_alias) else x
     return x, xs, skip
```

New measurement: 1132 images/s (median of 6 runs). Within noise of the previous version (+0.7%).
